# flatironinstitute/bayes-kit

Hardware: AMD Instinct MI355X
Metric: leapfrog steps/sec (whole node), D=1024 × 65 536 chains; ESS/sec (higher is better)
Workload: dtype f64; 1 GPU; BASELINE.json configs[2]: ill-conditioned Gaussian D=1024 (lam=logspace(0,4)), HMC L=64 eps=0.006, diag metric of ones, model-opaque gradient op; chains_per_gpu=65536, dims=1024, leapfrog_steps=64, parallelism=chains sharded x1, chain_tile=8192

## Files before the change

### bayes-kit_amd/bayes_kit_amd/_lib.py

```python
from __future__ import annotations

import ctypes
import os
from ctypes import c_double, c_int, c_int64, c_uint64, c_void_p

import torch

_LIB_PATH = os.path.join(os.path.dirname(os.path.abspath(__file__)), "lib", "libbkhip.so")

RNG_WORDS = 11
RNG_PHILOX = 0
RNG_PCG64 = 1
ACCEPT_HMC = 0
ACCEPT_MALA = 1

P = c_void_p
I = c_int64
F = c_double

SIGNATURES = {
    "bk_version": [],
    "bk_rng_init_philox": [P, I, c_uint64, c_uint64, I, P],
    "bk_refresh_work_elems": [I, I],
    "bk_momentum_refresh": [c_int, P, I, P, F, F, P, I, P, P, P, I, I, P, I, P],
    "bk_momentum_refresh_precond": [c_int, P, I, P, I, P, P, I, I, P, I, P],
    "bk_log_uniform": [c_int, P, I, P, P, I, P],
    "bk_uniform": [c_int, P, I, P, P, I, P],
    "bk_leapfrog_kick_drift": [P, P, P, P, I, P, I, I, P, F, c_int, F, c_int, F, I, I, P],
    "bk_leapfrog_finish": [P, P, I, P, I, I, P, F, c_int, P, I, I, P],
    "bk_precond_pack": [P, P, I, P],
    "bk_leapfrog_finish_precond": [P, P, I, P, I, I, P, F, c_int, P, I, I, P],
    "bk_leapfrog_kick_drift_n": [P, P, P, P, I, P, I, I, P, F, c_int, F, c_int, F, I, I, P, P],
    "bk_leapfrog_first_step_gather": [P, P, P, I, P, P, P, I, P, F, F, I, I, P, P],
    "bk_leapfrog_finish_level": [P, P, I, P, I, I, P, F, c_int, P, I, I, P, P, P, P, P, P, P, P],
    "bk_mh_accept": [c_int, P, P, P, P, P, P, P, P, I, P],
    "bk_select_columns": [P, P, P, P, P, P, I, I, I, P],
    "bk_blend_columns": [P, P, P, P, I, I, I, P],
    "bk_compact_indices": [P, I, P, P, P, P],
    "bk_dr_begin": [P, P, P, P, P, P, I, P],
    "bk_dr_retry_test": [c_int, P, I, P, F, P, I, P],
    "bk_dr_level_begin": [P, P, P, P, P, I, P, P],
    "bk_dr_ghost_update": [P, P, I, P, P, P, P, P],
    "bk_dr_accept_prob": [P, P, P, P, P, F, P, P, I, P, P],
    "bk_dr_accept_test": [c_int, P, I, P, P, P, I, P, P, P, P, P, P, P],
    "bk_dr_accept_prob_test": [c_int, P, I, P, P, P, P, P, F, I, P, P, P, P, P, P, P],
    "bk_dr_accept_prob_ghost": [P, P, P, P, P, F, P, P, I, P, P, P, P],
    "bk_dr_begin_retry": [c_int, P, I, P, P, P, P, P, P, F, P, I, P, I, P],
    "bk_dr_refresh_begin": [c_int, P, I, P, F, F, P, I, P, P, I, I, P, I, P, P, P, P, P, F, P, I, P, P, P],
    "bk_dr_accept_prob_test_next": [c_int, P, I, P, P, P, P, P, F, I, P, P, P, P, P, P, P, P, P],
    "bk_dr_accept_prob_ghost_next": [P, P, P, P, P, F, P, P, I, P, P, P, P, P, P],
    "bk_scatter_columns": [P, P, I, I, P, P, P, P, P, P, I, I, P, P, P, P],
    "bk_mala_propose": [c_int, P, I, P, P, P, I, F, F, I, I, P],
    "bk_mala_propose_from_normals": [P, P, P, I, I, P, I, F, F, I, I, P],
    "bk_mala_propose_from_normals_precond": [P, P, P, I, I, P, P, I, F, F, I, I, P],
    "bk_normals_chain_major": [c_int, P, I, P, I, I, I, P, I, P],
    "bk_mala_logq": [P, P, P, P, I, F, P, P, I, I, P],
    "bk_mala_logq_precond": [P, P, P, P, I, P, F, P, P, I, I, P],
    "bk_mala_single_draw": [c_int, P, I, P, P, P, P, P, P, P, I, P, P, F, F, I, c_int, F, P],
    "bk_mala_step_supported": [I, I, I],
    "bk_mala_step": [P, P, P, P, P, I, P, P, P, P, I, F, F, P, P, P, I, I, P],
    "bk_mala_step_gaussian": [P, P, P, I, P, P, P, P, P, I, F, F, P, P, P, I, I, P],
    "bk_mala_step_precond": [P, P, P, P, P, I, P, P, P, P, P, I, F, F, P, P, P, I, I, P],
    "bk_mala_step_gaussian_precond": [P, P, P, I, P, P, P, P, P, P, I, F, F, P, P, P, I, I, P],
    "bk_target_iso_gaussian_grad": [P, P, P, I, I, I, P],
    "bk_target_diag_gaussian_grad": [P, P, P, I, P, I, I, P],
    "bk_target_funnel_grad": [P, P, P, I, I, I, P],
    "bk_target_iso_gaussian_grad_n": [P, P, P, I, I, I, P, P],
    "bk_target_diag_gaussian_grad_n": [P, P, P, I, P, I, I, P, P],
    "bk_target_funnel_grad_n": [P, P, P, I, I, I, P, P],
    "bk_leapfrog_step_funnel": [P, P, I, P, F, I, I, P, P],
    "bk_leapfrog_step_gaussian": [P, P, I, P, P, F, I, I, P, P],
    "bk_dr_proposal_gaussian": [P, P, P, I, P, P, P, P, P, P, I, P, F, I, I, I, P, P, P, P, P, P, P, P, P, P, P],
    "bk_hmc_trajectory_funnel": [P, P, P, P, P, P, P, I, P, F, I, I, I, P],
    "bk_hmc_trajectory_gaussian": [P, P, P, P, I, P, P, F, I, I, I, P],
    "bk_hmc_draw_gaussian": [P, P, I, P, P, I, P, P, F, I, P, P, P, P, P, P, P, P, P, I, I, P],
    "bk_hmc_draw_gaussian_precond": [P, P, I, P, P, I, P, P, F, I, P, P, P, P, P, P, P, P, P, I, I, P],
    "bk_dr_proposal_funnel": [P, P, P, I, P, P, P, P, P, P, I, P, F, I, I, I, P, P, P, P, P, P, P, P, P, P],
    "bk_dense_metric_apply": [P, I, P, P, I, I, I, P],
    "bk_gemm_chains": [P, I, I, I, P, I, P, I, I, P, I, P],
    "bk_gemm_chains_work_elems": [I, I, I],
    "bk_logistic_residual": [P, I, P, P, I, I, I, P],
    "bk_logistic_finish": [P, P, I, P, I, F, F, P, P, P, I, I, P],
    "bk_dot_columns": [P, P, I, F, P, I, I, P],
    "bk_resample_indices": [P, I, P, I, P, P, P],
    "bk_gather_columns": [P, P, I, P, I, I, I, P],
    "bk_relayout": [P, I, I, P, I, I, I, I, P],
    "bk_welford_update": [P, P, I, P, I, I, I, I, P],
    "bk_record_series": [P, I, P, I, P, P, I, I, I, P],
    "bk_record_series_dev": [P, I, P, I, P, P, I, P, I, I, P],
    "bk_welford_update_dev": [P, P, I, P, I, P, I, I, I, P],
    "bk_rhat_partials": [P, P, I, I, P, P, I, I, P],
    "bk_accept_stat": [P, P, P, P, I, P, P, P],
    "bk_chain_mean_var": [P, I, P, I, P, P, I, P],
    "bk_end_pos_pairs": [P, I, I, P, I, P],
    "bk_ess": [P, I, I, c_int, P, P, I, P],
    "bk_iat_from_acor": [P, I, I, c_int, P, P, I, P],
    "bk_gemm_chains_logistic": [P, I, I, I, P, I, P, I, I, P, P],
    "bk_autocorr": [P, I, I, P, I, I, P],
    "bk_autocorr_fft_work_bytes": [I, I],
    "bk_autocorr_fft": [P, I, I, P, I, I, P, I, P],
    "bk_rank_normalize": [P, F, P, I, P],
    "bk_sort_by_key_work_bytes": [I],
    "bk_sort_by_key": [P, P, P, P, I, P, I, P],
    "bk_count_below": [P, I, P, I, P, P],
    "bk_scatter_ranks": [P, I, F, P, P],
    "bk_ess_multi_work_bytes": [I, I, I],
    "bk_ess_split_moments": [P, I, I, I, c_int, F, P, P, P, P, I, P],
    "bk_ess_between_sq": [P, I, P, P, P, I, P],
    "bk_ess_lag_sums_max_half": [],
    "bk_ess_lag_sums": [P, I, I, I, c_int, F, P, I, I, P, P, I, P],
    "bk_ess_acov_sums": [P, I, I, I, P, I, I, P, P, I, P],
    "bk_ess_indicator": [P, I, I, I, F, P, I, P],
    "bk_select_ranks": [P, P, I, P, I, P, P],
    "bk_host_normals": [c_int, P, P, I],
    "bk_host_uniforms": [c_int, P, P, I],
    "bk_host_log1p": [F],
    "bk_host_exp": [F],
}
_RESTYPE = {"bk_gemm_chains_work_elems": c_int64, "bk_host_log1p": c_double, "bk_host_exp": c_double, "bk_refresh_work_elems": c_int64, "bk_sort_by_key_work_bytes": c_int64,
             "bk_autocorr_fft_work_bytes": c_int64, "bk_ess_multi_work_bytes": c_int64, "bk_ess_lag_sums_max_half": c_int64}


class BkHipError(RuntimeError):
    pass


class GhostLink(ctypes.Structure):
    _fields_ = [("parent_H", P), ("parent_h", P), ("parent_live", P), ("parent_a", P), ("a_out", P),
                ("prob_retry", F), ("next_index", P), ("next_count", P)]


class Ghost0(ctypes.Structure):
    _fields_ = [("h", F), ("steps", I), ("parent_a", P), ("prob_retry", F), ("next_index", P), ("next_count", P),
                ("lanes_out", P), ("lanes_total", P)]


class DiagJob(ctypes.Structure):
    _fields_ = [("theta", P), ("ld_theta", I), ("C", I), ("D", I), ("n_dev", P), ("mean", P), ("m2", P), ("ld", I),
                ("n_offset", I), ("series", P), ("dims", P), ("K", I), ("logp", P), ("capacity", I), ("row_offset", I)]


class ScatterJob(ctypes.Structure):
    _fields_ = [("mask", P), ("index", P), ("n", I), ("D", I), ("dst0", P), ("src0", P), ("dst1", P), ("src1", P),
                ("dst2", P), ("src2", P), ("ld_dst", I), ("ld_src", I), ("sdst", P), ("ssrc", P), ("n_dev", P)]


_lib = None


def lib_path() -> str:
    return _LIB_PATH


def load() -> ctypes.CDLL:
    global _lib
    if _lib is not None:
        return _lib
    if not os.path.exists(_LIB_PATH):
        raise BkHipError(
            f"{_LIB_PATH} is missing: build it with `python bayes-kit_amd/build.py` "
            "(or __graft_entry__.build()).  There is no CPU fallback."
        )
    lib = ctypes.CDLL(_LIB_PATH)
    for name, argtypes in SIGNATURES.items():
        fn = getattr(lib, name)
        fn.argtypes = argtypes
        fn.restype = _RESTYPE.get(name, c_int)
    _lib = lib
    return lib


def require_gpu() -> torch.device:
    load()
    if not torch.cuda.is_available():
        raise BkHipError(
            "bayes_kit_amd needs an AMD Instinct GPU (gfx950) visible to PyTorch-ROCm; "
            "no device found and there is no CPU fallback."
        )
    return torch.device("cuda", torch.cuda.current_device())


class RawDeviceArray:

    _hip = None
    live = 0

    def __init__(self, shape):
        if RawDeviceArray._hip is None:
            RawDeviceArray._hip = ctypes.CDLL("libamdhip64.so")
        self.shape = tuple(int(x) for x in shape)
        n = 8
        for x in self.shape:
            n *= x
        p = c_void_p()
        rc = RawDeviceArray._hip.hipMalloc(ctypes.byref(p), ctypes.c_size_t(max(n, 8)))
        if rc != 0 or not p.value:
            raise BkHipError(f"hipMalloc of {n} bytes failed: hipError_t {rc}")
        self._ptr = p.value
        RawDeviceArray.live += 1
        self.__cuda_array_interface__ = {"shape": self.shape, "typestr": "<f8", "data": (self._ptr, False), "version": 2,
                                         "strides": None}

    def tensor(self):
        t = torch.as_tensor(self, device=torch.device("cuda", torch.cuda.current_device()))
        t._bk_raw = self
        return t

    def __del__(self):
        p, self._ptr = getattr(self, "_ptr", None), None
        cls = type(self)
        hip = getattr(cls, "_hip", None)
        if p and hip is not None:
            cls.live -= 1
            try:
                hip.hipFree(ctypes.c_void_p(p))
            except Exception:
                pass


def check(status: int, what: str) -> None:
    if status != 0:
        kind = "argument/layout error" if status < 0 else "hipError_t"
        raise BkHipError(f"{what} failed: {kind} {status}")


def ptr(t) -> int:
    return 0 if t is None else t.data_ptr()


def stream_handle() -> int:
    return torch.cuda.current_stream().cuda_stream


def _ld(t) -> int:
    if t.dim() != 2 or (t.shape[1] > 1 and t.stride(1) != 1):
        raise BkHipError(f"expected a [D, C] tensor with contiguous chains, got strides {t.stride()}")
    return t.stride(0) if t.shape[0] > 1 else max(t.stride(0), t.shape[1])


class Ops:

    name = "hip"

    def __init__(self):
        self.lib = load()
        self.device = require_gpu()
        self.timed = None
        self.timed_stride = 1
        self._timed_seen = {}

    def _call(self, name, *args):
        rec = self.timed.get(name) if self.timed is not None else None
        if rec is not None and self.timed_stride > 1:
            k = self._timed_seen.get(name, 0)
            self._timed_seen[name] = k + 1
            if k % self.timed_stride:
                rec = None
        if rec is None:
            check(getattr(self.lib, name)(*args), name)
            return
        e0 = torch.cuda.Event(enable_timing=True)
        e1 = torch.cuda.Event(enable_timing=True)
        e0.record()
        check(getattr(self.lib, name)(*args), name)
        e1.record()
        rec.append((e0, e1))

    @staticmethod
    def _s():
        return stream_handle()

    def rng_init_philox(self, state, key0, chain_id0):
        self._call("bk_rng_init_philox", ptr(state), state.stride(0), key0 & (2**64 - 1),
                   chain_id0 & (2**64 - 1), state.shape[1], self._s())

    def refresh_work(self, C, D):
        return torch.empty(self.lib.bk_refresh_work_elems(C, D), dtype=torch.float64, device=self.device)

    def momentum_refresh(self, kind, state, loc_in, loc_mul, scale, out, metric, kin_out, active=None, work=None):
        D, C = out.shape
        self._call("bk_momentum_refresh", kind, ptr(state), state.stride(0), ptr(loc_in), loc_mul, scale,
                   ptr(out), _ld(out), ptr(metric), ptr(kin_out), ptr(active), C, D, ptr(work),
                   0 if work is None else work.numel(), self._s())

    def momentum_refresh_precond(self, kind, state, out, precond, kin_out, work=None):
        D, C = out.shape
        assert precond.is_contiguous() and tuple(precond.shape) == (3, D)
        self._call("bk_momentum_refresh_precond", kind, ptr(state), state.stride(0), ptr(out), _ld(out), ptr(precond),
                   ptr(kin_out), C, D, ptr(work), 0 if work is None else work.numel(), self._s())

    def log_uniform(self, kind, state, out, active=None):
        self._call("bk_log_uniform", kind, ptr(state), state.stride(0), ptr(out), ptr(active),
                   out.shape[0], self._s())

    def uniform(self, kind, state, out, active=None):
        self._call("bk_uniform", kind, ptr(state), state.stride(0), ptr(out), ptr(active), out.shape[0],
                   self._s())

    def kick_drift(self, theta_in, theta_out, rho_in, rho_out, grad, metric, eps,
                   use_pre, pre, use_kick, kick, n_dev=None):
        D, C = theta_out.shape
        ld = _ld(theta_out)
        assert _ld(theta_in) == ld and _ld(rho_in) == ld and _ld(rho_out) == ld
        if n_dev is None:
            self._call("bk_leapfrog_kick_drift", ptr(theta_in), ptr(theta_out), ptr(rho_in), ptr(rho_out), ld,
                       ptr(grad), grad.stride(0), grad.stride(1), ptr(metric), eps, int(use_pre), pre,
                       int(use_kick), kick, C, D, self._s())
        else:
            self._call("bk_leapfrog_kick_drift_n", ptr(theta_in), ptr(theta_out), ptr(rho_in), ptr(rho_out), ld,
                       ptr(grad), grad.stride(0), grad.stride(1), ptr(metric), eps, int(use_pre), pre,
                       int(use_kick), kick, C, D, ptr(n_dev), self._s())

    def first_step_gather(self, theta_in, rho_in, grad_in, src_index, theta_out, rho_out, metric, eps, pre,
                          n_dev=None):
        D, n = theta_out.shape
        ld_in = _ld(theta_in)
        assert _ld(rho_in) == ld_in and _ld(grad_in) == ld_in and _ld(rho_out) == _ld(theta_out)
        self._call("bk_leapfrog_first_step_gather", ptr(theta_in), ptr(rho_in), ptr(grad_in), ld_in,
                   ptr(src_index), ptr(theta_out), ptr(rho_out), _ld(theta_out), ptr(metric), eps, pre,
                   n, D, ptr(n_dev), self._s())

    def leapfrog_finish(self, rho_in, rho_out, grad, metric, half, negate, kin_out, n_dev=None, level=None,
                        lanes_out=None, lanes_total=None):
        D, C = rho_in.shape
        if rho_out is not None:
            assert _ld(rho_out) == _ld(rho_in)
        gs = (0, 0) if grad is None else grad.stride()
        if n_dev is None and level is None and lanes_out is None and lanes_total is None:
            self._call("bk_leapfrog_finish", ptr(rho_in), ptr(rho_out), _ld(rho_in), ptr(grad), gs[0], gs[1],
                       ptr(metric), half, int(negate), ptr(kin_out), C, D, self._s())
            return
        logp, H, h, live = level if level is not None else (None,) * 4
        self._call("bk_leapfrog_finish_level", ptr(rho_in), ptr(rho_out), _ld(rho_in), ptr(grad), gs[0], gs[1],
                   ptr(metric), half, int(negate), ptr(kin_out), C, D, ptr(n_dev), ptr(logp), ptr(H), ptr(h),
                   ptr(live), ptr(lanes_out), ptr(lanes_total), self._s())

    def precond_pack(self, v, precond):
        D = v.shape[0]
        assert v.is_contiguous() and precond.is_contiguous() and tuple(precond.shape) == (3, D)
        self._call("bk_precond_pack", ptr(v), ptr(precond), D, self._s())

    def leapfrog_finish_precond(self, rho_in, rho_out, grad, precond, half, negate, kin_out):
        D, C = rho_in.shape
        if rho_out is not None:
            assert _ld(rho_out) == _ld(rho_in)
        assert precond.is_contiguous() and tuple(precond.shape) == (3, D)
        gs = (0, 0) if grad is None else grad.stride()
        self._call("bk_leapfrog_finish_precond", ptr(rho_in), ptr(rho_out), _ld(rho_in), ptr(grad), gs[0], gs[1],
                   ptr(precond), half, int(negate), ptr(kin_out), C, D, self._s())

    def accept_stat(self, lp_cur, a_cur, lp_prop, a_prop, out, work=None):
        C = lp_cur.shape[0]
        if work is None:
            work = torch.empty(max(2, 2 * ((C + 255) // 256)), dtype=torch.float64, device=lp_cur.device)
        assert work.numel() >= 2 * ((C + 255) // 256)
        self._call("bk_accept_stat", ptr(lp_cur), ptr(a_cur), ptr(lp_prop), ptr(a_prop), C, ptr(out), ptr(work), self._s())

    def mh_accept(self, mode, lp_cur, a_cur, lp_prop, a_prop, log_u, mask, ret, count):
        self._call("bk_mh_accept", mode, ptr(lp_cur), ptr(a_cur), ptr(lp_prop), ptr(a_prop), ptr(log_u),
                   ptr(mask), ptr(ret), ptr(count), lp_cur.shape[0], self._s())

    def select_columns(self, mask, dst0, src0, dst1=None, src1=None, copy0=None):
        D, C = dst0.shape
        ld = _ld(dst0)
        assert _ld(src0) == ld and (dst1 is None or (_ld(dst1) == ld and _ld(src1) == ld))
        assert copy0 is None or _ld(copy0) == ld
        self._call("bk_select_columns", ptr(mask), ptr(dst0), ptr(src0), ptr(dst1), ptr(src1), ptr(copy0), ld,
                   C, D, self._s())


    def blend_columns(self, mask, a, b, out):
        D, C = a.shape
        ld = _ld(a)
        assert _ld(b) == ld and _ld(out) == ld
        self._call("bk_blend_columns", ptr(mask), ptr(a), ptr(b), ptr(out), ld, C, D, self._s())

    def compact_indices(self, mask, n, idx_out, count_out, n_dev=None):
        self._call("bk_compact_indices", ptr(mask), n, ptr(idx_out), ptr(count_out), ptr(n_dev), self._s())

    def dr_begin(self, logp, kin, cur_H, cur_h, rej, alive):
        self._call("bk_dr_begin", ptr(logp), ptr(kin), ptr(cur_H), ptr(cur_h), ptr(rej), ptr(alive),
                   logp.shape[0], self._s())

    def dr_retry_test(self, kind, state, rej, prob_retry, alive):
        self._call("bk_dr_retry_test", kind, ptr(state), state.stride(0), ptr(rej), float(prob_retry),
                   ptr(alive), alive.shape[0], self._s())

    def dr_level_begin(self, logp, kin, H, h, live, n, n_dev=None):
        self._call("bk_dr_level_begin", ptr(logp), ptr(kin), ptr(H), ptr(h), ptr(live), n, ptr(n_dev), self._s())

    def dr_ghost_update(self, ga, sub_index, m, h, live, a, n_dev=None):
        self._call("bk_dr_ghost_update", ptr(ga), ptr(sub_index), m, ptr(h), ptr(live), ptr(a), ptr(n_dev),
                   self._s())

    def dr_accept_prob(self, H, cur_H, h, cur_h, cur_index, prob_retry, live, a, n, n_dev=None):
        self._call("bk_dr_accept_prob", ptr(H), ptr(cur_H), ptr(h), ptr(cur_h), ptr(cur_index),
                   float(prob_retry), ptr(live), ptr(a), n, ptr(n_dev), self._s())

    def dr_accept_test(self, kind, state, chain_index, a, H, n, cur_H, cur_h, rej, alive, accepted, n_dev=None):
        self._call("bk_dr_accept_test", kind, ptr(state), state.stride(0), ptr(chain_index), ptr(a), ptr(H),
                   n, ptr(cur_H), ptr(cur_h), ptr(rej), ptr(alive), ptr(accepted), ptr(n_dev), self._s())

    def dr_accept_prob_test(self, kind, state, chain_index, H, h, live, a, prob_retry, n, cur_H, cur_h, rej, alive,
                            accepted, n_dev=None):
        self._call("bk_dr_accept_prob_test", kind, ptr(state), state.stride(0), ptr(chain_index), ptr(H), ptr(h),
                   ptr(live), ptr(a), float(prob_retry), n, ptr(cur_H), ptr(cur_h), ptr(rej), ptr(alive),
                   ptr(accepted), ptr(n_dev), self._s())

    def dr_accept_prob_ghost(self, H, parent_H, h, parent_h, sub_index, prob_retry, live, a, n, parent_live, parent_a,
                             n_dev=None):
        self._call("bk_dr_accept_prob_ghost", ptr(H), ptr(parent_H), ptr(h), ptr(parent_h), ptr(sub_index),
                   float(prob_retry), ptr(live), ptr(a), n, ptr(n_dev), ptr(parent_live), ptr(parent_a), self._s())

    def dr_begin_retry(self, kind, state, logp, kin, cur_H, cur_h, rej, alive, prob_retry, counters, draw_counter=None):
        self._call("bk_dr_begin_retry", kind, ptr(state), state.stride(0), ptr(logp), ptr(kin), ptr(cur_H), ptr(cur_h),
                   ptr(rej), ptr(alive), float(prob_retry), ptr(counters), 0 if counters is None else counters.numel(),
                   ptr(draw_counter), logp.shape[0], self._s())

    def dr_refresh_begin(self, kind, state, loc_in, loc_mul, scale, out, metric, kin_out, work, logp, cur_H, cur_h, rej,
                         alive, prob_retry, counters, draw_counter=None, side=None):
        D, C = out.shape
        self._call("bk_dr_refresh_begin", kind, ptr(state), state.stride(0), ptr(loc_in), loc_mul, scale, ptr(out),
                   _ld(out), ptr(metric), ptr(kin_out), C, D, ptr(work), 0 if work is None else work.numel(), ptr(logp),
                   ptr(cur_H), ptr(cur_h), ptr(rej), ptr(alive), float(prob_retry), ptr(counters),
                   0 if counters is None else counters.numel(), ptr(draw_counter),
                   None if side is None else ctypes.cast(ctypes.pointer(side), P), self._s())

    def diag_job(self, theta, n_dev, welford=None, record=None):
        D, C = theta.shape
        assert n_dev.dtype == torch.int64 and (welford is not None or record is not None)
        j = DiagJob(ptr(theta), _ld(theta), C, D, ptr(n_dev), None, None, 0, 0, None, None, 0, None, 0, 0)
        if welford is not None:
            mean, m2, n_offset = welford
            assert _ld(m2) == _ld(mean)
            j.mean, j.m2, j.ld, j.n_offset = ptr(mean), ptr(m2), _ld(mean), int(n_offset)
        if record is not None:
            dims, logp, series, row_offset = record
            j.series, j.dims, j.K, j.logp = ptr(series), ptr(dims), (0 if dims is None else dims.numel()), ptr(logp) or None
            j.capacity, j.row_offset = series.shape[1], int(row_offset)
        return j

    def dr_accept_prob_test_next(self, kind, state, chain_index, H, h, live, a, prob_retry, n, cur_H, cur_h, rej, alive,
                                 accepted, next_index, next_count, n_dev=None):
        self._call("bk_dr_accept_prob_test_next", kind, ptr(state), state.stride(0), ptr(chain_index), ptr(H), ptr(h),
                   ptr(live), ptr(a), float(prob_retry), n, ptr(cur_H), ptr(cur_h), ptr(rej), ptr(alive),
                   ptr(accepted), ptr(n_dev), ptr(next_index), ptr(next_count), self._s())

    def dr_accept_prob_ghost_next(self, H, parent_H, h, parent_h, sub_index, prob_retry, live, a, n, parent_live,
                                  parent_a, next_index, next_count, n_dev=None):
        self._call("bk_dr_accept_prob_ghost_next", ptr(H), ptr(parent_H), ptr(h), ptr(parent_h), ptr(sub_index),
                   float(prob_retry), ptr(live), ptr(a), n, ptr(n_dev), ptr(parent_live), ptr(parent_a),
                   ptr(next_index), ptr(next_count), self._s())

    def scatter_columns(self, mask, index, n, dsts, srcs, sdst=None, ssrc=None, n_dev=None):
        d = list(dsts) + [None] * (3 - len(dsts))
        s_ = list(srcs) + [None] * (3 - len(srcs))
        D = dsts[0].shape[0]
        self._call("bk_scatter_columns", ptr(mask), ptr(index), n, D, ptr(d[0]), ptr(s_[0]), ptr(d[1]),
                   ptr(s_[1]), ptr(d[2]), ptr(s_[2]), _ld(dsts[0]), _ld(srcs[0]), ptr(sdst), ptr(ssrc),
                   ptr(n_dev), self._s())

    def mala_propose(self, kind, state, theta, grad, theta_prop, eps, sqrt2eps):
        D, C = theta.shape
        ld = _ld(theta)
        assert _ld(grad) == ld and _ld(theta_prop) == ld
        self._call("bk_mala_propose", kind, ptr(state), state.stride(0), ptr(theta), ptr(grad),
                   ptr(theta_prop), ld, eps, sqrt2eps, C, D, self._s())

    def mala_propose_from_normals(self, theta, grad, z, theta_prop, eps, sqrt2eps):
        D, C = theta.shape
        ld = _ld(theta)
        assert _ld(grad) == ld and _ld(theta_prop) == ld and tuple(z.shape) == (D, C)
        self._call("bk_mala_propose_from_normals", ptr(theta), ptr(grad), ptr(z), z.stride(0), z.stride(1),
                   ptr(theta_prop), ld, eps, sqrt2eps, C, D, self._s())

    def mala_propose_from_normals_precond(self, theta, grad, z, precond, theta_prop, eps, sqrt2eps):
        D, C = theta.shape
        ld = _ld(theta)
        assert _ld(grad) == ld and _ld(theta_prop) == ld and tuple(z.shape) == (D, C)
        assert precond.is_contiguous() and tuple(precond.shape) == (3, D)
        self._call("bk_mala_propose_from_normals_precond", ptr(theta), ptr(grad), ptr(z), z.stride(0), z.stride(1),
                   ptr(precond), ptr(theta_prop), ld, eps, sqrt2eps, C, D, self._s())

    def normals_chain_major(self, kind, state, zt, D, snapshot=None, max_workgroups=0):
        C = zt.shape[0]
        assert zt.stride(1) == 1 and zt.shape[1] >= D
        assert snapshot is None or (snapshot.shape == state.shape and snapshot.stride(0) == state.stride(0))
        self._call("bk_normals_chain_major", kind, ptr(state), state.stride(0), ptr(zt), zt.stride(0), C, D,
                   ptr(snapshot), int(max_workgroups or 0), self._s())

    def mala_logq(self, theta, grad, theta_prop, grad_prop, eps, lp_forward, lp_reverse):
        D, C = theta.shape
        ld = _ld(theta)
        assert _ld(grad) == ld and _ld(theta_prop) == ld and _ld(grad_prop) == ld
        self._call("bk_mala_logq", ptr(theta), ptr(grad), ptr(theta_prop), ptr(grad_prop), ld, eps,
                   ptr(lp_forward), ptr(lp_reverse), C, D, self._s())

    def mala_logq_precond(self, theta, grad, theta_prop, grad_prop, precond, eps, lp_forward, lp_reverse):
        D, C = theta.shape
        ld = _ld(theta)
        assert _ld(grad) == ld and _ld(theta_prop) == ld and _ld(grad_prop) == ld
        assert precond.is_contiguous() and tuple(precond.shape) == (3, D)
        self._call("bk_mala_logq_precond", ptr(theta), ptr(grad), ptr(theta_prop), ptr(grad_prop), ld, ptr(precond), eps,
                   ptr(lp_forward), ptr(lp_reverse), C, D, self._s())

    def mala_step_supported(self, C, D, ld):
        return bool(self.lib.bk_mala_step_supported(C, D, ld))

    def mala_step(self, theta, theta_out, grad, theta_prop, grad_prop, lp, lp_prop, log_u, zt_next, eps, sqrt2eps,
                  mask, ret, count):
        D, C = theta.shape
        ld = _ld(theta)
        assert _ld(theta_out) == ld and _ld(grad) == ld and _ld(theta_prop) == ld and _ld(grad_prop) == ld
        ldz = 0
        if zt_next is not None:
            assert zt_next.shape[0] == C and zt_next.stride(1) == 1 and zt_next.shape[1] >= D
            ldz = zt_next.stride(0)
        self._call("bk_mala_step", ptr(theta), ptr(theta_out), ptr(grad), ptr(theta_prop), ptr(grad_prop), ld,
                   ptr(lp), ptr(lp_prop), ptr(log_u), ptr(zt_next), ldz, eps, sqrt2eps, ptr(mask), ptr(ret),
                   ptr(count), C, D, self._s())

    def mala_step_precond(self, theta, theta_out, grad, theta_prop, grad_prop, precond, lp, lp_prop, log_u, zt_next, eps,
                          sqrt2eps, mask, ret, count):
        D, C = theta.shape
        ld = _ld(theta)
        assert _ld(theta_out) == ld and _ld(grad) == ld and _ld(theta_prop) == ld and _ld(grad_prop) == ld
        assert precond.is_contiguous() and tuple(precond.shape) == (3, D)
        ldz = 0
        if zt_next is not None:
            assert zt_next.shape[0] == C and zt_next.stride(1) == 1 and zt_next.shape[1] >= D
            ldz = zt_next.stride(0)
        self._call("bk_mala_step_precond", ptr(theta), ptr(theta_out), ptr(grad), ptr(theta_prop), ptr(grad_prop), ld,
                   ptr(precond), ptr(lp), ptr(lp_prop), ptr(log_u), ptr(zt_next), ldz, eps, sqrt2eps, ptr(mask), ptr(ret),
                   ptr(count), C, D, self._s())

    def mala_step_gaussian(self, lam, theta, theta_out, theta_prop, lp, lp_prop, log_u, zt_next, eps, sqrt2eps, mask, ret,
                           count, precond=None):
        D, C = theta.shape
        ld = _ld(theta)
        assert _ld(theta_out) == ld and _ld(theta_prop) == ld
        ldz = 0
        if zt_next is not None:
            assert zt_next.shape[0] == C and zt_next.stride(1) == 1 and zt_next.shape[1] >= D
            ldz = zt_next.stride(0)
        if precond is not None:
            assert precond.is_contiguous() and tuple(precond.shape) == (3, D)
            self._call("bk_mala_step_gaussian_precond", ptr(theta), ptr(theta_out), ptr(theta_prop), ld, ptr(lam),
                       ptr(precond), ptr(lp), ptr(lp_prop), ptr(log_u), ptr(zt_next), ldz, eps, sqrt2eps, ptr(mask),
                       ptr(ret), ptr(count), C, D, self._s())
            return
        self._call("bk_mala_step_gaussian", ptr(theta), ptr(theta_out), ptr(theta_prop), ld, ptr(lam), ptr(lp), ptr(lp_prop),
                   ptr(log_u), ptr(zt_next), ldz, eps, sqrt2eps, ptr(mask), ptr(ret), ptr(count), C, D, self._s())

    def target_grad(self, kind, params, theta, grad, logp, n_dev=None):
        D, C = theta.shape
        ld = _ld(theta)
        if grad is not None:
            assert _ld(grad) == ld
        if n_dev is not None:
            if kind == "iso_gaussian":
                self._call("bk_target_iso_gaussian_grad_n", ptr(theta), ptr(grad), ptr(logp), ld, C, D, ptr(n_dev),
                           self._s())
            elif kind == "diag_gaussian":
                self._call("bk_target_diag_gaussian_grad_n", ptr(theta), ptr(grad), ptr(logp), ld, ptr(params),
                           C, D, ptr(n_dev), self._s())
            elif kind == "funnel":
                self._call("bk_target_funnel_grad_n", ptr(theta), ptr(grad), ptr(logp), ld, C, D, ptr(n_dev),
                           self._s())
            else:
                raise BkHipError(f"built-in target {kind!r} has no counted gradient")
        elif kind == "iso_gaussian":
            self._call("bk_target_iso_gaussian_grad", ptr(theta), ptr(grad), ptr(logp), ld, C, D, self._s())
        elif kind == "diag_gaussian":
            self._call("bk_target_diag_gaussian_grad", ptr(theta), ptr(grad), ptr(logp), ld, ptr(params),
                       C, D, self._s())
        elif kind == "funnel":
            self._call("bk_target_funnel_grad", ptr(theta), ptr(grad), ptr(logp), ld, C, D, self._s())
        else:
            raise BkHipError(f"unknown built-in target {kind!r}")

    def hmc_trajectory_funnel(self, theta_in, rho, grad_in, theta_out, grad_out, logp_out, kin_out, metric, eps, steps):
        D, C = theta_in.shape
        ld = _ld(theta_in)
        assert all(_ld(t) == ld for t in (rho, grad_in, theta_out, grad_out))
        self._call("bk_hmc_trajectory_funnel", ptr(theta_in), ptr(rho), ptr(grad_in), ptr(theta_out), ptr(grad_out),
                   ptr(logp_out), ptr(kin_out), ld, ptr(metric), eps, steps, C, D, self._s())

    def leapfrog_step_funnel(self, theta, rho, metric, h, n_dev=None):
        D, n = theta.shape
        ld = _ld(theta)
        assert _ld(rho) == ld
        self._call("bk_leapfrog_step_funnel", ptr(theta), ptr(rho), ld, ptr(metric), h, n, D, ptr(n_dev), self._s())

    def hmc_trajectory_gaussian(self, theta_in, theta_out, rho_in, rho_out, lam, metric, eps, steps):
        D, C = theta_in.shape
        ld = _ld(theta_in)
        assert _ld(theta_out) == ld and _ld(rho_in) == ld and _ld(rho_out) == ld
        self._call("bk_hmc_trajectory_gaussian", ptr(theta_in), ptr(theta_out), ptr(rho_in), ptr(rho_out), ld,
                   ptr(lam), ptr(metric), eps, steps, C, D, self._s())

    def hmc_draw_gaussian(self, theta_in, theta_out, rho_in, zt, lam, metric, eps, steps, part, kin0, kin1, lp_out,
                          accept=None, precond=None):
        D, C = theta_in.shape
        ld = _ld(theta_in)
        assert _ld(theta_out) == ld and (rho_in is None or _ld(rho_in) == ld) and part.numel() >= 12 * C
        ldz = 0
        if zt is not None:
            assert zt.shape[0] == C and zt.stride(1) == 1 and zt.shape[1] >= D
            ldz = zt.stride(0)
        lp_cur, log_u, mask, ret, count = accept if accept is not None else (None,) * 5
        name = "bk_hmc_draw_gaussian"
        if precond is not None:
            assert metric is None and precond.is_contiguous() and tuple(precond.shape) == (3, D)
            name, metric = "bk_hmc_draw_gaussian_precond", precond
        self._call(name, ptr(theta_in), ptr(theta_out), ld, ptr(rho_in), ptr(zt), ldz, ptr(lam),
                   ptr(metric), eps, steps, ptr(part), ptr(kin0), ptr(kin1), ptr(lp_out), ptr(lp_cur), ptr(log_u),
                   ptr(mask), ptr(ret), ptr(count), C, D, self._s())

    def scatter_job(self, mask, index, n, dsts, srcs, sdst=None, ssrc=None, n_dev=None):
        d = list(dsts) + [None] * (3 - len(dsts))
        s_ = list(srcs) + [None] * (3 - len(srcs))
        return ScatterJob(ptr(mask) or None, ptr(index) or None, n, dsts[0].shape[0], ptr(d[0]) or None, ptr(s_[0]) or None,
                          ptr(d[1]) or None, ptr(s_[1]) or None, ptr(d[2]) or None, ptr(s_[2]) or None, _ld(dsts[0]),
                          _ld(srcs[0]), ptr(sdst) or None, ptr(ssrc) or None, ptr(n_dev) or None)

    def ghost_link(self, parent_H, parent_h, parent_live, parent_a, a_out, prob_retry, next_index=None, next_count=None):
        return GhostLink(ptr(parent_H), ptr(parent_h), ptr(parent_live), ptr(parent_a), ptr(a_out), float(prob_retry),
                         ptr(next_index) or None, ptr(next_count) or None)

    def ghost0(self, h, steps, parent_a, prob_retry, next_index=None, next_count=None, lanes_out=None, lanes_total=None):
        return Ghost0(float(h), int(steps), ptr(parent_a), float(prob_retry), ptr(next_index) or None,
                      ptr(next_count) or None, ptr(lanes_out) or None, ptr(lanes_total) or None)

    def dr_proposal_gaussian(self, lam, theta_in, rho_in, grad_in, src_index, theta_out, rho_out, grad_out, logp_out,
                             kin_out, metric, h, steps, n_dev=None, lanes_out=None, lanes_total=None, level=None, job=None,
                             ghost=None, ghost0=None):
        D, n = theta_out.shape
        H, hh, live = level if level is not None else (None, None, None)
        ld_in = _ld(theta_in)
        assert _ld(rho_in) == ld_in and (grad_in is None or _ld(grad_in) == ld_in)
        ld_out = _ld(theta_out)
        assert _ld(rho_out) == ld_out and (grad_out is None or _ld(grad_out) == ld_out)
        self._call("bk_dr_proposal_gaussian", ptr(theta_in), ptr(rho_in), ptr(grad_in), ld_in, ptr(src_index),
                   ptr(theta_out), ptr(rho_out), ptr(grad_out), ptr(logp_out), ptr(kin_out), ld_out, ptr(metric),
                   h, steps, n, D, ptr(n_dev), ptr(lanes_out), ptr(lanes_total), ptr(H), ptr(hh), ptr(live),
                   None if job is None else ctypes.byref(job), None if ghost is None else ctypes.byref(ghost),
                   None if ghost0 is None else ctypes.byref(ghost0), ptr(lam), self._s())

    def leapfrog_step_gaussian(self, lam, theta, rho, metric, h, n_dev=None):
        D, n = theta.shape
        ld = _ld(theta)
        assert _ld(rho) == ld
        self._call("bk_leapfrog_step_gaussian", ptr(theta), ptr(rho), ld, ptr(lam), ptr(metric), h, n, D, ptr(n_dev), self._s())

    def dr_proposal_funnel(self, theta_in, rho_in, grad_in, src_index, theta_out, rho_out, grad_out, logp_out,
                           kin_out, metric, h, steps, n_dev=None, lanes_out=None, lanes_total=None, level=None, job=None,
                           ghost=None, ghost0=None):
        D, n = theta_out.shape
        H, hh, live = level if level is not None else (None, None, None)
        ld_in = _ld(theta_in)
        assert _ld(rho_in) == ld_in and (grad_in is None or _ld(grad_in) == ld_in)
        ld_out = _ld(theta_out)
        assert _ld(rho_out) == ld_out and (grad_out is None or _ld(grad_out) == ld_out)
        args = (ptr(theta_in), ptr(rho_in), ptr(grad_in), ld_in, ptr(src_index),
                ptr(theta_out), ptr(rho_out), ptr(grad_out), ptr(logp_out), ptr(kin_out), ld_out, ptr(metric),
                h, steps, n, D, ptr(n_dev), ptr(lanes_out), ptr(lanes_total), ptr(H), ptr(hh), ptr(live))
        self._call("bk_dr_proposal_funnel", *args, None if job is None else ctypes.byref(job),
                   None if ghost is None else ctypes.byref(ghost),
                   None if ghost0 is None else ctypes.byref(ghost0), self._s())

    def dense_metric_apply(self, M, X, Y):
        D, C = X.shape
        assert _ld(Y) == _ld(X)
        self._call("bk_dense_metric_apply", ptr(M), _ld(M), ptr(X), ptr(Y), _ld(X), C, D, self._s())

    def gemm_chains_work(self, R, K, C):
        n = int(self.lib.bk_gemm_chains_work_elems(R, K, C))
        return torch.empty(n, dtype=torch.float64, device=self.device) if n > 0 else None

    def gemm_chains(self, A, X, Y, work=None):
        R, K = A.shape
        assert X.shape[0] == K and Y.shape[0] == R
        self._call("bk_gemm_chains", ptr(A), _ld(A), R, K, ptr(X), _ld(X), ptr(Y), _ld(Y), X.shape[1],
                   ptr(work), 0 if work is None else work.numel(), self._s())

    def gemm_chains_logistic(self, A, X, Y, y_rows):
        R, K = A.shape
        assert X.shape[0] == K and Y.shape[0] == R and y_rows.numel() == R
        self._call("bk_gemm_chains_logistic", ptr(A), _ld(A), R, K, ptr(X), _ld(X), ptr(Y), _ld(Y), X.shape[1],
                   ptr(y_rows), self._s())

    def logistic_residual(self, Z, y, part, segments=None):
        N, C = Z.shape
        self._call("bk_logistic_residual", ptr(Z), _ld(Z), ptr(y), ptr(part), N, C,
                   part.shape[0] if part is not None else int(segments or 256), self._s())

    def logistic_finish(self, G, theta, part, inv_prior_var, t, grad, logp, loglik):
        D, C = theta.shape
        ld = _ld(theta)
        assert (G is None or _ld(G) == ld) and (grad is None or _ld(grad) == ld)
        self._call("bk_logistic_finish", ptr(G), ptr(theta), ld, ptr(part), 1 if part is None else part.shape[0], inv_prior_var, t,
                   ptr(grad), ptr(logp), ptr(loglik), C, D, self._s())

    def dot_columns(self, x, y, scale, out):
        D, C = x.shape
        assert _ld(y) == _ld(x)
        self._call("bk_dot_columns", ptr(x), ptr(y), _ld(x), scale, ptr(out), C, D, self._s())

    def resample_indices(self, weights, u, cdf_work, idx_out):
        self._call("bk_resample_indices", ptr(weights), weights.shape[0], ptr(u), u.shape[0], ptr(cdf_work),
                   ptr(idx_out), self._s())

    def gather_columns(self, index, src, dst):
        D, m = dst.shape
        self._call("bk_gather_columns", ptr(index), ptr(src), _ld(src), ptr(dst), _ld(dst), m, D, self._s())

    def relayout(self, src, dst):
        D, C = dst.shape
        self._call("bk_relayout", ptr(src), src.stride(0), src.stride(1), ptr(dst), dst.stride(0),
                   dst.stride(1), C, D, self._s())

    def welford_update(self, mean, m2, theta, n):
        D, C = theta.shape
        assert _ld(m2) == _ld(mean)
        self._call("bk_welford_update", ptr(mean), ptr(m2), _ld(mean), ptr(theta), _ld(theta), n, C, D, self._s())

    def record_series(self, theta, dims, logp, series, row):
        D, C = theta.shape
        assert series.is_contiguous() and series.shape[2] == C
        self._call("bk_record_series", ptr(theta), _ld(theta), ptr(dims), 0 if dims is None else dims.numel(), ptr(logp),
                   ptr(series), series.shape[1], row, C, self._s())

    def record_series_dev(self, theta, dims, logp, series, row_dev, row_offset):
        D, C = theta.shape
        assert series.is_contiguous() and series.shape[2] == C and row_dev.dtype == torch.int64
        self._call("bk_record_series_dev", ptr(theta), _ld(theta), ptr(dims), 0 if dims is None else dims.numel(),
                   ptr(logp), ptr(series), series.shape[1], ptr(row_dev), int(row_offset), C, self._s())

    def welford_update_dev(self, mean, m2, theta, n_dev, n_offset):
        D, C = theta.shape
        assert _ld(m2) == _ld(mean) and n_dev.dtype == torch.int64
        self._call("bk_welford_update_dev", ptr(mean), ptr(m2), _ld(mean), ptr(theta), _ld(theta), ptr(n_dev),
                   int(n_offset), C, D, self._s())

    def rhat_partials(self, mean, m2, n, center, out):
        D, C = mean.shape
        assert _ld(m2) == _ld(mean)
        self._call("bk_rhat_partials", ptr(mean), ptr(m2), _ld(mean), n, ptr(center), ptr(out), C, D,
                   self._s())

    def chain_mean_var(self, x, lengths, mean, var):
        N, C = x.shape
        self._call("bk_chain_mean_var", ptr(x), _ld(x), ptr(lengths), N, ptr(mean), ptr(var), C, self._s())

    def rank_normalize(self, rank, S, out):
        self._call("bk_rank_normalize", ptr(rank), float(S), ptr(out), rank.numel(), self._s())

    def sort_by_key(self, keys, vals):
        n = keys.numel()
        ko, vo = torch.empty_like(keys), torch.empty_like(vals)
        if n == 0:
            return ko, vo
        nb = self.lib.bk_sort_by_key_work_bytes(n)
        if nb < 0:
            raise BkHipError("bk_sort_by_key_work_bytes failed")
        work = torch.empty(max(1, nb), dtype=torch.uint8, device=keys.device)
        self._call("bk_sort_by_key", ptr(keys), ptr(ko), ptr(vals), ptr(vo), n, ptr(work), work.numel(), self._s())
        return ko, vo

    def count_below(self, sorted_keys, queries):
        out = torch.empty(queries.numel(), dtype=torch.int64, device=queries.device)
        self._call("bk_count_below", ptr(sorted_keys), sorted_keys.numel(), ptr(queries), queries.numel(), ptr(out),
                   self._s())
        return out

    def scatter_ranks(self, payload, base, out):
        self._call("bk_scatter_ranks", ptr(payload), payload.numel(), float(base), ptr(out), self._s())

    def autocorr(self, x, out):
        N, C = x.shape
        self._call("bk_autocorr", ptr(x), _ld(x), N, ptr(out), _ld(out), C, self._s())

    def autocorr_fft_work_bytes(self, N, C):
        return int(self.lib.bk_autocorr_fft_work_bytes(N, C))

    def autocorr_fft(self, x, out):
        N, C = x.shape
        work = torch.empty(max(16, self.lib.bk_autocorr_fft_work_bytes(N, C)), dtype=torch.uint8, device=x.device)
        self._call("bk_autocorr_fft", ptr(x), _ld(x), N, ptr(out), _ld(out), C, ptr(work), work.numel(), self._s())

    def end_pos_pairs(self, acor, out):
        N, C = acor.shape
        self._call("bk_end_pos_pairs", ptr(acor), max(C, acor.stride(0)) if N else C, N, ptr(out), C, self._s())

    def iat_from_acor(self, acor, estimator, ess_out, iat_out=None):
        N, C = acor.shape
        self._call("bk_iat_from_acor", ptr(acor), _ld(acor), N, estimator, ptr(ess_out), ptr(iat_out), C, self._s())

    def ess(self, x, estimator, ess_out, iat_out=None):
        N, C = x.shape
        self._call("bk_ess", ptr(x), _ld(x), N, estimator, ptr(ess_out), ptr(iat_out), C, self._s())

    def _ess_work(self, n, C, nlags, device):
        nb = int(self.lib.bk_ess_multi_work_bytes(n, C, nlags))
        if nb < 0:
            raise BkHipError("bk_ess_multi_work_bytes failed")
        return torch.empty(nb // 8, dtype=torch.float64, device=device)

    def ess_lag_sums_max_half(self):
        return int(self.lib.bk_ess_lag_sums_max_half())

    def ess_split_moments(self, x, q, chain_mean, chain_g0):
        N, C = x.shape
        out = torch.empty(3, dtype=torch.float64, device=x.device)
        work = self._ess_work(N // 2, C, 1, x.device)
        self._call("bk_ess_split_moments", ptr(x), _ld(x), N, C, 0 if q is None else 1, 0.0 if q is None else float(q),
                   ptr(chain_mean), ptr(chain_g0), ptr(out), ptr(work), work.numel() * 8, self._s())
        return out

    def ess_between_sq(self, chain_mean, centre):
        out = torch.empty(1, dtype=torch.float64, device=chain_mean.device)
        work = self._ess_work(1, chain_mean.numel(), 1, chain_mean.device)
        self._call("bk_ess_between_sq", ptr(chain_mean), chain_mean.numel(), ptr(centre), ptr(out), ptr(work),
                   work.numel() * 8, self._s())
        return out

    def ess_lag_sums(self, x, q, chain_mean, lag0, nlags):
        N, C = x.shape
        out = torch.empty(nlags, dtype=torch.float64, device=x.device)
        work = self._ess_work(N // 2, C, nlags, x.device)
        self._call("bk_ess_lag_sums", ptr(x), _ld(x), N, C, 0 if q is None else 1, 0.0 if q is None else float(q),
                   ptr(chain_mean), lag0, nlags, ptr(out), ptr(work), work.numel() * 8, self._s())
        return out

    def ess_acov_sums(self, acor, chain_g0, lag0, nlags):
        n, C = acor.shape
        out = torch.empty(nlags, dtype=torch.float64, device=acor.device)
        work = self._ess_work(n, C, nlags, acor.device)
        self._call("bk_ess_acov_sums", ptr(acor), _ld(acor), n, C, ptr(chain_g0), lag0, nlags, ptr(out), ptr(work),
                   work.numel() * 8, self._s())
        return out

    def ess_indicator(self, x, q, out):
        n, C = x.shape
        self._call("bk_ess_indicator", ptr(x), _ld(x), n, C, float(q), ptr(out), _ld(out), self._s())

    def select_ranks(self, rank, values, targets, out):
        self._call("bk_select_ranks", ptr(rank), ptr(values), rank.numel(), ptr(targets), targets.numel(), ptr(out),
                   self._s())


_default_ops = None


def default_ops() -> Ops:
    global _default_ops
    if _default_ops is None:
        _default_ops = Ops()
    return _default_ops
```

### bayes-kit_amd/bayes_kit_amd/hmc.py

```python
from __future__ import annotations

from typing import Optional

import numpy as np
import torch

from . import _lib
from ._engine import ManyChainSampler


class HMCDiag(ManyChainSampler):
    TUNING = ("graph", "prefetch_rng", "tune_placement", "chain_tile")

    def __init__(
        self,
        model,
        stepsize: float,
        steps: int,
        metric_diag=None,
        init=None,
        seed=None,
        *,
        chains: Optional[int] = None,
        chain_id0: int = 0,
        path: str = "auto",
        metric_dense=None,
        precond_diag=None,
        tuning: Optional[dict] = None,
        ops=None,
        **knobs,
    ):
        fuse_builtin, fuse_steps = self._resolve_path(path)
        tn = self._resolve_tuning(tuning, knobs)
        chain_tile, graph = tn.get("chain_tile"), tn.get("graph")
        prefetch_rng, tune_placement = tn.get("prefetch_rng"), tn.get("tune_placement")
        self._stepsize = stepsize
        self._steps = steps
        self._pd = None
        self._stat = None
        if precond_diag is not None and (metric_diag is not None or metric_dense is not None):
            raise ValueError("give precond_diag or metric_diag / metric_dense, not both")
        self._setup(model, metric_diag, init, seed, chains, chain_id0, ops)
        self._M = None
        if metric_dense is not None:
            if metric_diag is not None:
                raise ValueError("give metric_diag or metric_dense, not both")
            if not self._batched:
                raise ValueError("metric_dense needs a batched device model")
            self._install_metric_dense(metric_dense)
            fuse_builtin = False
        if precond_diag is not None:
            self._install_precond(precond_diag)
        self._init_graph(graph, prefetch_rng)
        self._fused_draw = (bool(fuse_builtin) and self._batched and self._M is None and hasattr(model, "bk_hmc_draw"))
        if self._pd is not None and not hasattr(model, "bk_hmc_draw_precond"):
            self._fused_draw = False
        self._fused = self._fused_draw
        self._lanes_traj = (bool(fuse_builtin) and self._batched and self._M is None and hasattr(model, "bk_hmc_proposal"))
        self._step_hook = (bool(fuse_steps) and self._batched and self._M is None and hasattr(model, "bk_leapfrog_step"))
        self._traj_hook = (bool(fuse_builtin) and self._step_hook and hasattr(model, "bk_leapfrog_trajectory"))
        self._chain_tile = self._pick_tile(chain_tile)
        self._fused_zt = self._fused_draw and self._rng_kind == _lib.RNG_PHILOX and self._dim >= 32
        D, C, dev = self._dim, self._C, self._ops.device
        f64 = dict(dtype=torch.float64, device=dev)
        self._rho_bufs = [None if self._fused_zt else torch.empty((D, C), **f64)]
        self._theta_p = torch.empty((D, C), **f64)
        self._grad = torch.empty((D, C), **f64)
        self._grad_p = torch.empty((D, C), **f64)
        self._lp = torch.empty(C, **f64)
        self._lp_p = torch.empty(C, **f64)
        self._kin0_bufs = [torch.empty(C, **f64)]
        self._kin1 = torch.empty(C, **f64)
        self._logu_bufs = [torch.empty(C, **f64)]
        self._ret = torch.empty(C, **f64)
        self._mask = torch.empty(C, dtype=torch.uint8, device=dev)
        self._accepted = torch.zeros(1, dtype=torch.int32, device=dev)
        if self._fused_draw:
            self._part = torch.empty(12 * C, **f64)
        if self._fused_zt:
            dp = (D + 7) // 8 * 8
            self._zt_bufs = [torch.empty((C, dp), **f64)]
        if self._M is not None:
            self._mv = torch.empty((D, C), **f64)
            self._mv_rng = torch.empty((D, C), **f64)
        self._have_cache = False
        self._draws = 0
        self._rebind = self._batched and not self._use_graph
        if prefetch_rng is None:
            prefetch_rng = self._batched and self._ops.device.type == "cuda"
        self._prefetch = bool(prefetch_rng) and self._batched and not self._use_graph
        self._pf_slot = 0
        self._pf_ready = False
        self._pf_event = None
        self._pf_kin_stale = False
        self._snap = None
        if self._prefetch:
            if self._fused_zt:
                self._zt_bufs.append(torch.empty_like(self._zt_bufs[0]))
                self._rho_bufs.append(None)
            else:
                self._rho_bufs.append(torch.empty((D, C), **f64))
            self._kin0_bufs.append(torch.empty(C, **f64))
            self._logu_bufs.append(torch.empty(C, **f64))
            self._init_side_stream()
            if self._fused_zt:
                self._snap = [torch.empty_like(self._rng_state) for _ in range(2)]
            else:
                self._rng_logical = self._rng_state.clone()
        self.placement = None
        if self._wants_placement_tuning(tune_placement) and not self._fused and self._M is None:
            self._tune_placement()

    def _install_metric_dense(self, metric_dense):
        if isinstance(metric_dense, torch.Tensor) and metric_dense.dim() == 1 and self._M is not None:
            v = metric_dense.to(device=self._ops.device, dtype=torch.float64)
            if v.shape[0] != self._dim:
                raise ValueError(f"a diagonal metric needs {self._dim} entries")
            self._M.copy_(torch.diag(v))
            self._M_chol.copy_(torch.diag(torch.sqrt(v)))
            self._M_inv.copy_(torch.diag(1.0 / v))
            return
        Mt = torch.as_tensor(metric_dense, dtype=torch.float64).cpu()
        if tuple(Mt.shape) != (self._dim, self._dim):
            raise ValueError(f"metric_dense must be ({self._dim}, {self._dim})")
        Mt = 0.5 * (Mt + Mt.t())
        dev_ = self._ops.device
        chol = torch.linalg.cholesky(Mt)
        inv = torch.linalg.inv(Mt)
        inv = 0.5 * (inv + inv.t())
        if self._M is None:
            self._M, self._M_chol, self._M_inv = (x.to(dev_).contiguous() for x in (Mt, chol, inv))
        else:
            self._M.copy_(Mt)
            self._M_chol.copy_(chol)
            self._M_inv.copy_(inv)

    def set_metric_dense(self, metric_dense):
        if self._M is None:
            raise ValueError("this sampler was built without metric_dense")
        self._install_metric_dense(metric_dense)
        if self._prefetch and self._pf_ready:
            if self._pf_event is not None:
                torch.cuda.current_stream().wait_event(self._pf_event)
            self._pf_ready, self._pf_event = False, None

    def _install_precond(self, v):
        if self._M is not None or (self._pd is None and self._metric_dev is not None):
            raise ValueError("precond_diag cannot be combined with metric_diag / metric_dense")
        vt = torch.as_tensor(v, dtype=torch.float64).reshape(-1)
        if vt.shape[0] != self._dim:
            raise ValueError(f"precond_diag has {vt.shape[0]} entries, model has {self._dim} dims")
        vt = vt.to(self._ops.device).contiguous()
        if not bool((torch.isfinite(vt) & (vt > 0.0)).all()):
            raise ValueError("precond_diag must hold finite, positive variances")
        if self._pd is None:
            self._pd = torch.empty((3, self._dim), dtype=torch.float64, device=self._ops.device)
            self._metric_dev, self._metric_identity = self._pd[0], False
            self._drop_graphs()
        self._ops.precond_pack(vt, self._pd)

    def set_precond_diag(self, v):
        self._install_precond(v)
        if self._fused_draw and not hasattr(self._model, "bk_hmc_draw_precond"):
            self._leave_whole_draw()
        if getattr(self, "_prefetch", False) and self._pf_ready and not self._fused_zt:
            if self._pf_event is not None:
                torch.cuda.current_stream().wait_event(self._pf_event)
            self._rng_state.copy_(self._rng_logical)
            self._pf_ready, self._pf_event = False, None

    def _leave_whole_draw(self):
        if self._prefetch and self._pf_ready:
            if self._pf_event is not None:
                torch.cuda.current_stream().wait_event(self._pf_event)
            self._rng_state.copy_(self._snap[self._pf_slot] if self._snap is not None else self._rng_logical)
            self._pf_ready, self._pf_event = False, None
        self._fused_draw = self._fused = self._fused_zt = False
        self._rho_bufs = [r if r is not None else torch.empty_like(self._theta_p) for r in self._rho_bufs]
        if self._prefetch and self._snap is not None:
            self._snap, self._rng_logical = None, self._rng_state.clone()
        self._have_cache = False
        self._drop_graphs()

    @property
    def precond_diag(self):
        return None if self._pd is None else self._pd[0].cpu().numpy().copy()

    def _tune_placement(self):
        ops, m, eps = self._ops, self._metric_dev, float(self._stepsize)
        n_rho = len(self._rho_bufs)

        builtin = hasattr(self._model, "bk_eval")

        def cost(a):
            tp, gp, rhos = a[0], a[1], a[2:2 + n_rho]
            ms = sum(self._time_ms(lambda r=r: ops.kick_drift(tp, tp, r, r, gp, m, eps, False, 0.0, True, eps))
                     for r in rhos) / n_rho
            if builtin:
                ms += self._time_ms(lambda: self._model.bk_eval(tp, gp, None))
            return ms

        chosen, rep = self._tune_roles([self._theta_p, self._grad_p] + list(self._rho_bufs) + [self._grad], cost)
        self._theta_p, self._grad_p = chosen[0], chosen[1]
        self._rho_bufs = chosen[2:2 + n_rho]
        self._grad = chosen[2 + n_rho]
        key = "step_ms" if builtin else "kick_drift_ms"
        self.placement = {key + "_as_allocated": rep["ms_as_allocated"], key + "_chosen": rep["ms_chosen"],
                          "assignments_tried": rep["assignments_tried"]}

    LLC_BYTES = 192 << 20
    MIN_TILE = 8192

    @classmethod
    def default_chain_tile(cls, C, D):
        t = cls.LLC_BYTES // (3 * 8 * D)
        t -= t % 2
        return t if t >= cls.MIN_TILE and C >= 2 * t else C

    def _pick_tile(self, chain_tile):
        C = self._C
        if chain_tile is None:
            opaque_loop = (self._batched and self._M is None and hasattr(self._model, "bk_eval")
                           and not self._fused_draw and not self._lanes_traj and not self._step_hook)
            return self.default_chain_tile(C, self._dim) if opaque_loop else C
        t = int(chain_tile)
        return C if t <= 0 or t >= C else max(2, t - t % 2)

    def accept_rate(self) -> float:
        n = self._draws * self._C
        return float(self._accepted.item()) / n if n else float("nan")

    @property
    def last_accept(self):
        return self._mask.bool() if self._batched else bool(self._mask[0].item())

    def _set_metric(self, m):
        if self._pd is not None:
            raise ValueError("metric_diag cannot be combined with precond_diag")
        super()._set_metric(m)
        self._pf_kin_stale = True


    def rng_state(self):
        return self._logical_rng().cpu().numpy().view(np.uint64)

    def _state_tensors(self):
        return {"theta": self._theta_dc, "grad": self._grad, "lp": self._lp, "accepted": self._accepted}

    def _logical_rng(self):
        if getattr(self, "_prefetch", False) and self._pf_ready:
            if self._pf_event is not None:
                self._pf_event.synchronize()
            return self._rng_logical if self._snap is None else self._snap[self._pf_slot]
        return self._rng_state

    def load_state_dict(self, sd):
        if getattr(self, "_prefetch", False) and self._pf_ready:
            torch.cuda.synchronize()
            self._pf_ready, self._pf_event = False, None
        if self._rebind:
            self._theta_dc = torch.empty_like(self._theta_dc)
        super().load_state_dict(sd)

    def _state_extra(self):
        return {"stepsize": float(self._stepsize), "precond_diag": None if self._pd is None else self._pd[0].cpu().clone()}

    def _load_extra(self, extra):
        if "stepsize" in extra:
            self._stepsize = extra["stepsize"]
        pv = extra.get("precond_diag")
        if pv is not None:
            self._install_precond(pv)
            if self._fused_draw and not hasattr(self._model, "bk_hmc_draw_precond"):
                self._leave_whole_draw()
        elif self._pd is not None and "precond_diag" in extra:
            raise ValueError("checkpoint was written without precond_diag, this sampler has one")

    def _after_load(self):
        self._pf_event, self._pf_slot, self._pf_ready, self._pf_kin_stale = None, 0, False, False

    def _refresh_stale_kinetic(self):
        if self._pf_kin_stale and self._pf_ready and not self._fused_draw:
            self._ops.leapfrog_finish(self._rho_bufs[self._pf_slot], None, None, self._metric_dev, 0.0, False,
                                      self._kin0_bufs[self._pf_slot])
        self._pf_kin_stale = False

    def _randomness(self, slot):
        ops = self._ops
        if self._fused_zt:
            ops.normals_chain_major(self._rng_kind, self._rng_state, self._zt_bufs[slot], self._dim,
                                    None if self._snap is None else self._snap[slot])
        elif self._pd is not None:
            ops.momentum_refresh_precond(self._rng_kind, self._rng_state, self._rho_bufs[slot], self._pd,
                                         self._kin0_bufs[slot], self._rng_work)
        elif self._M is None:
            ops.momentum_refresh(self._rng_kind, self._rng_state, None, 0.0, 1.0, self._rho_bufs[slot],
                                 self._metric_dev, None if self._fused_draw else self._kin0_bufs[slot], None,
                                 self._rng_work)
        else:
            ops.momentum_refresh(self._rng_kind, self._rng_state, None, 0.0, 1.0, self._mv_rng, None, None,
                                 None, self._rng_work)
            ops.dense_metric_apply(self._M_chol, self._mv_rng, self._rho_bufs[slot])
            self._dense_kinetic(self._rho_bufs[slot], self._kin0_bufs[slot], self._mv_rng)
        ops.log_uniform(self._rng_kind, self._rng_state, self._logu_bufs[slot])

    def _dense_kinetic(self, rho, kin_out, scratch):
        self._ops.dense_metric_apply(self._M_inv, rho, scratch)
        self._ops.dot_columns(rho, scratch, 0.5, kin_out)

    def _mg(self, g):
        if self._M is None:
            return g
        self._ops.dense_metric_apply(self._M, self._materialize_dense(g), self._mv)
        return self._mv

    def _materialize_dense(self, g):
        if g.dim() == 2 and g.stride(1) == 1:
            return g
        self._ops.relayout(g, self._grad_p)
        return self._grad_p

    def _current_randomness(self):
        self._zt_slot = 0 if not self._prefetch else self._pf_slot
        if not self._prefetch:
            self._randomness(0)
            return self._rho_bufs[0], self._kin0_bufs[0], self._logu_bufs[0]
        cur = self._pf_slot
        if not self._pf_ready:
            self._randomness(cur)
            self._pf_kin_stale = False
        else:
            if self._pf_event is not None:
                torch.cuda.current_stream().wait_event(self._pf_event)
            self._refresh_stale_kinetic()
        return self._rho_bufs[cur], self._kin0_bufs[cur], self._logu_bufs[cur]

    def _start_next_randomness(self):
        if not self._prefetch:
            return
        main = torch.cuda.current_stream()
        nxt = 1 - self._pf_slot
        ready, ev = self._ev_ready[nxt], self._ev_done[nxt]
        ready.record(main)
        self._side.wait_event(ready)
        with torch.cuda.stream(self._side):
            if self._snap is None:
                self._rng_logical.copy_(self._rng_state)
            self._randomness(nxt)
            ev.record(self._side)
        self._pf_event, self._pf_slot, self._pf_ready = ev, nxt, True

    def _graph_key(self):
        return (float(self._stepsize), int(self._steps))

    def warmup(self, draws, target_accept=0.8, adapt_metric=True, group=None):
        from .adapt import DualAveraging, warmup_windows
        from .diagnostics import RunningMoments, _gather_sum, pooled_variance_from_moments

        draws = int(draws)
        if draws < 1:
            raise ValueError(f"warmup: draws must be >= 1, got {draws}")
        if not 0.0 < float(target_accept) < 1.0:
            raise ValueError(f"warmup: target_accept must be inside (0, 1), got {target_accept}")
        if adapt_metric and (self._M is not None or (self._pd is None and self._metric_dev is not None)):
            raise ValueError("warmup: adapt_metric=True estimates precond_diag, which cannot be combined with "
                             "metric_diag / metric_dense (pass adapt_metric=False to tune the step size alone)")
        if not self._batched:
            raise ValueError("warmup needs a batched device model (the statistics are taken across chains)")
        ops, dev, C, D = self._ops, self._ops.device, self._C, self._dim
        init, term, ends = warmup_windows(draws)
        if not adapt_metric:
            ends = []
        da = DualAveraging(float(self._stepsize), float(target_accept))
        mom = RunningMoments(D, C, ops) if ends else None
        self._stat = torch.zeros(3, dtype=torch.float64, device=dev)
        self._stat[2] = float(C)
        self._stat_work = torch.empty(max(2, 2 * ((C + 255) // 256)), dtype=torch.float64, device=dev)
        eps_hist, alpha_hist, nan_chains = [], [], 0
        try:
            for it in range(draws):
                eps_hist.append(float(self._stepsize))
                self._draw()
                self._join_side_stream()
                self._draws += 1
                tot = _gather_sum(self._stat, group).cpu()
                chains_total = float(tot[2])
                alpha = float(tot[0]) / chains_total
                alpha_hist.append(alpha)
                nan_chains += int(tot[1])
                if mom is not None and init <= it < draws - term:
                    mom.update(self._theta_dc, layout="dc")
                eps = da.step(alpha)
                if it + 1 in ends:
                    n_eff = float(mom.n) * chains_total
                    var = pooled_variance_from_moments(mom.mean, mom.m2, mom.n, ops, group)
                    self.set_precond_diag(n_eff / (n_eff + 5.0) * var + 1e-3 * 5.0 / (n_eff + 5.0))
                    mom.reset()
                    eps = da.final()
                    da.restart(eps)
                if it + 1 == draws:
                    eps = da.final()
                self._stepsize = eps
        finally:
            self._stat, self._stat_work = None, None
            del mom
            self._drop_graphs()
        return {"stepsize": float(self._stepsize), "precond_diag": self.precond_diag, "eps": eps_hist, "alpha": alpha_hist,
                "window_ends": list(ends), "nan_chains": nan_chains}

    def sample(self):
        self._run_draw(self._draw)
        self._join_side_stream()
        self._draws += 1
        return self._draw_out(self._theta_dc, self._ret)

    def _draw(self):
        ops = self._ops
        eps, L, m = float(self._stepsize), int(self._steps), self._metric_dev
        half = 0.5 * eps
        th, thp = self._theta_dc, self._theta_p
        mirror = not self._batched

        rho, kin0, logu = self._current_randomness()
        self._start_next_randomness()

        if self._fused_draw:
            if not self._have_cache:
                self._eval_logp(th, self._lp)
                self._have_cache = True
            zt = self._zt_bufs[self._zt_slot] if self._fused_zt else None
            m_draw = None if (m is None or self._metric_identity) else m
            accept = (self._lp, logu, self._mask, self._ret, self._accepted)
            in_launch = accept if self._stat is None else None
            if self._pd is not None:
                self._model.bk_hmc_draw_precond(th, thp, rho, zt, self._pd, eps, L, self._part, kin0, self._kin1, self._lp_p,
                                                accept=in_launch)
            else:
                self._model.bk_hmc_draw(th, thp, rho, zt, m_draw, eps, L, self._part, kin0, self._kin1, self._lp_p,
                                        accept=in_launch)
            if in_launch is None:
                self._accept(kin0, logu)
            self._take(th, thp)
            return

        if self._lanes_traj and L >= 1 and self._pd is None:
            if not self._have_cache:
                self._materialize(self._eval_grad(th, self._grad, self._lp), self._grad)
                self._have_cache = True
            if self._model.bk_hmc_proposal(th, rho, self._grad, thp, self._grad_p, self._lp_p, self._kin1, m, eps, L):
                self._accept(kin0, logu)
                self._take(th, thp, self._grad, self._grad_p)
                return

        if mirror:
            self._eval_logp(th, self._lp)
            g = self._eval_grad(th, self._grad, None)
        else:
            if not self._have_cache:
                self._materialize(self._eval_grad(th, self._grad, self._lp), self._grad)
                self._have_cache = True
            g = self._grad

        if self._M is not None:
            m = None
        if L == 0:
            ops.kick_drift(th, thp, rho, rho, self._mg(g), m, 0.0, True, -half, False, 0.0)
            g_last = g
            if not mirror:
                self._lp_p.copy_(self._lp)
        elif (self._traj_hook and not mirror and self._chain_tile >= self._C
              and self._model.bk_leapfrog_trajectory(th, rho, g, None, thp, rho, self._grad_p, self._lp_p, m, eps, L,
                                                     hmc_first=True)):
            self._grad_calls += L
            g_last = self._grad_p
        else:
            g_last = None
            T = self._chain_tile
            for c0 in range(0, self._C, T):
                c1 = min(self._C, c0 + T)
                tile = (c0, c1) != (0, self._C)
                v = (lambda a: a[:, c0:c1]) if tile else (lambda a: a)
                th_t, thp_t, rho_t, gp_t, g_t = v(th), v(thp), v(rho), v(self._grad_p), v(g)
                lp_t = self._lp_p[c0:c1] if tile else self._lp_p
                gl = None
                for n in range(L):
                    last = n == L - 1
                    if n == 0:
                        ops.kick_drift(th_t, thp_t, rho_t, rho_t, self._mg(g_t), m, eps, True, -half, True, eps)
                    elif self._step_hook and not mirror:
                        self._grad_calls += 1
                        self._model.bk_leapfrog_step(thp_t, rho_t, m, eps)
                    else:
                        ops.kick_drift(thp_t, thp_t, rho_t, rho_t, self._mg(gl), m, eps, False, 0.0, True, eps)
                    if self._step_hook and not mirror and not last:
                        continue
                    want_lp = lp_t if (last and not mirror) else None
                    gl = self._eval_grad(thp_t, gp_t, want_lp)
                if tile:
                    self._materialize(gl, gp_t)
                    g_last = self._grad_p
                else:
                    g_last = gl
        if self._pd is not None:
            ops.leapfrog_finish_precond(rho, None, g_last, self._pd, half, False, self._kin1)
        elif self._M is None:
            ops.leapfrog_finish(rho, None, g_last, m, half, False, self._kin1)
        else:
            ops.leapfrog_finish(rho, rho, self._mg(g_last), None, half, False, None)
            self._dense_kinetic(rho, self._kin1, self._mv)
        if mirror:
            self._eval_logp(thp, self._lp_p)
        self._accept(kin0, logu)
        if mirror:
            self._select(self._mask, th, thp)
        else:
            gp = self._materialize(g_last, self._grad_p) if L > 0 else None
            self._take(th, thp, self._grad if gp is not None else None, gp)

    def _accept(self, kin0, logu):
        if self._stat is not None:
            self._ops.accept_stat(self._lp, kin0, self._lp_p, self._kin1, self._stat, self._stat_work)
        self._ops.mh_accept(_lib.ACCEPT_HMC, self._lp, kin0, self._lp_p, self._kin1, logu,
                            self._mask, self._ret, self._accepted)

    def _take(self, th, thp, g=None, gp=None):
        if not self._rebind:
            self._select(self._mask, th, thp, g, gp)
            return
        self._out = torch.empty_like(th)
        self._ops.blend_columns(self._mask, th, thp, self._out)
        self._theta_dc = self._out
        if gp is not None:
            self._ops.select_columns(self._mask, g, gp)
```

### bayes-kit_amd/build.py

```python
#!/usr/bin/env python3
import os
import subprocess
import sys
from concurrent.futures import ThreadPoolExecutor

HERE = os.path.dirname(os.path.abspath(__file__))
CSRC = os.path.join(HERE, "csrc")
OUT_DIR = os.path.join(HERE, "bayes_kit_amd", "lib")
OBJ_DIR = os.path.join(HERE, "build")
LIB = os.path.join(OUT_DIR, "libbkhip.so")
SOURCES = ["bk_rng.hip", "bk_integrator.hip", "bk_targets.hip", "bk_targets_gauss_lanes.hip", "bk_diag.hip", "bk_dr.hip", "bk_dense.hip", "bk_smc.hip", "bk_mala.hip", "bk_sort.hip", "bk_fft.hip", "bk_ess_multi.hip"]
HEADERS = ["bk_common.hpp", "bk_ess_tile.hpp", "bk_rng.hpp", "bk_lanes.hpp", "bk_elementwise.hpp", "bk_mala_step.hpp", "ziggurat_tables.inc", os.path.join("..", "..", "include", "bkhip.h"),
           os.path.join("..", "..", "include", "bkhip_math.h")]
FLAGS = ["--offload-arch=gfx950", "-O3", "-std=c++17", "-fPIC", "-ffp-contract=off", "-fno-fast-math",
         "-Wall", "-Wno-unused-function"]
FILE_FLAGS = {"bk_rng.hip": ["-mllvm", "-disable-machine-licm"]}


def _hipcc():
    for c in (os.environ.get("HIPCC"), "/opt/rocm/bin/hipcc", "hipcc"):
        if c and (os.path.isabs(c) and os.path.exists(c) or not os.path.isabs(c)):
            return c
    return "hipcc"


def _stale(target, deps):
    if not os.path.exists(target):
        return True
    t = os.path.getmtime(target)
    return any(os.path.getmtime(d) > t for d in deps)


def build(force=False, verbose=True):
    os.makedirs(OUT_DIR, exist_ok=True)
    os.makedirs(OBJ_DIR, exist_ok=True)
    hdrs = [os.path.join(CSRC, h) for h in HEADERS] + [os.path.abspath(__file__)]
    hipcc = _hipcc()
    jobs = []
    objs = []
    for s in SOURCES:
        src = os.path.join(CSRC, s)
        obj = os.path.join(OBJ_DIR, s.replace(".hip", ".o"))
        objs.append(obj)
        if force or _stale(obj, [src] + hdrs):
            jobs.append([hipcc] + FLAGS + FILE_FLAGS.get(s, []) + ["-c", src, "-o", obj])

    def run(cmd):
        if verbose:
            print(" ".join(cmd), flush=True)
        subprocess.check_call(cmd)

    with ThreadPoolExecutor(max_workers=4) as ex:
        list(ex.map(run, jobs))
    if force or jobs or _stale(LIB, objs):
        run([hipcc, "--offload-arch=gfx950", "-shared", "-fPIC", "-o", LIB] + objs)
    return LIB


PLUGIN_DIR = os.path.join(HERE, "..", "examples", "plugin_target")
PLUGINS = ["ar1_target", "funnel_target"]
PLUGIN_LIB = os.path.join(PLUGIN_DIR, "libar1_target.so")


def build_example_plugin(force=False, verbose=True):
    libs = []
    for name in PLUGINS:
        src = os.path.abspath(os.path.join(PLUGIN_DIR, name + ".hip"))
        lib = os.path.abspath(os.path.join(PLUGIN_DIR, "lib" + name + ".so"))
        public = [os.path.abspath(os.path.join(HERE, "..", "include", h)) for h in ("bkhip.h", "bkhip_math.h")]
        if force or _stale(lib, [src] + public):
            cmd = [_hipcc(), "--offload-arch=gfx950", "-O3", "-std=c++17", "-fPIC", "-shared", "-ffp-contract=off",
                   src, "-o", lib]
            if verbose:
                print(" ".join(cmd), flush=True)
            subprocess.check_call(cmd)
        libs.append(lib)
    return libs[0]


C_HOST_SRC = os.path.join(HERE, "..", "examples", "c_host", "hmc_main.c")
C_HOST_BIN = os.path.join(HERE, "..", "examples", "c_host", "hmc_main")


def build_c_host_example(force=False, verbose=True):
    src, exe = os.path.abspath(C_HOST_SRC), os.path.abspath(C_HOST_BIN)
    if force or _stale(exe, [src, LIB, os.path.join(HERE, "..", "include", "bkhip.h")]):
        rocm = os.environ.get("ROCM_PATH", "/opt/rocm")
        cmd = ["gcc", "-std=gnu11", "-O2", "-D__HIP_PLATFORM_AMD__", src, "-I" + os.path.join(rocm, "include"),
               "-I" + os.path.abspath(os.path.join(HERE, "..", "include")), "-L" + OUT_DIR, "-lbkhip",
               "-L" + os.path.join(rocm, "lib"), "-lamdhip64",
               "-Wl,-rpath,$ORIGIN/../../bayes-kit_amd/bayes_kit_amd/lib", "-Wl,-rpath," + os.path.join(rocm, "lib"),
               "-o", exe]
        if verbose:
            print(" ".join(cmd), flush=True)
        subprocess.check_call(cmd)
    return exe


if __name__ == "__main__":
    print(build(force="--force" in sys.argv))
    print(build_example_plugin(force="--force" in sys.argv))
    print(build_c_host_example(force="--force" in sys.argv))
```

### bayes-kit_amd/csrc/bk_integrator.hip

```cpp
#include "bk_common.hpp"

namespace {

constexpr int KD_ROWS = 4;
constexpr int KD_BLOCK = 256;

__device__ __forceinline__ double kd_elem(double th, double rho, double g, double m, bool has_m,
                                          double eps, int use_pre, double pre, int use_kick,
                                          double kick, double& rho_new) {
  double t = has_m ? m * g : g;
  double r = rho;
  if (use_pre) r = r + pre * t;
  if (use_kick) r = r + kick * t;
  rho_new = r;
  return th + eps * r;
}

typedef double dvec2 __attribute__((ext_vector_type(2)));

template <int ROWS, bool NT>
__global__ __launch_bounds__(KD_BLOCK) void k_kick_drift_v2(
    const double* th_in, double* th_out, const double* rho_in, double* rho_out, i64 ld,
    const double* grad, i64 ldg, const double* metric, double eps, int use_pre, double pre,
    int use_kick, double kick, i64 C2, i64 D) {
  i64 c2 = (i64)blockIdx.x * KD_BLOCK + threadIdx.x;
  i64 d0 = (i64)blockIdx.y * ROWS;
  if (c2 >= C2) return;
  dvec2 t[ROWS], r[ROWS], g[ROWS];
  double m[ROWS];
#pragma unroll
  for (int i = 0; i < ROWS; ++i) {
    i64 d = d0 + i;
    if (d < D) {
      const dvec2* pt = reinterpret_cast<const dvec2*>(th_in + d * ld + 2 * c2);
      const dvec2* pr = reinterpret_cast<const dvec2*>(rho_in + d * ld + 2 * c2);
      const dvec2* pg = reinterpret_cast<const dvec2*>(grad + d * ldg + 2 * c2);
      if (NT) {
        t[i] = __builtin_nontemporal_load(pt);
        r[i] = __builtin_nontemporal_load(pr);
        g[i] = __builtin_nontemporal_load(pg);
      } else {
        t[i] = *pt;
        r[i] = *pr;
        g[i] = *pg;
      }
      m[i] = metric ? metric[d] : 1.0;
    }
  }
#pragma unroll
  for (int i = 0; i < ROWS; ++i) {
    i64 d = d0 + i;
    if (d < D) {
      dvec2 rn, tn;
      double rx, ry;
      tn.x = kd_elem(t[i].x, r[i].x, g[i].x, m[i], metric != nullptr, eps, use_pre, pre, use_kick, kick, rx);
      tn.y = kd_elem(t[i].y, r[i].y, g[i].y, m[i], metric != nullptr, eps, use_pre, pre, use_kick, kick, ry);
      rn.x = rx;
      rn.y = ry;
      dvec2* qr = reinterpret_cast<dvec2*>(rho_out + d * ld + 2 * c2);
      dvec2* qt = reinterpret_cast<dvec2*>(th_out + d * ld + 2 * c2);
      if (NT) {
        __builtin_nontemporal_store(rn, qr);
        __builtin_nontemporal_store(tn, qt);
      } else {
        *qr = rn;
        *qt = tn;
      }
    }
  }
}

__global__ __launch_bounds__(KD_BLOCK) void k_kick_drift_s(
    const double* th_in, double* th_out, const double* rho_in, double* rho_out, i64 ld,
    const double* grad, i64 ldg_d, i64 ldg_c, const double* metric, double eps, int use_pre,
    double pre, int use_kick, double kick, i64 C, i64 D) {
  i64 c = (i64)blockIdx.x * KD_BLOCK + threadIdx.x;
  i64 d0 = (i64)blockIdx.y * KD_ROWS;
  if (c >= C) return;
  double t[KD_ROWS], r[KD_ROWS], g[KD_ROWS], m[KD_ROWS];
#pragma unroll
  for (int i = 0; i < KD_ROWS; ++i) {
    i64 d = d0 + i;
    if (d < D) {
      t[i] = th_in[d * ld + c];
      r[i] = rho_in[d * ld + c];
      g[i] = grad[d * ldg_d + c * ldg_c];
      m[i] = metric ? metric[d] : 1.0;
    }
  }
#pragma unroll
  for (int i = 0; i < KD_ROWS; ++i) {
    i64 d = d0 + i;
    if (d < D) {
      double rn;
      double tn = kd_elem(t[i], r[i], g[i], m[i], metric != nullptr, eps, use_pre, pre, use_kick, kick, rn);
      rho_out[d * ld + c] = rn;
      th_out[d * ld + c] = tn;
    }
  }
}

constexpr int TR_TILE = 64;
__global__ __launch_bounds__(256) void k_kick_drift_tr(
    const double* th_in, double* th_out, const double* rho_in, double* rho_out, i64 ld,
    const double* grad, i64 ldg_c, const double* metric, double eps, int use_pre, double pre,
    int use_kick, double kick, i64 C, i64 D) {
  __shared__ double tile[TR_TILE][TR_TILE + 1];
  i64 c0 = (i64)blockIdx.x * TR_TILE, d0 = (i64)blockIdx.y * TR_TILE;
  int tx = threadIdx.x & 63, ty = bk_wave_id();
#pragma unroll 4
  for (int i = 0; i < TR_TILE / 4; ++i) {
    int cl = ty + 4 * i;
    i64 c = c0 + cl, d = d0 + tx;
    tile[cl][tx] = (c < C && d < D) ? grad[c * ldg_c + d] : 0.0;
  }
  __syncthreads();
  i64 c = c0 + tx;
  if (c >= C) return;
#pragma unroll 4
  for (int i = 0; i < TR_TILE / 4; ++i) {
    int dl = ty + 4 * i;
    i64 d = d0 + dl;
    if (d < D) {
      double rn;
      double m = metric ? metric[d] : 1.0;
      double tn = kd_elem(th_in[d * ld + c], rho_in[d * ld + c], tile[tx][dl], m, metric != nullptr, eps,
                          use_pre, pre, use_kick, kick, rn);
      rho_out[d * ld + c] = rn;
      th_out[d * ld + c] = tn;
    }
  }
}

constexpr int PC_BLOCK = 64;
constexpr int RED_BLOCK_N = 4 * BK_WAVE;
constexpr int PC_UNROLL = 8;

__global__ __launch_bounds__(PC_BLOCK) void k_first_step_gather(
    const double* th_in, const double* rho_in, const double* g_in, i64 ld_in, const int32_t* idx,
    double* th_out, double* rho_out, i64 ld_out, const double* metric, double eps, double pre, i64 n,
    i64 D) {
  i64 j = (i64)blockIdx.x * PC_BLOCK + threadIdx.x;
  if (j >= n) return;
  i64 src = idx ? (i64)idx[j] : j;
  for (i64 d0 = 0; d0 < D; d0 += PC_UNROLL) {
    double t[PC_UNROLL], r[PC_UNROLL], g[PC_UNROLL];
#pragma unroll
    for (int u = 0; u < PC_UNROLL; ++u)
      if (d0 + u < D) {
        i64 o = (d0 + u) * ld_in + src;
        t[u] = th_in[o];
        r[u] = rho_in[o];
        g[u] = g_in[o];
      }
#pragma unroll
    for (int u = 0; u < PC_UNROLL; ++u)
      if (d0 + u < D) {
        double rn;
        double m = metric ? metric[d0 + u] : 1.0;
        double tn = kd_elem(t[u], r[u], g[u], m, metric != nullptr, eps, 1, pre, 0, 0.0, rn);
        i64 o = (d0 + u) * ld_out + j;
        rho_out[o] = rn;
        th_out[o] = tn;
      }
  }
}

constexpr int KN_U = 8;
__global__ __launch_bounds__(RED_BLOCK_N) void k_kick_drift_n(
    const double* th_in, const double* rho_in, const double* g_in, i64 ld_in, i64 ldg, const int32_t* idx,
    double* th_out, double* rho_out, i64 ld_out, const double* metric, double eps, int use_pre, double pre,
    int use_kick, double kick, i64 n_host, i64 D, const uint32_t* n_dev) {
  const i64 n = bk_lanes(n_host, n_dev);
  const i64 j0 = (i64)blockIdx.x * BK_WAVE;
  if (j0 >= n) return;
  const int lane = threadIdx.x & (BK_WAVE - 1), w = bk_wave_id();
  const i64 j = j0 + lane;
  if (j >= n) return;
  const i64 src = idx ? (i64)idx[j] : j;
  const i64 stride = (i64)4 * gridDim.y;
  for (i64 d0 = (i64)blockIdx.y * 4 + w; d0 < D; d0 += stride * KN_U) {
    double t[KN_U], r[KN_U], g[KN_U], m[KN_U];
#pragma unroll
    for (int u = 0; u < KN_U; ++u) {
      const i64 d = d0 + u * stride;
      if (d < D) {
        t[u] = th_in[d * ld_in + src];
        r[u] = rho_in[d * ld_in + src];
        g[u] = g_in[d * ldg + src];
        m[u] = metric ? metric[d] : 1.0;
      }
    }
#pragma unroll
    for (int u = 0; u < KN_U; ++u) {
      const i64 d = d0 + u * stride;
      if (d < D) {
        double rn;
        double tn = kd_elem(t[u], r[u], g[u], m[u], metric != nullptr, eps, use_pre, pre, use_kick, kick, rn);
        rho_out[d * ld_out + j] = rn;
        th_out[d * ld_out + j] = tn;
      }
    }
  }
}

constexpr int RED_WAVES = 4;
constexpr int RED_BLOCK = RED_WAVES * BK_WAVE;
constexpr int FIN_UNROLL = 8;

__device__ __forceinline__ double red_combine(double (&part)[RED_WAVES][BK_WAVE], int w, int lane, double p) {
  part[w][lane] = p;
  __syncthreads();
  double s = part[0][lane];
#pragma unroll
  for (int k = 1; k < RED_WAVES; ++k) s = s + part[k][lane];
  return s;
}

struct FinishLevel {
  const double* logp;
  double* H;
  double* h;
  uint8_t* live;
  uint32_t* lanes_out;
  unsigned long long* lanes_total;
};

template <bool KV>
__global__ __launch_bounds__(RED_BLOCK) void k_finish(const double* rho_in, double* rho_out, i64 ld,
                                                      const double* grad, i64 ldg_d, i64 ldg_c,
                                                      const double* metric, double half, int negate,
                                                      double* kin_out, i64 C_host, i64 D, const uint32_t* n_dev,
                                                      FinishLevel lv) {
  __shared__ double part[RED_WAVES][BK_WAVE];
  constexpr int PC_UNROLL = FIN_UNROLL;
  const int lane = threadIdx.x & (BK_WAVE - 1), w = bk_wave_id();
  const i64 C = bk_lanes(C_host, n_dev);
  if (blockIdx.x == 0 && threadIdx.x == 0) {
    if (lv.lanes_out) *lv.lanes_out = (uint32_t)C;
    if (lv.lanes_total) *lv.lanes_total += (unsigned long long)C;
  }
  if ((i64)blockIdx.x * BK_WAVE >= C) return;
  const i64 c = (i64)blockIdx.x * BK_WAVE + lane;
  const i64 Dq = (D + RED_WAVES - 1) / RED_WAVES;
  const i64 dlo = w * Dq, dhi = (dlo + Dq < D) ? dlo + Dq : D;
  double kin = 0.0;
  if (c < C) {
    for (i64 d0 = dlo; d0 < dhi; d0 += PC_UNROLL) {
      double r[PC_UNROLL], g[PC_UNROLL];
#pragma unroll
      for (int u = 0; u < PC_UNROLL; ++u)
        if (d0 + u < dhi) {
          r[u] = rho_in[(d0 + u) * ld + c];
          g[u] = grad ? grad[(d0 + u) * ldg_d + c * ldg_c] : 0.0;
        }
#pragma unroll
      for (int u = 0; u < PC_UNROLL; ++u)
        if (d0 + u < dhi) {
          double m = metric ? metric[d0 + u] : 1.0;
          double t = metric ? m * g[u] : g[u];
          double v = grad ? r[u] + half * t : r[u];
          if (negate) v = -v;
          if (rho_out) rho_out[(d0 + u) * ld + c] = v;
          double mv = KV ? metric[2 * D + d0 + u] * v : (metric ? m * v : v);
          kin = kin + v * mv;
        }
    }
  }
  if (!kin_out) return;
  double s = red_combine(part, w, lane, kin);
  if (w == 0 && c < C) {
    const double k = 0.5 * s;
    kin_out[c] = k;
    if (lv.H) {
      lv.H[c] = dr_joint(lv.logp[c], k);
      lv.h[c] = 0.0;
      lv.live[c] = 1;
    }
  }
}

template <bool KV>
__global__ __launch_bounds__(RED_BLOCK) void k_finish_v2(const double* rho_in, double* rho_out, i64 ld,
                                                         const double* grad, i64 ldg, const double* metric,
                                                         double half, int negate, double* kin_out, i64 C2, i64 D) {
  __shared__ dvec2 part[RED_WAVES][BK_WAVE];
  constexpr int U = FIN_UNROLL;
  const int lane = threadIdx.x & (BK_WAVE - 1), w = bk_wave_id();
  const i64 c2 = (i64)blockIdx.x * BK_WAVE + lane;
  const i64 Dq = (D + RED_WAVES - 1) / RED_WAVES;
  const i64 dlo = w * Dq, dhi = (dlo + Dq < D) ? dlo + Dq : D;
  dvec2 kin = {0.0, 0.0};
  if (c2 < C2) {
    for (i64 d0 = dlo; d0 < dhi; d0 += U) {
      dvec2 r[U], g[U];
#pragma unroll
      for (int u = 0; u < U; ++u)
        if (d0 + u < dhi) {
          r[u] = __builtin_nontemporal_load(reinterpret_cast<const dvec2*>(rho_in + (d0 + u) * ld + 2 * c2));
          if (grad) g[u] = __builtin_nontemporal_load(reinterpret_cast<const dvec2*>(grad + (d0 + u) * ldg + 2 * c2));
        }
#pragma unroll
      for (int u = 0; u < U; ++u)
        if (d0 + u < dhi) {
          const double m = metric ? metric[d0 + u] : 1.0;
          dvec2 v;
          {
            double t = metric ? m * g[u].x : g[u].x;
            v.x = grad ? r[u].x + half * t : r[u].x;
            t = metric ? m * g[u].y : g[u].y;
            v.y = grad ? r[u].y + half * t : r[u].y;
          }
          if (negate) {
            v.x = -v.x;
            v.y = -v.y;
          }
          if (rho_out) *reinterpret_cast<dvec2*>(rho_out + (d0 + u) * ld + 2 * c2) = v;
          const double km = KV ? metric[2 * D + d0 + u] : m;
          const double mx = metric ? km * v.x : v.x, my = metric ? km * v.y : v.y;
          kin.x = kin.x + v.x * mx;
          kin.y = kin.y + v.y * my;
        }
    }
  }
  if (!kin_out) return;
  part[w][lane] = kin;
  __syncthreads();
  if (w == 0 && c2 < C2) {
    dvec2 s = part[0][lane];
#pragma unroll
    for (int k = 1; k < RED_WAVES; ++k) {
      s.x = s.x + part[k][lane].x;
      s.y = s.y + part[k][lane].y;
    }
    s.x = 0.5 * s.x;
    s.y = 0.5 * s.y;
    *reinterpret_cast<dvec2*>(kin_out + 2 * c2) = s;
  }
}

__global__ __launch_bounds__(256) void k_mh_accept(int mode, double* lp_cur, const double* a_cur,
                                                   const double* lp_prop, const double* a_prop,
                                                   const double* log_u, uint8_t* mask, double* ret,
                                                   uint32_t* count, i64 C) {
  i64 c = (i64)blockIdx.x * 256 + threadIdx.x;
  bool acc = false;
  if (c < C) {
    double l0 = lp_cur[c], l1 = lp_prop[c];
    double a0 = a_cur ? a_cur[c] : 0.0, a1 = a_prop ? a_prop[c] : 0.0;
    double r0, r1;
    if (mode == BK_ACCEPT_HMC) {
      double h0 = l0 - a0, h1 = l1 - a1;
      acc = log_u[c] < h1 - h0;
      r0 = h0;
      r1 = h1;
    } else {
      acc = log_u[c] < (l1 - l0) + (a1 - a0);
      r0 = l0;
      r1 = l1;
    }
    if (mask) mask[c] = acc ? 1 : 0;
    if (ret) ret[c] = acc ? r1 : r0;
    if (acc) lp_cur[c] = l1;
  }
  if (count) {
    unsigned long long b = __ballot(acc);
    if ((threadIdx.x & (BK_WAVE - 1)) == 0 && b) atomicAdd(count, (uint32_t)__popcll(b));
  }
}

constexpr int SEL_ROWS = 2;
__global__ __launch_bounds__(256) void k_select(const uint8_t* mask, double* dst0, const double* src0,
                                                double* dst1, const double* src1, double* copy0, i64 ld,
                                                i64 C, i64 D) {
  i64 c = (i64)blockIdx.x * 256 + threadIdx.x;
  i64 d0 = (i64)blockIdx.y * SEL_ROWS;
  if (c >= C) return;
  const bool m = mask[c] != 0;
  if (!m && !copy0) return;
  double a[SEL_ROWS], b[SEL_ROWS];
#pragma unroll
  for (int i = 0; i < SEL_ROWS; ++i)
    if (d0 + i < D) {
      a[i] = m ? src0[(d0 + i) * ld + c] : dst0[(d0 + i) * ld + c];
      if (dst1 && m) b[i] = src1[(d0 + i) * ld + c];
    }
#pragma unroll
  for (int i = 0; i < SEL_ROWS; ++i)
    if (d0 + i < D) {
      if (m) dst0[(d0 + i) * ld + c] = a[i];
      if (dst1 && m) dst1[(d0 + i) * ld + c] = b[i];
      if (copy0) copy0[(d0 + i) * ld + c] = a[i];
    }
}

template <bool COPY>
__global__ __launch_bounds__(256) void k_select_v2(const uint8_t* mask, double* dst0, const double* src0,
                                                   double* dst1, const double* src1, double* copy0, i64 ld,
                                                   i64 C2, i64 D) {
  i64 c2 = (i64)blockIdx.x * 256 + threadIdx.x;
  i64 d0 = (i64)blockIdx.y * SEL_ROWS;
  if (c2 >= C2) return;
  const bool m0 = mask[2 * c2] != 0, m1 = mask[2 * c2 + 1] != 0;
  const bool any = m0 || m1, both = m0 && m1;
  dvec2 a[SEL_ROWS], b[SEL_ROWS];
#pragma unroll
  for (int i = 0; i < SEL_ROWS; ++i)
    if (d0 + i < D) {
      const i64 o = (d0 + i) * ld + 2 * c2;
      if (any) {
        a[i] = __builtin_nontemporal_load(reinterpret_cast<const dvec2*>(src0 + o));
        if (dst1) b[i] = __builtin_nontemporal_load(reinterpret_cast<const dvec2*>(src1 + o));
      }
      if (!both) {
        dvec2 old = __builtin_nontemporal_load(reinterpret_cast<const dvec2*>(dst0 + o));
        if (!m0) a[i].x = old.x;
        if (!m1) a[i].y = old.y;
        if (dst1) {
          old = __builtin_nontemporal_load(reinterpret_cast<const dvec2*>(dst1 + o));
          if (!m0) b[i].x = old.x;
          if (!m1) b[i].y = old.y;
        }
      }
    }
#pragma unroll
  for (int i = 0; i < SEL_ROWS; ++i)
    if (d0 + i < D) {
      const i64 o = (d0 + i) * ld + 2 * c2;
      __builtin_nontemporal_store(a[i], reinterpret_cast<dvec2*>(dst0 + o));
      if (dst1) __builtin_nontemporal_store(b[i], reinterpret_cast<dvec2*>(dst1 + o));
      if (COPY) __builtin_nontemporal_store(a[i], reinterpret_cast<dvec2*>(copy0 + o));
    }
}

__global__ __launch_bounds__(256) void k_blend(const uint8_t* mask, const double* a, const double* b, double* out,
                                               i64 ld, i64 C, i64 D) {
  i64 c = (i64)blockIdx.x * 256 + threadIdx.x;
  i64 d0 = (i64)blockIdx.y * SEL_ROWS;
  if (c >= C) return;
  const double* src = mask[c] ? b : a;
#pragma unroll
  for (int i = 0; i < SEL_ROWS; ++i)
    if (d0 + i < D) out[(d0 + i) * ld + c] = src[(d0 + i) * ld + c];
}

__global__ __launch_bounds__(256) void k_blend_v2(const uint8_t* mask, const double* a, const double* b,
                                                  double* out, i64 ld, i64 C2, i64 D) {
  i64 c2 = (i64)blockIdx.x * 256 + threadIdx.x;
  i64 d0 = (i64)blockIdx.y * SEL_ROWS;
  if (c2 >= C2) return;
  const bool m0 = mask[2 * c2] != 0, m1 = mask[2 * c2 + 1] != 0;
  dvec2 v[SEL_ROWS];
#pragma unroll
  for (int i = 0; i < SEL_ROWS; ++i)
    if (d0 + i < D) {
      const i64 o = (d0 + i) * ld + 2 * c2;
      if (m0 || m1) v[i] = __builtin_nontemporal_load(reinterpret_cast<const dvec2*>(b + o));
      if (!(m0 && m1)) {
        dvec2 old = __builtin_nontemporal_load(reinterpret_cast<const dvec2*>(a + o));
        if (!m0) v[i].x = old.x;
        if (!m1) v[i].y = old.y;
      }
    }
#pragma unroll
  for (int i = 0; i < SEL_ROWS; ++i)
    if (d0 + i < D)
      __builtin_nontemporal_store(v[i], reinterpret_cast<dvec2*>(out + (d0 + i) * ld + 2 * c2));
}

template <bool PC>
__global__ __launch_bounds__(RED_BLOCK) void k_mala_logq(const double* th, const double* g,
                                                         const double* thp, const double* gp, i64 ld,
                                                         double eps, double* fwd, double* rev, i64 C,
                                                         i64 D, const double* __restrict__ pc) {
  __shared__ double part_f[RED_WAVES][BK_WAVE];
  __shared__ double part_r[RED_WAVES][BK_WAVE];
  const int lane = threadIdx.x & (BK_WAVE - 1), w = bk_wave_id();
  const i64 c = (i64)blockIdx.x * BK_WAVE + lane;
  const i64 Dq = (D + RED_WAVES - 1) / RED_WAVES;
  const i64 dlo = w * Dq, dhi = (dlo + Dq < D) ? dlo + Dq : D;
  double sf = 0.0, sr = 0.0;
  constexpr int U = 4;
  if (c < C) {
    for (i64 d0 = dlo; d0 < dhi; d0 += U) {
      double a[U], b[U], p[U], q[U];
#pragma unroll
      for (int u = 0; u < U; ++u)
        if (d0 + u < dhi) {
          i64 o = (d0 + u) * ld + c;
          a[u] = th[o];
          b[u] = g[o];
          p[u] = thp[o];
          q[u] = gp[o];
        }
#pragma unroll
      for (int u = 0; u < U; ++u)
        if (d0 + u < dhi) {
          if (PC) {
            const double v = pc[d0 + u], iv = pc[2 * D + d0 + u];
            double xf = (p[u] - a[u]) - eps * (v * b[u]);
            double xr = (a[u] - p[u]) - eps * (v * q[u]);
            sf = sf + (xf * xf) * iv;
            sr = sr + (xr * xr) * iv;
          } else {
            double xf = (p[u] - a[u]) - eps * b[u];
            double xr = (a[u] - p[u]) - eps * q[u];
            sf = sf + xf * xf;
            sr = sr + xr * xr;
          }
        }
    }
  }
  double tf = red_combine(part_f, w, lane, sf);
  double tr = red_combine(part_r, w, lane, sr);
  if (w == 0 && c < C) {
    double k = -0.25 / eps;
    fwd[c] = k * tf;
    rev[c] = k * tr;
  }
}

__global__ __launch_bounds__(256) void k_relayout(const double* src, i64 s_d, i64 s_c, double* dst,
                                                  i64 t_d, i64 t_c, i64 C, i64 D) {
  __shared__ double tile[TR_TILE][TR_TILE + 1];
  i64 c0 = (i64)blockIdx.x * TR_TILE, d0 = (i64)blockIdx.y * TR_TILE;
  int tx = threadIdx.x & 63, ty = bk_wave_id();
  bool src_d_fast = (s_d == 1);
#pragma unroll 4
  for (int i = 0; i < TR_TILE / 4; ++i) {
    int slow = ty + 4 * i;
    int cl = src_d_fast ? slow : tx, dl = src_d_fast ? tx : slow;
    i64 c = c0 + cl, d = d0 + dl;
    if (c < C && d < D) tile[cl][dl] = src[d * s_d + c * s_c];
  }
  __syncthreads();
  bool dst_d_fast = (t_d == 1);
#pragma unroll 4
  for (int i = 0; i < TR_TILE / 4; ++i) {
    int slow = ty + 4 * i;
    int cl = dst_d_fast ? slow : tx, dl = dst_d_fast ? tx : slow;
    i64 c = c0 + cl, d = d0 + dl;
    if (c < C && d < D) dst[d * t_d + c * t_c] = tile[cl][dl];
  }
}

}

extern "C" {

int bk_leapfrog_kick_drift(const double* theta_in, double* theta_out, const double* rho_in,
                           double* rho_out, int64_t ld, const double* grad, int64_t ldg_d,
                           int64_t ldg_c, const double* metric, double eps, int use_pre, double pre,
                           int use_kick, double kick, int64_t C, int64_t D, void* stream) {
  if (!theta_in || !theta_out || !rho_in || !rho_out || !grad || C < 0 || D < 0) return BK_E_ARG;
  if (ld < C) return BK_E_ALIGN;
  if (C == 0 || D == 0) return BK_OK;
  hipStream_t s = bk_stream(stream);
  if (ldg_c == 1) {
    bool vec = (C % 2 == 0) && (ld % 2 == 0) && (ldg_d % 2 == 0) && bk_aligned16(theta_in) &&
               bk_aligned16(theta_out) && bk_aligned16(rho_in) && bk_aligned16(rho_out) &&
               bk_aligned16(grad);
    if (vec) {
      const i64 arrays = bk_distinct_arrays({theta_in, theta_out, rho_in, rho_out, grad});
#define BK_KD_LAUNCH(ROWS, NT)                                                                          \
  do {                                                                                                  \
    dim3 grid((unsigned)bk_cdiv(C / 2, KD_BLOCK), (unsigned)bk_cdiv(D, ROWS));                          \
    k_kick_drift_v2<ROWS, NT><<<grid, dim3(KD_BLOCK), 0, s>>>(theta_in, theta_out, rho_in, rho_out, ld, \
                                                              grad, ldg_d, metric, eps, use_pre, pre,   \
                                                              use_kick, kick, C / 2, D);                \
  } while (0)
      if (bk_streams_past_llc(arrays * C * D))
        BK_KD_LAUNCH(2, true);
      else if (D <= 65535)
        BK_KD_LAUNCH(1, false);
      else
        BK_KD_LAUNCH(2, false);
#undef BK_KD_LAUNCH
      BK_RETURN_LAUNCH_STATUS();
    }
  } else if (ldg_d == 1 && C >= TR_TILE / 2 && D >= TR_TILE / 2) {
    dim3 grid((unsigned)bk_cdiv(C, TR_TILE), (unsigned)bk_cdiv(D, TR_TILE));
    k_kick_drift_tr<<<grid, dim3(256), 0, s>>>(theta_in, theta_out, rho_in, rho_out, ld, grad, ldg_c, metric,
                                               eps, use_pre, pre, use_kick, kick, C, D);
    BK_RETURN_LAUNCH_STATUS();
  }
  dim3 grid((unsigned)bk_cdiv(C, KD_BLOCK), (unsigned)bk_cdiv(D, KD_ROWS));
  k_kick_drift_s<<<grid, dim3(KD_BLOCK), 0, s>>>(theta_in, theta_out, rho_in, rho_out, ld, grad, ldg_d, ldg_c,
                                                 metric, eps, use_pre, pre, use_kick, kick, C, D);
  BK_RETURN_LAUNCH_STATUS();
}

static unsigned kn_row_groups(i64 D) {
  i64 g = bk_cdiv(D, 4 * KN_U);
  return (unsigned)(g < 1 ? 1 : (g > 65535 ? 65535 : g));
}

int bk_leapfrog_kick_drift_n(const double* theta_in, double* theta_out, const double* rho_in, double* rho_out,
                             int64_t ld, const double* grad, int64_t ldg_d, int64_t ldg_c, const double* metric,
                             double eps, int use_pre, double pre, int use_kick, double kick, int64_t C, int64_t D,
                             const uint32_t* n_dev, void* stream) {
  if (!n_dev)
    return bk_leapfrog_kick_drift(theta_in, theta_out, rho_in, rho_out, ld, grad, ldg_d, ldg_c, metric, eps, use_pre,
                                  pre, use_kick, kick, C, D, stream);
  if (!theta_in || !theta_out || !rho_in || !rho_out || !grad || C < 0 || D < 0) return BK_E_ARG;
  if (ldg_c != 1 && C > 1) return BK_E_ARG;
  if (ld < C) return BK_E_ALIGN;
  if (C == 0 || D == 0) return BK_OK;
  dim3 grid((unsigned)bk_cdiv(C, BK_WAVE), kn_row_groups(D));
  k_kick_drift_n<<<grid, dim3(RED_BLOCK_N), 0, bk_stream(stream)>>>(theta_in, rho_in, grad, ld, ldg_d, nullptr, theta_out,
                                                                    rho_out, ld, metric, eps, use_pre, pre, use_kick,
                                                                    kick, C, D, n_dev);
  BK_RETURN_LAUNCH_STATUS();
}

int bk_leapfrog_first_step_gather(const double* theta_in, const double* rho_in, const double* grad_in,
                                    int64_t ld_in, const int32_t* src_index, double* theta_out, double* rho_out,
                                    int64_t ld_out, const double* metric, double eps, double pre, int64_t n,
                                    int64_t D, const uint32_t* n_dev, void* stream) {
  if (!theta_in || !rho_in || !grad_in || !theta_out || !rho_out || n < 0 || D < 0) return BK_E_ARG;
  if (ld_out < n) return BK_E_ALIGN;
  if (n == 0 || D == 0) return BK_OK;
  dim3 grid((unsigned)bk_cdiv(n, BK_WAVE), kn_row_groups(D));
  k_kick_drift_n<<<grid, dim3(RED_BLOCK_N), 0, bk_stream(stream)>>>(theta_in, rho_in, grad_in, ld_in, ld_in, src_index,
                                                                    theta_out, rho_out, ld_out, metric, eps, 1, pre, 0,
                                                                    0.0, n, D, n_dev);
  BK_RETURN_LAUNCH_STATUS();
}

}

__global__ __launch_bounds__(256) void k_precond_pack(const double* v, double* precond, i64 D) {
  const i64 d = (i64)blockIdx.x * 256 + threadIdx.x;
  if (d >= D) return;
  const double x = v[d];
  precond[d] = x;
  precond[D + d] = sqrt(x);
  precond[2 * D + d] = 1.0 / x;
}

template <bool KV>
static int finish_level(const double* rho_in, double* rho_out, int64_t ld, const double* grad, int64_t ldg_d,
                        int64_t ldg_c, const double* metric, double half, int negate, double* kin_out,
                        int64_t C, int64_t D, const uint32_t* n_dev, const double* logp, double* H_out,
                        double* h_out, uint8_t* live_out, uint32_t* lanes_out, uint64_t* lanes_total,
                        void* stream) {
  if (!rho_in || C < 0 || D < 0 || (KV && !metric)) return BK_E_ARG;
  if (H_out && (!logp || !h_out || !live_out || !kin_out)) return BK_E_ARG;
  if (ld < C) return BK_E_ALIGN;
  hipStream_t s = bk_stream(stream);
  if (C == 0) {
    if (lanes_out) return (int)hipMemsetAsync(lanes_out, 0, sizeof(uint32_t), s);
    return BK_OK;
  }
  FinishLevel lv = {logp, H_out, h_out, live_out, lanes_out, reinterpret_cast<unsigned long long*>(lanes_total)};
  const bool plain = !n_dev && !H_out && !lanes_out && !lanes_total;
  const bool vec = plain && C % 2 == 0 && ld % 2 == 0 && C * D >= ((i64)1 << 22) && bk_aligned16(rho_in) &&
                   (!rho_out || bk_aligned16(rho_out)) && (!kin_out || bk_aligned16(kin_out)) &&
                   (!grad || (ldg_c == 1 && ldg_d % 2 == 0 && bk_aligned16(grad)));
  if (vec)
    k_finish_v2<KV><<<dim3((unsigned)bk_cdiv(C / 2, BK_WAVE)), dim3(RED_BLOCK), 0, s>>>(
        rho_in, rho_out, ld, grad, ldg_d, metric, half, negate, kin_out, C / 2, D);
  else
    k_finish<KV><<<dim3((unsigned)bk_cdiv(C, BK_WAVE)), dim3(RED_BLOCK), 0, s>>>(
        rho_in, rho_out, ld, grad, ldg_d, ldg_c, metric, half, negate, kin_out, C, D, n_dev, lv);
  BK_RETURN_LAUNCH_STATUS();
}

extern "C" {

int bk_leapfrog_finish_level(const double* rho_in, double* rho_out, int64_t ld, const double* grad, int64_t ldg_d,
                             int64_t ldg_c, const double* metric, double half, int negate, double* kin_out,
                             int64_t C, int64_t D, const uint32_t* n_dev, const double* logp, double* H_out,
                             double* h_out, uint8_t* live_out, uint32_t* lanes_out, uint64_t* lanes_total,
                             void* stream) {
  return finish_level<false>(rho_in, rho_out, ld, grad, ldg_d, ldg_c, metric, half, negate, kin_out, C, D, n_dev, logp, H_out,
                             h_out, live_out, lanes_out, lanes_total, stream);
}

int bk_precond_pack(const double* v, double* precond, int64_t D, void* stream) {
  if (!v || !precond || D < 0) return BK_E_ARG;
  if (D == 0) return BK_OK;
  k_precond_pack<<<dim3((unsigned)bk_cdiv(D, 256)), dim3(256), 0, bk_stream(stream)>>>(v, precond, D);
  BK_RETURN_LAUNCH_STATUS();
}

int bk_leapfrog_finish_precond(const double* rho_in, double* rho_out, int64_t ld, const double* grad, int64_t ldg_d,
                               int64_t ldg_c, const double* precond, double half, int negate, double* kin_out, int64_t C,
                               int64_t D, void* stream) {
  return finish_level<true>(rho_in, rho_out, ld, grad, ldg_d, ldg_c, precond, half, negate, kin_out, C, D, nullptr, nullptr,
                            nullptr, nullptr, nullptr, nullptr, nullptr, stream);
}

int bk_leapfrog_finish(const double* rho_in, double* rho_out, int64_t ld, const double* grad,
                       int64_t ldg_d, int64_t ldg_c, const double* metric, double half, int negate,
                       double* kin_out, int64_t C, int64_t D, void* stream) {
  return bk_leapfrog_finish_level(rho_in, rho_out, ld, grad, ldg_d, ldg_c, metric, half, negate, kin_out, C, D,
                                  nullptr, nullptr, nullptr, nullptr, nullptr, nullptr, nullptr, stream);
}

int bk_mh_accept(int mode, double* lp_cur, const double* a_cur, const double* lp_prop,
                 const double* a_prop, const double* log_u, uint8_t* accept_mask, double* ret,
                 uint32_t* accept_count, int64_t C, void* stream) {
  if (!lp_cur || !lp_prop || !log_u || C < 0) return BK_E_ARG;
  if (mode != BK_ACCEPT_HMC && mode != BK_ACCEPT_MALA) return BK_E_ARG;
  if (C == 0) return BK_OK;
  k_mh_accept<<<dim3((unsigned)bk_cdiv(C, 256)), dim3(256), 0, bk_stream(stream)>>>(
      mode, lp_cur, a_cur, lp_prop, a_prop, log_u, accept_mask, ret, accept_count, C);
  BK_RETURN_LAUNCH_STATUS();
}

int bk_select_columns(const uint8_t* mask, double* dst0, const double* src0, double* dst1,
                      const double* src1, double* copy0, int64_t ld, int64_t C, int64_t D, void* stream) {
  if (!mask || !dst0 || !src0 || (dst1 && !src1) || C < 0 || D < 0) return BK_E_ARG;
  if (ld < C) return BK_E_ALIGN;
  if (C == 0 || D == 0) return BK_OK;
  hipStream_t s = bk_stream(stream);
  if (C % 2 == 0 && ld % 2 == 0 && bk_aligned16(dst0) && bk_aligned16(src0) &&
      (!dst1 || (bk_aligned16(dst1) && bk_aligned16(src1))) && (!copy0 || bk_aligned16(copy0))) {
    dim3 grid((unsigned)bk_cdiv(C / 2, 256), (unsigned)bk_cdiv(D, SEL_ROWS));
    if (copy0)
      k_select_v2<true><<<grid, dim3(256), 0, s>>>(mask, dst0, src0, dst1, src1, copy0, ld, C / 2, D);
    else
      k_select_v2<false><<<grid, dim3(256), 0, s>>>(mask, dst0, src0, dst1, src1, nullptr, ld, C / 2, D);
  } else {
    dim3 grid((unsigned)bk_cdiv(C, 256), (unsigned)bk_cdiv(D, SEL_ROWS));
    k_select<<<grid, dim3(256), 0, s>>>(mask, dst0, src0, dst1, src1, copy0, ld, C, D);
  }
  BK_RETURN_LAUNCH_STATUS();
}

int bk_blend_columns(const uint8_t* mask, const double* a, const double* b, double* out, int64_t ld, int64_t C,
                     int64_t D, void* stream) {
  if (!mask || !a || !b || !out || C < 0 || D < 0) return BK_E_ARG;
  if (ld < C) return BK_E_ALIGN;
  if (C == 0 || D == 0) return BK_OK;
  hipStream_t s = bk_stream(stream);
  if (C % 2 == 0 && ld % 2 == 0 && bk_aligned16(a) && bk_aligned16(b) && bk_aligned16(out)) {
    dim3 grid((unsigned)bk_cdiv(C / 2, 256), (unsigned)bk_cdiv(D, SEL_ROWS));
    k_blend_v2<<<grid, dim3(256), 0, s>>>(mask, a, b, out, ld, C / 2, D);
  } else {
    dim3 grid((unsigned)bk_cdiv(C, 256), (unsigned)bk_cdiv(D, SEL_ROWS));
    k_blend<<<grid, dim3(256), 0, s>>>(mask, a, b, out, ld, C, D);
  }
  BK_RETURN_LAUNCH_STATUS();
}

int bk_mala_logq(const double* theta, const double* grad, const double* theta_prop,
                 const double* grad_prop, int64_t ld, double eps, double* lp_forward,
                 double* lp_reverse, int64_t C, int64_t D, void* stream) {
  if (!theta || !grad || !theta_prop || !grad_prop || !lp_forward || !lp_reverse || C < 0 || D < 0)
    return BK_E_ARG;
  if (ld < C) return BK_E_ALIGN;
  if (C == 0) return BK_OK;
  k_mala_logq<false><<<dim3((unsigned)bk_cdiv(C, BK_WAVE)), dim3(RED_BLOCK), 0, bk_stream(stream)>>>(
      theta, grad, theta_prop, grad_prop, ld, eps, lp_forward, lp_reverse, C, D, nullptr);
  BK_RETURN_LAUNCH_STATUS();
}

int bk_mala_logq_precond(const double* theta, const double* grad, const double* theta_prop,
                         const double* grad_prop, int64_t ld, const double* precond, double eps,
                         double* lp_forward, double* lp_reverse, int64_t C, int64_t D, void* stream) {
  if (!theta || !grad || !theta_prop || !grad_prop || !precond || !lp_forward || !lp_reverse || C < 0 || D < 0)
    return BK_E_ARG;
  if (ld < C) return BK_E_ALIGN;
  if (C == 0 || D == 0) return BK_OK;
  k_mala_logq<true><<<dim3((unsigned)bk_cdiv(C, BK_WAVE)), dim3(RED_BLOCK), 0, bk_stream(stream)>>>(
      theta, grad, theta_prop, grad_prop, ld, eps, lp_forward, lp_reverse, C, D, precond);
  BK_RETURN_LAUNCH_STATUS();
}

int bk_relayout(const double* src, int64_t lds_d, int64_t lds_c, double* dst, int64_t ldd_d,
                int64_t ldd_c, int64_t C, int64_t D, void* stream) {
  if (!src || !dst || C < 0 || D < 0) return BK_E_ARG;
  if (C == 0 || D == 0) return BK_OK;
  dim3 grid((unsigned)bk_cdiv(C, TR_TILE), (unsigned)bk_cdiv(D, TR_TILE));
  k_relayout<<<grid, dim3(256), 0, bk_stream(stream)>>>(src, lds_d, lds_c, dst, ldd_d, ldd_c, C, D);
  BK_RETURN_LAUNCH_STATUS();
}

}
```

### bayes-kit_amd/csrc/bk_targets.hip

```cpp
#include "bk_common.hpp"
#include "bk_elementwise.hpp"
#include "bk_mala_step.hpp"
#include "bk_lanes.hpp"

namespace {

constexpr int TG_ROWS = 4;
constexpr int TG_BLOCK = 256;

typedef double dvec2 __attribute__((ext_vector_type(2)));

template <int ROWS, bool NT>
__global__ __launch_bounds__(TG_BLOCK) void k_gauss_grad_v2(const double* th, double* g, i64 ld,
                                                            const double* lam, i64 C2, i64 D) {
  i64 c2 = (i64)blockIdx.x * TG_BLOCK + threadIdx.x;
  i64 d0 = (i64)blockIdx.y * ROWS;
  if (c2 >= C2) return;
  dvec2 t[ROWS];
  double l[ROWS];
#pragma unroll
  for (int i = 0; i < ROWS; ++i)
    if (d0 + i < D) {
      const dvec2* p = reinterpret_cast<const dvec2*>(th + (d0 + i) * ld + 2 * c2);
      t[i] = NT ? __builtin_nontemporal_load(p) : *p;
      l[i] = lam ? lam[d0 + i] : 1.0;
    }
#pragma unroll
  for (int i = 0; i < ROWS; ++i)
    if (d0 + i < D) {
      dvec2 o;
      o.x = lam ? -(l[i] * t[i].x) : -t[i].x;
      o.y = lam ? -(l[i] * t[i].y) : -t[i].y;
      dvec2* q = reinterpret_cast<dvec2*>(g + (d0 + i) * ld + 2 * c2);
      if (NT) __builtin_nontemporal_store(o, q);
      else *q = o;
    }
}

__global__ __launch_bounds__(TG_BLOCK) void k_gauss_grad_s(const double* th, double* g, i64 ld,
                                                           const double* lam, i64 C_host, i64 D,
                                                           const uint32_t* n_dev) {
  const i64 C = bk_lanes(C_host, n_dev);
  i64 c = (i64)blockIdx.x * TG_BLOCK + threadIdx.x;
  i64 d0 = (i64)blockIdx.y * TG_ROWS;
  if (c >= C) return;
#pragma unroll
  for (int i = 0; i < TG_ROWS; ++i)
    if (d0 + i < D) {
      double t = th[(d0 + i) * ld + c];
      g[(d0 + i) * ld + c] = lam ? -(lam[d0 + i] * t) : -t;
    }
}

constexpr int RED_WAVES = 4;
constexpr int RED_BLOCK = RED_WAVES * BK_WAVE;
__global__ __launch_bounds__(RED_BLOCK) void k_gauss_logp(const double* th, double* g, double* logp, i64 ld,
                                                          const double* lam, i64 C_host, i64 D,
                                                          const uint32_t* n_dev) {
  __shared__ double part[RED_WAVES][BK_WAVE];
  constexpr int PC_UNROLL = 8;
  const int lane = threadIdx.x & (BK_WAVE - 1), w = bk_wave_id();
  const i64 C = bk_lanes(C_host, n_dev);
  if ((i64)blockIdx.x * BK_WAVE >= C) return;
  const i64 c = (i64)blockIdx.x * BK_WAVE + lane;
  const i64 Dq = (D + RED_WAVES - 1) / RED_WAVES;
  const i64 dlo = w * Dq, dhi = (dlo + Dq < D) ? dlo + Dq : D;
  double s = 0.0;
  if (c < C) {
    for (i64 d0 = dlo; d0 < dhi; d0 += PC_UNROLL) {
      double t[PC_UNROLL];
#pragma unroll
      for (int u = 0; u < PC_UNROLL; ++u)
        if (d0 + u < dhi) t[u] = th[(d0 + u) * ld + c];
#pragma unroll
      for (int u = 0; u < PC_UNROLL; ++u)
        if (d0 + u < dhi) {
          double lt = lam ? lam[d0 + u] * t[u] : t[u];
          s = s + t[u] * lt;
          if (g) g[(d0 + u) * ld + c] = -lt;
        }
    }
  }
  part[w][lane] = s;
  __syncthreads();
  if (w == 0 && c < C) {
    double tot = part[0][lane];
#pragma unroll
    for (int k = 1; k < RED_WAVES; ++k) tot = tot + part[k][lane];
    logp[c] = -0.5 * tot;
  }
}

__global__ __launch_bounds__(RED_BLOCK) void k_gauss_logp_v2(const double* th, double* g, double* logp, i64 ld,
                                                             const double* lam, i64 C2, i64 D) {
  __shared__ dvec2 part[RED_WAVES][BK_WAVE];
  constexpr int U = 8;
  const int lane = threadIdx.x & (BK_WAVE - 1), w = bk_wave_id();
  const i64 c2 = (i64)blockIdx.x * BK_WAVE + lane;
  const i64 Dq = (D + RED_WAVES - 1) / RED_WAVES;
  const i64 dlo = w * Dq, dhi = (dlo + Dq < D) ? dlo + Dq : D;
  dvec2 s = {0.0, 0.0};
  if (c2 < C2) {
    for (i64 d0 = dlo; d0 < dhi; d0 += U) {
      dvec2 t[U];
#pragma unroll
      for (int u = 0; u < U; ++u)
        if (d0 + u < dhi) t[u] = __builtin_nontemporal_load(reinterpret_cast<const dvec2*>(th + (d0 + u) * ld + 2 * c2));
#pragma unroll
      for (int u = 0; u < U; ++u)
        if (d0 + u < dhi) {
          const double l = lam ? lam[d0 + u] : 1.0;
          const double lx = lam ? l * t[u].x : t[u].x, ly = lam ? l * t[u].y : t[u].y;
          s.x = s.x + t[u].x * lx;
          s.y = s.y + t[u].y * ly;
          if (g) {
            dvec2 o = {-lx, -ly};
            __builtin_nontemporal_store(o, reinterpret_cast<dvec2*>(g + (d0 + u) * ld + 2 * c2));
          }
        }
    }
  }
  part[w][lane] = s;
  __syncthreads();
  if (w == 0 && c2 < C2) {
    dvec2 tot = part[0][lane];
#pragma unroll
    for (int k = 1; k < RED_WAVES; ++k) {
      tot.x = tot.x + part[k][lane].x;
      tot.y = tot.y + part[k][lane].y;
    }
    tot.x = -0.5 * tot.x;
    tot.y = -0.5 * tot.y;
    *reinterpret_cast<dvec2*>(logp + 2 * c2) = tot;
  }
}

template <bool HL>
struct GaussTerm {
  __device__ __forceinline__ static void eval(double th, i64 d, const double* lam, double& term, double& grad) {
    const double lt = HL ? lam[d] * th : th;
    term = th * lt;
    grad = -lt;
  }
  __device__ __forceinline__ static double finish(double s) { return -0.5 * s; }
};

struct FunnelDensity {
  static constexpr int HEAD = 1;
  template <class L>
  __device__ __forceinline__ static double eval(L& c, const double*) {
    const double v = c.head(0);
    const double s = c.sum([](double x, i64) { return x * x; });
    const double ev = bk_exp(-v);
    const double hn = 0.5 * (double)(c.dims() - 1);
    const double he = 0.5 * ev;
    c.grad_head(0, ((-v / 9.0) - hn) + he * s);
    c.grad([ev](double x, i64) { return -(ev * x); });
    return ((-(v * v) / 18.0) - hn * v) - he * s;
  }
};

int gauss(const double* theta, double* grad, double* logp, i64 ld, const double* lam, i64 C, i64 D,
          const uint32_t* n_dev, void* stream) {
  if (!theta || (!grad && !logp) || C < 0 || D < 0) return BK_E_ARG;
  if (ld < C) return BK_E_ALIGN;
  if (C == 0) return BK_OK;
  hipStream_t s = bk_stream(stream);
  if (n_dev) {
    if (logp)
      k_gauss_logp<<<dim3((unsigned)bk_cdiv(C, BK_WAVE)), dim3(RED_BLOCK), 0, s>>>(theta, grad, logp, ld, lam, C, D, n_dev);
    else if (D > 0)
      k_gauss_grad_s<<<dim3((unsigned)bk_cdiv(C, TG_BLOCK), (unsigned)bk_cdiv(D, TG_ROWS)), dim3(TG_BLOCK), 0, s>>>(
          theta, grad, ld, lam, C, D, n_dev);
    BK_RETURN_LAUNCH_STATUS();
  }
  if (logp) {
    if (C % 2 == 0 && ld % 2 == 0 && C * D >= ((i64)1 << 22) && bk_aligned16(theta) && bk_aligned16(logp) &&
        (!grad || bk_aligned16(grad)))
      k_gauss_logp_v2<<<dim3((unsigned)bk_cdiv(C / 2, BK_WAVE)), dim3(RED_BLOCK), 0, s>>>(theta, grad, logp, ld, lam,
                                                                                          C / 2, D);
    else
      k_gauss_logp<<<dim3((unsigned)bk_cdiv(C, BK_WAVE)), dim3(RED_BLOCK), 0, s>>>(theta, grad, logp, ld, lam, C, D,
                                                                                   nullptr);
    BK_RETURN_LAUNCH_STATUS();
  }
  if (D == 0) return BK_OK;
  if (C % 2 == 0 && ld % 2 == 0 && bk_aligned16(theta) && bk_aligned16(grad)) {
    const bool streams = bk_streams_past_llc(bk_distinct_arrays({theta, grad}) * C * D);
    if (D <= 65535) {
      dim3 grid((unsigned)bk_cdiv(C / 2, TG_BLOCK), (unsigned)D);
      if (streams) k_gauss_grad_v2<1, true><<<grid, dim3(TG_BLOCK), 0, s>>>(theta, grad, ld, lam, C / 2, D);
      else k_gauss_grad_v2<1, false><<<grid, dim3(TG_BLOCK), 0, s>>>(theta, grad, ld, lam, C / 2, D);
    } else {
      dim3 grid((unsigned)bk_cdiv(C / 2, TG_BLOCK), (unsigned)bk_cdiv(D, 2));
      k_gauss_grad_v2<2, false><<<grid, dim3(TG_BLOCK), 0, s>>>(theta, grad, ld, lam, C / 2, D);
    }
  } else {
    dim3 grid((unsigned)bk_cdiv(C, TG_BLOCK), (unsigned)bk_cdiv(D, TG_ROWS));
    k_gauss_grad_s<<<grid, dim3(TG_BLOCK), 0, s>>>(theta, grad, ld, lam, C, D, nullptr);
  }
  BK_RETURN_LAUNCH_STATUS();
}

}

extern "C" {

int bk_target_iso_gaussian_grad(const double* theta, double* grad, double* logp, int64_t ld, int64_t C,
                                int64_t D, void* stream) {
  return gauss(theta, grad, logp, ld, nullptr, C, D, nullptr, stream);
}

int bk_target_diag_gaussian_grad(const double* theta, double* grad, double* logp, int64_t ld,
                                 const double* lam, int64_t C, int64_t D, void* stream) {
  if (!lam) return BK_E_ARG;
  return gauss(theta, grad, logp, ld, lam, C, D, nullptr, stream);
}

int bk_target_iso_gaussian_grad_n(const double* theta, double* grad, double* logp, int64_t ld, int64_t C,
                                  int64_t D, const uint32_t* n_dev, void* stream) {
  return gauss(theta, grad, logp, ld, nullptr, C, D, n_dev, stream);
}

int bk_target_diag_gaussian_grad_n(const double* theta, double* grad, double* logp, int64_t ld,
                                   const double* lam, int64_t C, int64_t D, const uint32_t* n_dev, void* stream) {
  if (!lam) return BK_E_ARG;
  return gauss(theta, grad, logp, ld, lam, C, D, n_dev, stream);
}

int bk_hmc_trajectory_gaussian(const double* theta_in, double* theta_out, const double* rho_in,
                               double* rho_out, int64_t ld, const double* lam, const double* metric,
                               double eps, int64_t steps, int64_t C, int64_t D, void* stream) {
  if (lam)
    return bke::hmc_trajectory_launch<GaussTerm<true>>(theta_in, theta_out, rho_in, rho_out, ld, lam, metric, eps, steps, C, D,
                                                       stream);
  return bke::hmc_trajectory_launch<GaussTerm<false>>(theta_in, theta_out, rho_in, rho_out, ld, lam, metric, eps, steps, C, D,
                                                      stream);
}

int bk_hmc_draw_gaussian(const double* theta_in, double* theta_out, int64_t ld, const double* rho_in,
                         const double* zt, int64_t ldz, const double* lam, const double* metric, double eps,
                         int64_t steps, double* part, double* kin0, double* kin1, double* lp_out, double* lp_cur,
                         const double* log_u, uint8_t* accept_mask, double* ret, uint32_t* accept_count, int64_t C,
                         int64_t D, void* stream) {
  if (lam)
    return bke::hmc_draw_launch<GaussTerm<true>>(theta_in, theta_out, ld, rho_in, zt, ldz, lam, metric, eps, steps, part, kin0,
                                                 kin1, lp_out, lp_cur, log_u, accept_mask, ret, accept_count, C, D, stream);
  return bke::hmc_draw_launch<GaussTerm<false>>(theta_in, theta_out, ld, rho_in, zt, ldz, lam, metric, eps, steps, part, kin0,
                                                kin1, lp_out, lp_cur, log_u, accept_mask, ret, accept_count, C, D, stream);
}

int bk_hmc_draw_gaussian_precond(const double* theta_in, double* theta_out, int64_t ld, const double* rho_in,
                                 const double* zt, int64_t ldz, const double* lam, const double* precond, double eps,
                                 int64_t steps, double* part, double* kin0, double* kin1, double* lp_out, double* lp_cur,
                                 const double* log_u, uint8_t* accept_mask, double* ret, uint32_t* accept_count, int64_t C,
                                 int64_t D, void* stream) {
  if (lam)
    return bke::hmc_draw_launch<GaussTerm<true>, true>(theta_in, theta_out, ld, rho_in, zt, ldz, lam, precond, eps, steps, part,
                                                       kin0, kin1, lp_out, lp_cur, log_u, accept_mask, ret, accept_count, C, D,
                                                       stream);
  return bke::hmc_draw_launch<GaussTerm<false>, true>(theta_in, theta_out, ld, rho_in, zt, ldz, lam, precond, eps, steps, part,
                                                      kin0, kin1, lp_out, lp_cur, log_u, accept_mask, ret, accept_count, C, D,
                                                      stream);
}

int bk_mala_step_gaussian(const double* theta, double* theta_out, double* theta_prop, int64_t ld, const double* lam,
                          double* lp, const double* lp_prop, const double* log_u, const double* zt_next, int64_t ldz,
                          double eps, double sqrt2eps, uint8_t* accept_mask, double* ret, uint32_t* accept_count, int64_t C,
                          int64_t D, void* stream) {
  if (lam)
    return bkm::mala_step_sep_launch<GaussTerm<true>>(theta, theta_out, theta_prop, ld, lam, lp, lp_prop, log_u, zt_next, ldz, eps,
                                                      sqrt2eps, accept_mask, ret, accept_count, C, D, stream);
  return bkm::mala_step_sep_launch<GaussTerm<false>>(theta, theta_out, theta_prop, ld, lam, lp, lp_prop, log_u, zt_next, ldz, eps,
                                                     sqrt2eps, accept_mask, ret, accept_count, C, D, stream);
}

int bk_mala_step_gaussian_precond(const double* theta, double* theta_out, double* theta_prop, int64_t ld, const double* lam,
                                  const double* precond, double* lp, const double* lp_prop, const double* log_u,
                                  const double* zt_next, int64_t ldz, double eps, double sqrt2eps, uint8_t* accept_mask,
                                  double* ret, uint32_t* accept_count, int64_t C, int64_t D, void* stream) {
  if (lam)
    return bkm::mala_step_sep_launch<GaussTerm<true>, true>(theta, theta_out, theta_prop, ld, lam, lp, lp_prop, log_u, zt_next,
                                                            ldz, eps, sqrt2eps, accept_mask, ret, accept_count, C, D, stream,
                                                            precond);
  return bkm::mala_step_sep_launch<GaussTerm<false>, true>(theta, theta_out, theta_prop, ld, lam, lp, lp_prop, log_u, zt_next,
                                                           ldz, eps, sqrt2eps, accept_mask, ret, accept_count, C, D, stream,
                                                           precond);
}

int bk_target_funnel_grad_n(const double* theta, double* grad, double* logp, int64_t ld, int64_t C,
                            int64_t D, const uint32_t* n_dev, void* stream) {
  return bkl::target_launch<FunnelDensity>(theta, grad, logp, ld, nullptr, C, D, n_dev, stream);
}

int bk_target_funnel_grad(const double* theta, double* grad, double* logp, int64_t ld, int64_t C,
                          int64_t D, void* stream) {
  return bkl::target_launch<FunnelDensity>(theta, grad, logp, ld, nullptr, C, D, nullptr, stream);
}

int bk_leapfrog_step_funnel(double* theta, double* rho, int64_t ld, const double* metric, double h, int64_t n, int64_t D,
                            const uint32_t* n_dev, void* stream) {
  return bkl::step_launch<FunnelDensity>(theta, rho, ld, metric, h, nullptr, n, D, n_dev, stream);
}

int bk_hmc_trajectory_funnel(const double* theta_in, double* rho, const double* grad_in, double* theta_out, double* grad_out,
                             double* logp_out, double* kin_out, int64_t ld, const double* metric, double eps, int64_t steps,
                             int64_t C, int64_t D, void* stream) {
  return bkl::hmc_trajectory_launch<FunnelDensity>(theta_in, rho, grad_in, ld, theta_out, grad_out, logp_out, kin_out, ld, metric,
                                                   eps, steps, C, D, nullptr, stream);
}

int bk_dr_proposal_funnel(const double* theta_in, const double* rho_in, const double* grad_in, int64_t ld_in,
                              const int32_t* src_index, double* theta_out, double* rho_out, double* grad_out,
                              double* logp_out, double* kin_out, int64_t ld_out, const double* metric, double h,
                              int64_t steps, int64_t n, int64_t D, const uint32_t* n_dev, uint32_t* lanes_out,
                              uint64_t* lanes_total, double* H_out, double* h_out, uint8_t* live_out,
                              const bk_scatter_job* job_in, const bk_ghost_link* ghost_in, const bk_ghost0* g0_in,
                              void* stream) {
  return bkl::dr_proposal_launch<FunnelDensity>(theta_in, rho_in, grad_in, ld_in, src_index, theta_out, rho_out, grad_out,
                                                logp_out, kin_out, ld_out, metric, h, steps, n, D, n_dev, lanes_out,
                                                lanes_total, H_out, h_out, live_out, job_in, ghost_in, g0_in, nullptr, stream);
}

}
```

### include/bkhip.h

```cpp
#ifndef BKHIP_H
#define BKHIP_H

#include <stdint.h>

#ifdef __cplusplus
extern "C" {
#endif

#define BK_OK 0
#define BK_E_ARG (-1)
#define BK_E_ALIGN (-2)

#define BK_RNG_WORDS 11
#define BK_RNG_PHILOX 0
#define BK_RNG_PCG64 1

int bk_version(void);

int bk_rng_init_philox(uint64_t* state, int64_t ldr, uint64_t key0, uint64_t chain_id0,
                       int64_t C, void* stream);

int64_t bk_refresh_work_elems(int64_t C, int64_t D);
int bk_momentum_refresh(int rng_kind, uint64_t* state, int64_t ldr,
                        const double* loc_in, double loc_mul, double scale,
                        double* out, int64_t ld, const double* metric, double* kin_out,
                        const uint8_t* active, int64_t C, int64_t D, double* work,
                        int64_t work_elems, void* stream);

int bk_momentum_refresh_precond(int rng_kind, uint64_t* state, int64_t ldr, double* out, int64_t ld,
                                const double* precond, double* kin_out, int64_t C, int64_t D, double* work,
                                int64_t work_elems, void* stream);

typedef struct bk_diag_job {
  const double* theta;
  int64_t ld_theta;
  int64_t C, D;
  const int64_t* n_dev;
  double* mean;
  double* m2;
  int64_t ld;
  int64_t n_offset;
  double* series;
  const int32_t* dims;
  int64_t K;
  const double* logp;
  int64_t capacity;
  int64_t row_offset;
} bk_diag_job;
int bk_dr_refresh_begin(int rng_kind, uint64_t* state, int64_t ldr, const double* loc_in, double loc_mul,
                        double scale, double* out, int64_t ld, const double* metric, double* kin_out, int64_t C,
                        int64_t D, double* work, int64_t work_elems, const double* logp, double* cur_H,
                        double* cur_h, double* rej, uint8_t* alive, double prob_retry, uint32_t* counters,
                        int64_t n_counters, int64_t* draw_counter, const bk_diag_job* side, void* stream);

int bk_log_uniform(int rng_kind, uint64_t* state, int64_t ldr, double* out,
                   const uint8_t* active, int64_t C, void* stream);

int bk_uniform(int rng_kind, uint64_t* state, int64_t ldr, double* out, const uint8_t* active,
               int64_t C, void* stream);

int bk_leapfrog_kick_drift(const double* theta_in, double* theta_out,
                           const double* rho_in, double* rho_out, int64_t ld,
                           const double* grad, int64_t ldg_d, int64_t ldg_c,
                           const double* metric, double eps,
                           int use_pre, double pre, int use_kick, double kick,
                           int64_t C, int64_t D, void* stream);

int bk_leapfrog_first_step_gather(const double* theta_in, const double* rho_in, const double* grad_in,
                                  int64_t ld_in, const int32_t* src_index, double* theta_out,
                                  double* rho_out, int64_t ld_out, const double* metric, double eps,
                                  double pre, int64_t n, int64_t D, const uint32_t* n_dev, void* stream);

int bk_leapfrog_finish(const double* rho_in, double* rho_out, int64_t ld,
                       const double* grad, int64_t ldg_d, int64_t ldg_c,
                       const double* metric, double half, int negate,
                       double* kin_out, int64_t C, int64_t D, void* stream);

int bk_precond_pack(const double* v, double* precond, int64_t D, void* stream);

int bk_leapfrog_finish_precond(const double* rho_in, double* rho_out, int64_t ld, const double* grad, int64_t ldg_d,
                               int64_t ldg_c, const double* precond, double half, int negate, double* kin_out,
                               int64_t C, int64_t D, void* stream);

int bk_leapfrog_kick_drift_n(const double* theta_in, double* theta_out, const double* rho_in, double* rho_out,
                             int64_t ld, const double* grad, int64_t ldg_d, int64_t ldg_c,
                             const double* metric, double eps, int use_pre, double pre, int use_kick,
                             double kick, int64_t C, int64_t D, const uint32_t* n_dev, void* stream);
int bk_leapfrog_finish_level(const double* rho_in, double* rho_out, int64_t ld, const double* grad,
                             int64_t ldg_d, int64_t ldg_c, const double* metric, double half, int negate,
                             double* kin_out, int64_t C, int64_t D, const uint32_t* n_dev,
                             const double* logp, double* H_out, double* h_out, uint8_t* live_out,
                             uint32_t* lanes_out, uint64_t* lanes_total, void* stream);

#define BK_ACCEPT_HMC 0
#define BK_ACCEPT_MALA 1
int bk_mh_accept(int mode, double* lp_cur, const double* a_cur, const double* lp_prop,
                 const double* a_prop, const double* log_u, uint8_t* accept_mask,
                 double* ret, uint32_t* accept_count, int64_t C, void* stream);

int bk_select_columns(const uint8_t* mask, double* dst0, const double* src0,
                      double* dst1, const double* src1, double* copy0, int64_t ld,
                      int64_t C, int64_t D, void* stream);

int bk_blend_columns(const uint8_t* mask, const double* a, const double* b, double* out,
                     int64_t ld, int64_t C, int64_t D, void* stream);


int bk_compact_indices(const uint8_t* mask, int64_t n, int32_t* idx_out, uint32_t* count_out,
                       const uint32_t* n_dev, void* stream);

int bk_dr_begin(const double* logp, const double* kin, double* cur_H, double* cur_h, double* rej,
                uint8_t* alive, int64_t C, void* stream);

int bk_dr_retry_test(int rng_kind, uint64_t* state, int64_t ldr, const double* rej,
                     double prob_retry, uint8_t* alive, int64_t C, void* stream);

int bk_dr_level_begin(const double* logp, const double* kin, double* H, double* h, uint8_t* live,
                      int64_t n, const uint32_t* n_dev, void* stream);

int bk_dr_ghost_update(const double* ga, const int32_t* sub_index, int64_t m, double* h,
                       uint8_t* live, double* a, const uint32_t* n_dev, void* stream);

int bk_dr_accept_prob(const double* H, const double* cur_H, const double* h, const double* cur_h,
                      const int32_t* cur_index, double prob_retry, const uint8_t* live, double* a,
                      int64_t n, const uint32_t* n_dev, void* stream);

int bk_dr_accept_test(int rng_kind, uint64_t* state, int64_t ldr, const int32_t* chain_index,
                      const double* a, const double* H, int64_t n, double* cur_H, double* cur_h,
                      double* rej, uint8_t* alive, uint8_t* accepted, const uint32_t* n_dev,
                      void* stream);

int bk_dr_accept_prob_test(int rng_kind, uint64_t* state, int64_t ldr, const int32_t* chain_index,
                           const double* H, const double* h, const uint8_t* live, double* a,
                           double prob_retry, int64_t n, double* cur_H, double* cur_h, double* rej,
                           uint8_t* alive, uint8_t* accepted, const uint32_t* n_dev, void* stream);

int bk_dr_begin_retry(int rng_kind, uint64_t* state, int64_t ldr, const double* logp, const double* kin,
                      double* cur_H, double* cur_h, double* rej, uint8_t* alive, double prob_retry,
                      uint32_t* counters, int64_t n_counters, int64_t* draw_counter, int64_t C, void* stream);

int bk_dr_accept_prob_test_next(int rng_kind, uint64_t* state, int64_t ldr, const int32_t* chain_index,
                                const double* H, const double* h, const uint8_t* live, double* a,
                                double prob_retry, int64_t n, double* cur_H, double* cur_h, double* rej,
                                uint8_t* alive, uint8_t* accepted, const uint32_t* n_dev, int32_t* next_index,
                                uint32_t* next_count, void* stream);

int bk_dr_accept_prob_ghost_next(const double* H, const double* parent_H, const double* h, double* parent_h,
                                 const int32_t* sub_index, double prob_retry, const uint8_t* live, double* a,
                                 int64_t n, const uint32_t* n_dev, uint8_t* parent_live, double* parent_a,
                                 int32_t* next_index, uint32_t* next_count, void* stream);

int bk_dr_accept_prob_ghost(const double* H, const double* parent_H, const double* h, double* parent_h,
                            const int32_t* sub_index, double prob_retry, const uint8_t* live, double* a,
                            int64_t n, const uint32_t* n_dev, uint8_t* parent_live, double* parent_a,
                            void* stream);

int bk_scatter_columns(const uint8_t* mask, const int32_t* index, int64_t n, int64_t D,
                       double* dst0, const double* src0, double* dst1, const double* src1,
                       double* dst2, const double* src2, int64_t ld_dst, int64_t ld_src,
                       double* sdst, const double* ssrc, const uint32_t* n_dev, void* stream);

int bk_mala_propose(int rng_kind, uint64_t* state, int64_t ldr, const double* theta,
                    const double* grad, double* theta_prop, int64_t ld, double eps,
                    double sqrt2eps, int64_t C, int64_t D, void* stream);

int bk_mala_propose_from_normals(const double* theta, const double* grad, const double* z,
                                 int64_t z_stride_d, int64_t z_stride_c, double* theta_prop,
                                 int64_t ld, double eps, double sqrt2eps, int64_t C, int64_t D,
                                 void* stream);

int bk_mala_propose_from_normals_precond(const double* theta, const double* grad, const double* z,
                                         int64_t z_stride_d, int64_t z_stride_c, const double* precond,
                                         double* theta_prop, int64_t ld, double eps, double sqrt2eps,
                                         int64_t C, int64_t D, void* stream);

int bk_normals_chain_major(int rng_kind, uint64_t* state, int64_t ldr, double* zt, int64_t ldz, int64_t C,
                           int64_t D, uint64_t* snapshot, int64_t max_workgroups, void* stream);

int bk_mala_single_draw(int rng_kind, uint64_t* state, int64_t ldr, double* theta, double* grad, double* lp,
                        double* theta_prop, const double* host_in, double* host_out, uint64_t* snapshot,
                        int64_t lds, uint8_t* accept_mask, uint32_t* accept_count, double eps, double sqrt2eps,
                        int64_t D, int have_prop, double seq, void* stream);

int bk_mala_logq(const double* theta, const double* grad, const double* theta_prop,
                 const double* grad_prop, int64_t ld, double eps, double* lp_forward,
                 double* lp_reverse, int64_t C, int64_t D, void* stream);

int bk_mala_logq_precond(const double* theta, const double* grad, const double* theta_prop,
                         const double* grad_prop, int64_t ld, const double* precond, double eps,
                         double* lp_forward, double* lp_reverse, int64_t C, int64_t D, void* stream);

int bk_mala_step_supported(int64_t C, int64_t D, int64_t ld);
int bk_mala_step(const double* theta, double* theta_out, double* grad, double* theta_prop,
                 const double* grad_prop, int64_t ld, double* lp, const double* lp_prop,
                 const double* log_u, const double* zt_next, int64_t ldz, double eps,
                 double sqrt2eps, uint8_t* accept_mask, double* ret, uint32_t* accept_count,
                 int64_t C, int64_t D, void* stream);

int bk_mala_step_precond(const double* theta, double* theta_out, double* grad, double* theta_prop,
                         const double* grad_prop, int64_t ld, const double* precond, double* lp,
                         const double* lp_prop, const double* log_u, const double* zt_next, int64_t ldz,
                         double eps, double sqrt2eps, uint8_t* accept_mask, double* ret,
                         uint32_t* accept_count, int64_t C, int64_t D, void* stream);

int bk_target_iso_gaussian_grad(const double* theta, double* grad, double* logp, int64_t ld,
                                int64_t C, int64_t D, void* stream);
int bk_target_diag_gaussian_grad(const double* theta, double* grad, double* logp, int64_t ld,
                                 const double* lam, int64_t C, int64_t D, void* stream);
int bk_target_funnel_grad(const double* theta, double* grad, double* logp, int64_t ld,
                          int64_t C, int64_t D, void* stream);

int bk_target_iso_gaussian_grad_n(const double* theta, double* grad, double* logp, int64_t ld,
                                  int64_t C, int64_t D, const uint32_t* n_dev, void* stream);
int bk_target_diag_gaussian_grad_n(const double* theta, double* grad, double* logp, int64_t ld,
                                   const double* lam, int64_t C, int64_t D, const uint32_t* n_dev,
                                   void* stream);
int bk_target_funnel_grad_n(const double* theta, double* grad, double* logp, int64_t ld,
                            int64_t C, int64_t D, const uint32_t* n_dev, void* stream);

int bk_leapfrog_step_funnel(double* theta, double* rho, int64_t ld, const double* metric, double h, int64_t n,
                            int64_t D, const uint32_t* n_dev, void* stream);

int bk_hmc_trajectory_funnel(const double* theta_in, double* rho, const double* grad_in, double* theta_out,
                             double* grad_out, double* logp_out, double* kin_out, int64_t ld,
                             const double* metric, double eps, int64_t steps, int64_t C, int64_t D, void* stream);

typedef int (*bk_target_fn)(const double* theta, double* grad, double* logp, int64_t ld,
                            const void* params, int64_t C, int64_t D, void* stream);

typedef int (*bk_target_fn_n)(const double* theta, double* grad, double* logp, int64_t ld,
                              const void* params, int64_t C, int64_t D, const uint32_t* n_dev,
                              void* stream);

int bk_hmc_trajectory_gaussian(const double* theta_in, double* theta_out, const double* rho_in,
                               double* rho_out, int64_t ld, const double* lam, const double* metric,
                               double eps, int64_t steps, int64_t C, int64_t D, void* stream);

int bk_hmc_draw_gaussian(const double* theta_in, double* theta_out, int64_t ld, const double* rho_in,
                         const double* zt, int64_t ldz, const double* lam, const double* metric,
                         double eps, int64_t steps, double* part, double* kin0, double* kin1,
                         double* lp_out, double* lp_cur, const double* log_u, uint8_t* accept_mask,
                         double* ret, uint32_t* accept_count, int64_t C, int64_t D, void* stream);

int bk_hmc_draw_gaussian_precond(const double* theta_in, double* theta_out, int64_t ld, const double* rho_in,
                                 const double* zt, int64_t ldz, const double* lam, const double* precond, double eps,
                                 int64_t steps, double* part, double* kin0, double* kin1, double* lp_out,
                                 double* lp_cur, const double* log_u, uint8_t* accept_mask, double* ret,
                                 uint32_t* accept_count, int64_t C, int64_t D, void* stream);

int bk_mala_step_gaussian(const double* theta, double* theta_out, double* theta_prop, int64_t ld, const double* lam,
                          double* lp, const double* lp_prop, const double* log_u, const double* zt_next, int64_t ldz,
                          double eps, double sqrt2eps, uint8_t* accept_mask, double* ret, uint32_t* accept_count, int64_t C,
                          int64_t D, void* stream);

int bk_mala_step_gaussian_precond(const double* theta, double* theta_out, double* theta_prop, int64_t ld, const double* lam,
                                  const double* precond, double* lp, const double* lp_prop, const double* log_u,
                                  const double* zt_next, int64_t ldz, double eps, double sqrt2eps, uint8_t* accept_mask,
                                  double* ret, uint32_t* accept_count, int64_t C, int64_t D, void* stream);


typedef struct bk_scatter_job {
  const uint8_t* mask;
  const int32_t* index;
  int64_t n, D;
  double* dst0; const double* src0;
  double* dst1; const double* src1;
  double* dst2; const double* src2;
  int64_t ld_dst, ld_src;
  double* sdst; const double* ssrc;
  const uint32_t* n_dev;
} bk_scatter_job;

typedef struct bk_ghost_link {
  const double* parent_H;
  double* parent_h;
  uint8_t* parent_live;
  double* parent_a;
  double* a_out;
  double prob_retry;
  int32_t* next_index;
  uint32_t* next_count;
} bk_ghost_link;

typedef struct bk_ghost0 {
  double h;
  int64_t steps;
  double* parent_a;
  double prob_retry;
  int32_t* next_index;
  uint32_t* next_count;
  uint32_t* lanes_out;
  uint64_t* lanes_total;
} bk_ghost0;

int bk_dr_proposal_funnel(const double* theta_in, const double* rho_in, const double* grad_in,
                          int64_t ld_in, const int32_t* src_index, double* theta_out,
                          double* rho_out, double* grad_out, double* logp_out, double* kin_out,
                          int64_t ld_out, const double* metric, double h, int64_t steps, int64_t n,
                          int64_t D, const uint32_t* n_dev, uint32_t* lanes_out, uint64_t* lanes_total,
                          double* H_out, double* h_out, uint8_t* live_out, const bk_scatter_job* job,
                              const bk_ghost_link* ghost, const bk_ghost0* ghost0, void* stream);

int bk_dr_proposal_gaussian(const double* theta_in, const double* rho_in, const double* grad_in,
                                int64_t ld_in, const int32_t* src_index, double* theta_out,
                                double* rho_out, double* grad_out, double* logp_out, double* kin_out,
                                int64_t ld_out, const double* metric, double h, int64_t steps, int64_t n,
                                int64_t D, const uint32_t* n_dev, uint32_t* lanes_out, uint64_t* lanes_total,
                                double* H_out, double* h_out, uint8_t* live_out, const bk_scatter_job* job,
                                const bk_ghost_link* ghost, const bk_ghost0* ghost0, const double* lam,
                                void* stream);
int bk_leapfrog_step_gaussian(double* theta, double* rho, int64_t ld, const double* lam, const double* metric,
                              double h, int64_t n, int64_t D, const uint32_t* n_dev, void* stream);

int bk_dense_metric_apply(const double* M, int64_t ldm, const double* X, double* Y, int64_t ld,
                          int64_t C, int64_t D, void* stream);

int64_t bk_gemm_chains_work_elems(int64_t R, int64_t K, int64_t C);
int bk_gemm_chains(const double* A, int64_t lda, int64_t R, int64_t K, const double* X, int64_t ldx,
                   double* Y, int64_t ldy, int64_t C, double* work, int64_t work_elems, void* stream);

int bk_gemm_chains_logistic(const double* A, int64_t lda, int64_t R, int64_t K, const double* X, int64_t ldx,
                            double* Y, int64_t ldy, int64_t C, const double* y_rows, void* stream);

int bk_logistic_residual(double* Z, int64_t ldz, const double* y, double* part, int64_t N, int64_t C,
                         int64_t segments, void* stream);
int bk_logistic_finish(const double* G, const double* theta, int64_t ld, const double* part,
                       int64_t segments, double inv_prior_var, double t, double* grad, double* logp,
                       double* loglik, int64_t C, int64_t D, void* stream);

int bk_dot_columns(const double* x, const double* y, int64_t ld, double scale, double* out,
                   int64_t C, int64_t D, void* stream);

int bk_resample_indices(const double* weights, int64_t n, const double* u, int64_t m,
                        double* cdf_work, int32_t* idx_out, void* stream);

int bk_gather_columns(const int32_t* index, const double* src, int64_t ld_src, double* dst,
                      int64_t ld_dst, int64_t m, int64_t D, void* stream);

int bk_relayout(const double* src, int64_t lds_d, int64_t lds_c, double* dst, int64_t ldd_d,
                int64_t ldd_c, int64_t C, int64_t D, void* stream);

int bk_welford_update(double* mean, double* m2, int64_t ld, const double* theta, int64_t ld_theta,
                      int64_t n, int64_t C, int64_t D, void* stream);
int bk_welford_update_dev(double* mean, double* m2, int64_t ld, const double* theta, int64_t ld_theta,
                          const int64_t* n_dev, int64_t n_offset, int64_t C, int64_t D, void* stream);

int bk_record_series(const double* theta, int64_t ld, const int32_t* dims, int64_t K, const double* logp,
                     double* series, int64_t capacity, int64_t row, int64_t C, void* stream);

int bk_record_series_dev(const double* theta, int64_t ld, const int32_t* dims, int64_t K, const double* logp,
                         double* series, int64_t capacity, const int64_t* row_dev, int64_t row_offset, int64_t C,
                         void* stream);

int bk_rhat_partials(const double* mean, const double* m2, int64_t ld, int64_t n,
                     const double* center, double* out, int64_t C, int64_t D, void* stream);

int bk_accept_stat(const double* lp_cur, const double* a_cur, const double* lp_prop, const double* a_prop, int64_t C,
                   double* out, double* work, void* stream);

int bk_chain_mean_var(const double* x, int64_t ld, const int32_t* len, int64_t N,
                      double* mean, double* var, int64_t C, void* stream);

int bk_rank_normalize(const double* rank, double S, double* out, int64_t n, void* stream);

int64_t bk_sort_by_key_work_bytes(int64_t n);
int bk_sort_by_key(const double* keys_in, double* keys_out, const int64_t* vals_in, int64_t* vals_out,
                   int64_t n, void* work, int64_t work_bytes, void* stream);
int bk_count_below(const double* sorted_keys, int64_t n, const double* queries, int64_t m, int64_t* out,
                   void* stream);
int bk_scatter_ranks(const int64_t* payload, int64_t n, double base, double* out, void* stream);

int bk_autocorr(const double* x, int64_t ld, int64_t N, double* out, int64_t ldo, int64_t C,
                void* stream);

int64_t bk_autocorr_fft_work_bytes(int64_t N, int64_t C);
int bk_autocorr_fft(const double* x, int64_t ld, int64_t N, double* out, int64_t ldo, int64_t C, void* work,
                    int64_t work_bytes, void* stream);

int bk_iat_from_acor(const double* acor, int64_t ld, int64_t N, int estimator, double* ess_out,
                     double* iat_out, int64_t C, void* stream);

int bk_end_pos_pairs(const double* acor, int64_t ld, int64_t N, int64_t* out, int64_t C,
                     void* stream);

int bk_ess(const double* x, int64_t ld, int64_t N, int estimator, double* ess_out,
           double* iat_out, int64_t C, void* stream);

int64_t bk_ess_multi_work_bytes(int64_t n, int64_t C, int64_t nlags);
int bk_ess_split_moments(const double* x, int64_t ld, int64_t N, int64_t C, int indicator, double q, double* chain_mean,
                         double* chain_g0, double* out, void* work, int64_t work_bytes, void* stream);
int bk_ess_between_sq(const double* chain_mean, int64_t M, const double* centre, double* out, void* work,
                      int64_t work_bytes, void* stream);
int64_t bk_ess_lag_sums_max_half(void);
int bk_ess_lag_sums(const double* x, int64_t ld, int64_t N, int64_t C, int indicator, double q, const double* chain_mean,
                    int64_t lag0, int64_t nlags, double* out, void* work, int64_t work_bytes, void* stream);
int bk_ess_acov_sums(const double* acor, int64_t ldo, int64_t n, int64_t C, const double* chain_g0, int64_t lag0,
                     int64_t nlags, double* out, void* work, int64_t work_bytes, void* stream);
int bk_ess_indicator(const double* x, int64_t ld, int64_t n, int64_t C, double q, double* out, int64_t ldo, void* stream);
int bk_select_ranks(const double* rank, const double* values, int64_t n, const double* targets, int64_t k, double* out,
                    void* stream);

int bk_host_normals(int rng_kind, uint64_t* state_words , double* out,
                    int64_t n);
int bk_host_uniforms(int rng_kind, uint64_t* state_words, double* out, int64_t n);
double bk_host_log1p(double x);
double bk_host_exp(double x);

#ifdef __cplusplus
}
#endif
#endif
```

Measured before the change: 111.8 million leapfrog steps/sec.

## Store proposal theta/grad tile-major and run whole trajectory per chain tile

When chains are tiled, the proposal position and gradient buffers are laid out tile-major, so each 8192-chain tile is a contiguous dense block with its own leading dimension. The full L-step trajectory, finish, MH accept and column select then run per tile, using new leading-dimension-aware kick-drift/select/blend kernels with non-temporal hints. A tiled reduction kernel is added for the finish step when the data fits in the LLC. The intent is to keep each tile's working set cache-resident and contiguous instead of touching strided slices of full-width arrays. In exchange it adds layout-conversion logic through property accessors, which assemble a copy on read and can cost extra when used.

```diff
diff --git a/bayes-kit_amd/bayes_kit_amd/_lib.py b/bayes-kit_amd/bayes_kit_amd/_lib.py
--- a/bayes-kit_amd/bayes_kit_amd/_lib.py
+++ b/bayes-kit_amd/bayes_kit_amd/_lib.py
@@ -36,6 +36,9 @@
     "bk_mh_accept": [c_int, P, P, P, P, P, P, P, P, I, P],
     "bk_select_columns": [P, P, P, P, P, P, I, I, I, P],
     "bk_blend_columns": [P, P, P, P, I, I, I, P],
+    "bk_leapfrog_kick_drift_ld": [P, I, P, I, P, I, P, I, P, I, I, P, F, c_int, F, c_int, F, I, I, P],
+    "bk_blend_columns_ld": [P, P, I, P, I, P, I, I, I, P],
+    "bk_select_columns_ld": [P, P, I, P, I, I, I, P],
     "bk_compact_indices": [P, I, P, P, P, P],
     "bk_dr_begin": [P, P, P, P, P, P, I, P],
     "bk_dr_retry_test": [c_int, P, I, P, F, P, I, P],
@@ -311,6 +314,13 @@
                        ptr(grad), grad.stride(0), grad.stride(1), ptr(metric), eps, int(use_pre), pre,
                        int(use_kick), kick, C, D, ptr(n_dev), self._s())
 
+    def kick_drift_ld(self, theta_in, theta_out, rho_in, rho_out, grad, metric, eps, use_pre, pre, use_kick, kick):
+        D, C = theta_out.shape
+        assert theta_in.shape == (D, C) and rho_in.shape == (D, C) and rho_out.shape == (D, C) and grad.shape == (D, C)
+        self._call("bk_leapfrog_kick_drift_ld", ptr(theta_in), _ld(theta_in), ptr(theta_out), _ld(theta_out), ptr(rho_in),
+                   _ld(rho_in), ptr(rho_out), _ld(rho_out), ptr(grad), grad.stride(0), grad.stride(1), ptr(metric), eps,
+                   int(use_pre), pre, int(use_kick), kick, C, D, self._s())
+
     def first_step_gather(self, theta_in, rho_in, grad_in, src_index, theta_out, rho_out, metric, eps, pre,
                           n_dev=None):
         D, n = theta_out.shape
@@ -374,6 +384,16 @@
         ld = _ld(a)
         assert _ld(b) == ld and _ld(out) == ld
         self._call("bk_blend_columns", ptr(mask), ptr(a), ptr(b), ptr(out), ld, C, D, self._s())
+
+    def blend_columns_ld(self, mask, a, b, out):
+        D, C = out.shape
+        assert a.shape == (D, C) and b.shape == (D, C) and mask.shape[0] == C
+        self._call("bk_blend_columns_ld", ptr(mask), ptr(a), _ld(a), ptr(b), _ld(b), ptr(out), _ld(out), C, D, self._s())
+
+    def select_columns_ld(self, mask, dst, src):
+        D, C = dst.shape
+        assert src.shape == (D, C) and mask.shape[0] == C
+        self._call("bk_select_columns_ld", ptr(mask), ptr(dst), _ld(dst), ptr(src), _ld(src), C, D, self._s())
 
     def compact_indices(self, mask, n, idx_out, count_out, n_dev=None):
         self._call("bk_compact_indices", ptr(mask), n, ptr(idx_out), ptr(count_out), ptr(n_dev), self._s())
diff --git a/bayes-kit_amd/bayes_kit_amd/hmc.py b/bayes-kit_amd/bayes_kit_amd/hmc.py
--- a/bayes-kit_amd/bayes_kit_amd/hmc.py
+++ b/bayes-kit_amd/bayes_kit_amd/hmc.py
@@ -74,6 +74,7 @@
         self._logu_bufs = [torch.empty(C, **f64)]
         self._ret = torch.empty(C, **f64)
         self._mask = torch.empty(C, dtype=torch.uint8, device=dev)
+        self._rho_tile = torch.empty(D * self._chain_tile, **f64) if self._chain_tile < C else None
         self._accepted = torch.zeros(1, dtype=torch.int32, device=dev)
         if self._fused_draw:
             self._part = torch.empty(12 * C, **f64)
@@ -176,7 +177,7 @@
             self._rng_state.copy_(self._snap[self._pf_slot] if self._snap is not None else self._rng_logical)
             self._pf_ready, self._pf_event = False, None
         self._fused_draw = self._fused = self._fused_zt = False
-        self._rho_bufs = [r if r is not None else torch.empty_like(self._theta_p) for r in self._rho_bufs]
+        self._rho_bufs = [r if r is not None else torch.empty_like(self._thp_raw) for r in self._rho_bufs]
         if self._prefetch and self._snap is not None:
             self._snap, self._rng_logical = None, self._rng_state.clone()
         self._have_cache = False
@@ -207,6 +208,78 @@
         key = "step_ms" if builtin else "kick_drift_ms"
         self.placement = {key + "_as_allocated": rep["ms_as_allocated"], key + "_chosen": rep["ms_chosen"],
                           "assignments_tried": rep["assignments_tried"]}
+
+    _tm_last = False
+
+    @staticmethod
+    def tile_major_blocks(C, D, T):
+        return [(c0, min(C, c0 + T), D * c0) for c0 in range(0, C, T)]
+
+    def _tm_assemble(self, raw):
+        D, C = self._dim, self._C
+        flat, out = raw.view(-1), torch.empty((D, C), dtype=raw.dtype, device=raw.device)
+        for c0, c1, off in self.tile_major_blocks(C, D, self._chain_tile):
+            out[:, c0:c1].copy_(flat[off:off + D * (c1 - c0)].view(D, c1 - c0))
+        return out
+
+    @property
+    def _theta_p(self):
+        return self._tm_assemble(self._thp_raw) if self._tm_last else self._thp_raw
+
+    @_theta_p.setter
+    def _theta_p(self, a):
+        self._thp_raw = a
+
+    @property
+    def _grad_p(self):
+        return self._tm_assemble(self._gp_raw) if self._tm_last else self._gp_raw
+
+    @_grad_p.setter
+    def _grad_p(self, a):
+        self._gp_raw = a
+
+    def _tm_flat(self, name):
+        a = getattr(self, name)
+        if not a.is_contiguous() or a.numel() != self._dim * self._C:
+            a = torch.empty((self._dim, self._C), dtype=a.dtype, device=a.device)
+            setattr(self, name, a)
+        return a.view(-1)
+
+    def _draw_tile_major(self, th, rho, kin0, logu, g, m, eps, half, L):
+        ops, D, C, T = self._ops, self._dim, self._C, self._chain_tile
+        thp_f, gp_f = self._tm_flat("_thp_raw"), self._tm_flat("_gp_raw")
+        if self._rho_tile is None or self._rho_tile.numel() != D * T:
+            self._rho_tile = torch.empty(D * T, dtype=torch.float64, device=ops.device)
+        lp0 = self._lp.clone() if self._stat is not None else None
+        self._out = torch.empty_like(th) if self._rebind else None
+        for c0, c1, off in self.tile_major_blocks(C, D, T):
+            n, sl = c1 - c0, slice(c0, c1)
+            thp_k, gp_k = thp_f[off:off + D * n].view(D, n), gp_f[off:off + D * n].view(D, n)
+            rho_k = self._rho_tile[:D * n].view(D, n)
+            gl = None
+            for s in range(L):
+                if s == 0:
+                    ops.kick_drift_ld(th[:, sl], thp_k, rho[:, sl], rho_k, g[:, sl], m, eps, True, -half, True, eps)
+                else:
+                    ops.kick_drift(thp_k, thp_k, rho_k, rho_k, gl, m, eps, False, 0.0, True, eps)
+                gl = self._eval_grad(thp_k, gp_k, self._lp_p[sl] if s == L - 1 else None)
+            gl = self._materialize(gl, gp_k)
+            if self._pd is not None:
+                ops.leapfrog_finish_precond(rho_k, None, gl, self._pd, half, False, self._kin1[sl])
+            else:
+                ops.leapfrog_finish(rho_k, None, gl, m, half, False, self._kin1[sl])
+            ops.mh_accept(_lib.ACCEPT_HMC, self._lp[sl], kin0[sl], self._lp_p[sl], self._kin1[sl], logu[sl],
+                          self._mask[sl], self._ret[sl], self._accepted)
+            if self._rebind:
+                ops.blend_columns_ld(self._mask[sl], th[:, sl], thp_k, self._out[:, sl])
+            else:
+                ops.select_columns_ld(self._mask[sl], th[:, sl], thp_k)
+            ops.select_columns_ld(self._mask[sl], self._grad[:, sl], gp_k)
+        if lp0 is not None:
+            ops.accept_stat(lp0, kin0, self._lp_p, self._kin1, self._stat, self._stat_work)
+        if self._rebind:
+            self._theta_dc = self._out
+        self._tm_last = True
 
     LLC_BYTES = 192 << 20
     MIN_TILE = 8192
@@ -317,8 +390,8 @@
     def _materialize_dense(self, g):
         if g.dim() == 2 and g.stride(1) == 1:
             return g
-        self._ops.relayout(g, self._grad_p)
-        return self._grad_p
+        self._ops.relayout(g, self._gp_raw)
+        return self._gp_raw
 
     def _current_randomness(self):
         self._zt_slot = 0 if not self._prefetch else self._pf_slot
@@ -418,8 +491,9 @@
         ops = self._ops
         eps, L, m = float(self._stepsize), int(self._steps), self._metric_dev
         half = 0.5 * eps
-        th, thp = self._theta_dc, self._theta_p
+        th, thp, gp_raw = self._theta_dc, self._thp_raw, self._gp_raw
         mirror = not self._batched
+        self._tm_last = False
 
         rho, kin0, logu = self._current_randomness()
         self._start_next_randomness()
@@ -447,9 +521,9 @@
             if not self._have_cache:
                 self._materialize(self._eval_grad(th, self._grad, self._lp), self._grad)
                 self._have_cache = True
-            if self._model.bk_hmc_proposal(th, rho, self._grad, thp, self._grad_p, self._lp_p, self._kin1, m, eps, L):
+            if self._model.bk_hmc_proposal(th, rho, self._grad, thp, gp_raw, self._lp_p, self._kin1, m, eps, L):
                 self._accept(kin0, logu)
-                self._take(th, thp, self._grad, self._grad_p)
+                self._take(th, thp, self._grad, gp_raw)
                 return
 
         if mirror:
@@ -469,10 +543,14 @@
             if not mirror:
                 self._lp_p.copy_(self._lp)
         elif (self._traj_hook and not mirror and self._chain_tile >= self._C
-              and self._model.bk_leapfrog_trajectory(th, rho, g, None, thp, rho, self._grad_p, self._lp_p, m, eps, L,
+              and self._model.bk_leapfrog_trajectory(th, rho, g, None, thp, rho, gp_raw, self._lp_p, m, eps, L,
                                                      hmc_first=True)):
             self._grad_calls += L
-            g_last = self._grad_p
+            g_last = gp_raw
+        elif (self._chain_tile < self._C and not mirror and self._M is None and not self._step_hook
+              and hasattr(ops, "kick_drift_ld")):
+            self._draw_tile_major(th, rho, kin0, logu, g, m, eps, half, L)
+            return
         else:
             g_last = None
             T = self._chain_tile
@@ -480,7 +558,7 @@
                 c1 = min(self._C, c0 + T)
                 tile = (c0, c1) != (0, self._C)
                 v = (lambda a: a[:, c0:c1]) if tile else (lambda a: a)
-                th_t, thp_t, rho_t, gp_t, g_t = v(th), v(thp), v(rho), v(self._grad_p), v(g)
+                th_t, thp_t, rho_t, gp_t, g_t = v(th), v(thp), v(rho), v(gp_raw), v(g)
                 lp_t = self._lp_p[c0:c1] if tile else self._lp_p
                 gl = None
                 for n in range(L):
@@ -498,7 +576,7 @@
                     gl = self._eval_grad(thp_t, gp_t, want_lp)
                 if tile:
                     self._materialize(gl, gp_t)
-                    g_last = self._grad_p
+                    g_last = gp_raw
                 else:
                     g_last = gl
         if self._pd is not None:
@@ -514,7 +592,7 @@
         if mirror:
             self._select(self._mask, th, thp)
         else:
-            gp = self._materialize(g_last, self._grad_p) if L > 0 else None
+            gp = self._materialize(g_last, gp_raw) if L > 0 else None
             self._take(th, thp, self._grad if gp is not None else None, gp)
 
     def _accept(self, kin0, logu):
diff --git a/bayes-kit_amd/build.py b/bayes-kit_amd/build.py
--- a/bayes-kit_amd/build.py
+++ b/bayes-kit_amd/build.py
@@ -10,7 +10,7 @@
 OBJ_DIR = os.path.join(HERE, "build")
 LIB = os.path.join(OUT_DIR, "libbkhip.so")
 SOURCES = ["bk_rng.hip", "bk_integrator.hip", "bk_targets.hip", "bk_targets_gauss_lanes.hip", "bk_diag.hip", "bk_dr.hip", "bk_dense.hip", "bk_smc.hip", "bk_mala.hip", "bk_sort.hip", "bk_fft.hip", "bk_ess_multi.hip"]
-HEADERS = ["bk_common.hpp", "bk_ess_tile.hpp", "bk_rng.hpp", "bk_lanes.hpp", "bk_elementwise.hpp", "bk_mala_step.hpp", "ziggurat_tables.inc", os.path.join("..", "..", "include", "bkhip.h"),
+HEADERS = ["bk_common.hpp", "bk_ess_tile.hpp", "bk_rng.hpp", "bk_lanes.hpp", "bk_elementwise.hpp", "bk_mala_step.hpp", "bk_tile_kernels.hpp", "ziggurat_tables.inc", os.path.join("..", "..", "include", "bkhip.h"),
            os.path.join("..", "..", "include", "bkhip_math.h")]
 FLAGS = ["--offload-arch=gfx950", "-O3", "-std=c++17", "-fPIC", "-ffp-contract=off", "-fno-fast-math",
          "-Wall", "-Wno-unused-function"]
diff --git a/bayes-kit_amd/csrc/bk_integrator.hip b/bayes-kit_amd/csrc/bk_integrator.hip
--- a/bayes-kit_amd/csrc/bk_integrator.hip
+++ b/bayes-kit_amd/csrc/bk_integrator.hip
@@ -1,4 +1,5 @@
 #include "bk_common.hpp"
+#include "bk_tile_kernels.hpp"
 
 namespace {
 
@@ -638,6 +639,8 @@
   precond[2 * D + d] = 1.0 / x;
 }
 
+constexpr int BK_RED_T_CP = 8, BK_RED_T_U = 8;
+
 template <bool KV>
 static int finish_level(const double* rho_in, double* rho_out, int64_t ld, const double* grad, int64_t ldg_d,
                         int64_t ldg_c, const double* metric, double half, int negate, double* kin_out,
@@ -657,7 +660,10 @@
   const bool vec = plain && C % 2 == 0 && ld % 2 == 0 && C * D >= ((i64)1 << 22) && bk_aligned16(rho_in) &&
                    (!rho_out || bk_aligned16(rho_out)) && (!kin_out || bk_aligned16(kin_out)) &&
                    (!grad || (ldg_c == 1 && ldg_d % 2 == 0 && bk_aligned16(grad)));
-  if (vec)
+  if (vec && !bk_streams_past_llc(bk_distinct_arrays({rho_in, rho_out, grad}) * C * D))
+    bkt::k_finish_t<BK_RED_T_CP, BK_RED_T_U, 0, KV><<<dim3((unsigned)bk_cdiv(C / 2, BK_RED_T_CP)), dim3(RED_BLOCK), 0, s>>>(
+        rho_in, rho_out, ld, grad, ldg_d, metric, half, negate, kin_out, C / 2, D);
+  else if (vec)
     k_finish_v2<KV><<<dim3((unsigned)bk_cdiv(C / 2, BK_WAVE)), dim3(RED_BLOCK), 0, s>>>(
         rho_in, rho_out, ld, grad, ldg_d, metric, half, negate, kin_out, C / 2, D);
   else
@@ -745,6 +751,82 @@
   BK_RETURN_LAUNCH_STATUS();
 }
 
+static unsigned ld_rows(i64 n) { return (unsigned)(n < 1 ? 1 : (n > 65535 ? 65535 : n)); }
+
+int bk_leapfrog_kick_drift_ld(const double* theta_in, int64_t ld_ti, double* theta_out, int64_t ld_to,
+                              const double* rho_in, int64_t ld_ri, double* rho_out, int64_t ld_ro, const double* grad,
+                              int64_t ldg_d, int64_t ldg_c, const double* metric, double eps, int use_pre, double pre,
+                              int use_kick, double kick, int64_t C, int64_t D, void* stream) {
+  if (!theta_in || !theta_out || !rho_in || !rho_out || !grad || C < 0 || D < 0) return BK_E_ARG;
+  if (ld_ti < C || ld_to < C || ld_ri < C || ld_ro < C) return BK_E_ALIGN;
+  if ((theta_in == theta_out && ld_ti != ld_to) || (rho_in == rho_out && ld_ri != ld_ro)) return BK_E_ARG;
+  if (C == 0 || D == 0) return BK_OK;
+  hipStream_t s = bk_stream(stream);
+  const bool vec = ldg_c == 1 && C % 2 == 0 && ld_ti % 2 == 0 && ld_to % 2 == 0 && ld_ri % 2 == 0 && ld_ro % 2 == 0 &&
+                   ldg_d % 2 == 0 && bk_aligned16(theta_in) && bk_aligned16(theta_out) && bk_aligned16(rho_in) &&
+                   bk_aligned16(rho_out) && bk_aligned16(grad);
+  if (!vec) {
+    dim3 grid((unsigned)bk_cdiv(C, bkt::KDL_BLOCK), ld_rows(D));
+    bkt::k_kick_drift_ld_s<<<grid, dim3(bkt::KDL_BLOCK), 0, s>>>(theta_in, ld_ti, theta_out, ld_to, rho_in, ld_ri, rho_out,
+                                                                 ld_ro, grad, ldg_d, ldg_c, metric, eps, use_pre, pre,
+                                                                 use_kick, kick, C, D);
+    BK_RETURN_LAUNCH_STATUS();
+  }
+  const bool past = bk_streams_past_llc(bk_distinct_arrays({theta_in, theta_out, rho_in, rho_out, grad}) * C * D);
+  const bool out_past = bk_streams_past_llc(bk_distinct_arrays({theta_out, rho_out}) * C * D);
+  dim3 grid((unsigned)bk_cdiv(C / 2, bkt::KDL_BLOCK), ld_rows(D));
+#define BK_KDL_LAUNCH(H)                                                                                              \
+  bkt::k_kick_drift_ld<H><<<grid, dim3(bkt::KDL_BLOCK), 0, s>>>(theta_in, ld_ti, theta_out, ld_to, rho_in, ld_ri, rho_out, \
+                                                                ld_ro, grad, ldg_d, metric, eps, use_pre, pre, use_kick, \
+                                                                kick, C / 2, D)
+  if (!past) BK_KDL_LAUNCH(0);
+  else if (!out_past) BK_KDL_LAUNCH(bkt::NT_IN);
+  else BK_KDL_LAUNCH(bkt::NT_IN | bkt::NT_OUT);
+#undef BK_KDL_LAUNCH
+  BK_RETURN_LAUNCH_STATUS();
+}
+
+int bk_blend_columns_ld(const uint8_t* mask, const double* a, int64_t ld_a, const double* b, int64_t ld_b, double* out,
+                        int64_t ld_o, int64_t C, int64_t D, void* stream) {
+  if (!mask || !a || !b || !out || C < 0 || D < 0) return BK_E_ARG;
+  if (ld_a < C || ld_b < C || ld_o < C) return BK_E_ALIGN;
+  if (C == 0 || D == 0) return BK_OK;
+  hipStream_t s = bk_stream(stream);
+  if (C % 2 == 0 && ld_a % 2 == 0 && ld_b % 2 == 0 && ld_o % 2 == 0 && bk_aligned16(a) && bk_aligned16(b) &&
+      bk_aligned16(out)) {
+    dim3 grid((unsigned)bk_cdiv(C / 2, 256), ld_rows(bk_cdiv(D, bkt::SELL_ROWS)));
+    if (ld_b < ld_a)
+      bkt::k_blend_ld<bkt::NT_IN | bkt::NT_OUT><<<grid, dim3(256), 0, s>>>(mask, a, ld_a, b, ld_b, out, ld_o, C / 2, D);
+    else
+      bkt::k_blend_ld<bkt::NT_IN | bkt::NT_OUT | bkt::NT_TILE><<<grid, dim3(256), 0, s>>>(mask, a, ld_a, b, ld_b, out, ld_o,
+                                                                                        C / 2, D);
+  } else {
+    dim3 grid((unsigned)bk_cdiv(C, 256), ld_rows(D));
+    bkt::k_blend_ld_s<<<grid, dim3(256), 0, s>>>(mask, a, ld_a, b, ld_b, out, ld_o, C, D);
+  }
+  BK_RETURN_LAUNCH_STATUS();
+}
+
+int bk_select_columns_ld(const uint8_t* mask, double* dst, int64_t ld_d, const double* src, int64_t ld_s, int64_t C,
+                         int64_t D, void* stream) {
+  if (!mask || !dst || !src || C < 0 || D < 0) return BK_E_ARG;
+  if (ld_d < C || ld_s < C) return BK_E_ALIGN;
+  if (C == 0 || D == 0) return BK_OK;
+  hipStream_t s = bk_stream(stream);
+  if (C % 2 == 0 && ld_d % 2 == 0 && ld_s % 2 == 0 && bk_aligned16(dst) && bk_aligned16(src)) {
+    dim3 grid((unsigned)bk_cdiv(C / 2, 256), ld_rows(bk_cdiv(D, bkt::SELL_ROWS)));
+    if (ld_s < ld_d)
+      bkt::k_select_ld<bkt::NT_IN | bkt::NT_OUT><<<grid, dim3(256), 0, s>>>(mask, dst, ld_d, src, ld_s, C / 2, D);
+    else
+      bkt::k_select_ld<bkt::NT_IN | bkt::NT_OUT | bkt::NT_TILE><<<grid, dim3(256), 0, s>>>(mask, dst, ld_d, src, ld_s,
+                                                                                         C / 2, D);
+  } else {
+    dim3 grid((unsigned)bk_cdiv(C, 256), ld_rows(D));
+    bkt::k_select_ld_s<<<grid, dim3(256), 0, s>>>(mask, dst, ld_d, src, ld_s, C, D);
+  }
+  BK_RETURN_LAUNCH_STATUS();
+}
+
 int bk_mala_logq(const double* theta, const double* grad, const double* theta_prop,
                  const double* grad_prop, int64_t ld, double eps, double* lp_forward,
                  double* lp_reverse, int64_t C, int64_t D, void* stream) {
diff --git a/bayes-kit_amd/csrc/bk_targets.hip b/bayes-kit_amd/csrc/bk_targets.hip
--- a/bayes-kit_amd/csrc/bk_targets.hip
+++ b/bayes-kit_amd/csrc/bk_targets.hip
@@ -1,5 +1,6 @@
 #include "bk_common.hpp"
 #include "bk_elementwise.hpp"
+#include "bk_tile_kernels.hpp"
 #include "bk_mala_step.hpp"
 #include "bk_lanes.hpp"
 
@@ -160,6 +161,8 @@
   }
 };
 
+constexpr int BK_RED_T_CP = 8, BK_RED_T_U = 8;
+
 int gauss(const double* theta, double* grad, double* logp, i64 ld, const double* lam, i64 C, i64 D,
           const uint32_t* n_dev, void* stream) {
   if (!theta || (!grad && !logp) || C < 0 || D < 0) return BK_E_ARG;
@@ -175,8 +178,12 @@
     BK_RETURN_LAUNCH_STATUS();
   }
   if (logp) {
-    if (C % 2 == 0 && ld % 2 == 0 && C * D >= ((i64)1 << 22) && bk_aligned16(theta) && bk_aligned16(logp) &&
-        (!grad || bk_aligned16(grad)))
+    const bool vec = C % 2 == 0 && ld % 2 == 0 && C * D >= ((i64)1 << 22) && bk_aligned16(theta) && bk_aligned16(logp) &&
+                     (!grad || bk_aligned16(grad));
+    if (vec && !bk_streams_past_llc(bk_distinct_arrays({theta, grad}) * C * D))
+      bkt::k_gauss_logp_t<BK_RED_T_CP, BK_RED_T_U, 0><<<dim3((unsigned)bk_cdiv(C / 2, BK_RED_T_CP)), dim3(RED_BLOCK), 0, s>>>(
+          theta, grad, logp, ld, lam, C / 2, D);
+    else if (vec)
       k_gauss_logp_v2<<<dim3((unsigned)bk_cdiv(C / 2, BK_WAVE)), dim3(RED_BLOCK), 0, s>>>(theta, grad, logp, ld, lam,
                                                                                           C / 2, D);
     else
diff --git a/bayes-kit_amd/csrc/bk_tile_kernels.hpp b/bayes-kit_amd/csrc/bk_tile_kernels.hpp
--- /dev/null
+++ b/bayes-kit_amd/csrc/bk_tile_kernels.hpp
@@ -0,0 +1,311 @@
+#pragma once
+#include "bk_common.hpp"
+
+namespace bkt {
+
+typedef double dvec2 __attribute__((ext_vector_type(2)));
+
+constexpr int NT_IN = 1;
+constexpr int NT_OUT = 2;
+constexpr int NT_TILE = 4;
+
+template <bool NT, class T>
+__device__ __forceinline__ T gload(const T* p) {
+  return NT ? __builtin_nontemporal_load(p) : *p;
+}
+template <bool NT, class T>
+__device__ __forceinline__ void gstore(T v, T* p) {
+  if (NT) __builtin_nontemporal_store(v, p);
+  else *p = v;
+}
+
+__device__ __forceinline__ double kd_elem(double th, double rho, double g, double m, bool has_m, double eps, int use_pre,
+                                          double pre, int use_kick, double kick, double& rho_new) {
+  double t = has_m ? m * g : g;
+  double r = rho;
+  if (use_pre) r = r + pre * t;
+  if (use_kick) r = r + kick * t;
+  rho_new = r;
+  return th + eps * r;
+}
+
+constexpr int KDL_BLOCK = 256;
+template <int HINTS>
+__global__ __launch_bounds__(KDL_BLOCK) void k_kick_drift_ld(const double* th_in, i64 ld_ti, double* th_out, i64 ld_to,
+                                                             const double* rho_in, i64 ld_ri, double* rho_out, i64 ld_ro,
+                                                             const double* grad, i64 ldg, const double* metric, double eps,
+                                                             int use_pre, double pre, int use_kick, double kick, i64 C2,
+                                                             i64 D) {
+  constexpr bool NI = (HINTS & NT_IN) != 0, NO = (HINTS & NT_OUT) != 0;
+  const i64 c2 = (i64)blockIdx.x * KDL_BLOCK + threadIdx.x;
+  if (c2 >= C2) return;
+  for (i64 d = blockIdx.y; d < D; d += gridDim.y) {
+    const dvec2 t = gload<NI>(reinterpret_cast<const dvec2*>(th_in + d * ld_ti + 2 * c2));
+    const dvec2 r = gload<NI>(reinterpret_cast<const dvec2*>(rho_in + d * ld_ri + 2 * c2));
+    const dvec2 g = gload<NI>(reinterpret_cast<const dvec2*>(grad + d * ldg + 2 * c2));
+    const double m = metric ? metric[d] : 1.0;
+    dvec2 rn, tn;
+    double rx, ry;
+    tn.x = kd_elem(t.x, r.x, g.x, m, metric != nullptr, eps, use_pre, pre, use_kick, kick, rx);
+    tn.y = kd_elem(t.y, r.y, g.y, m, metric != nullptr, eps, use_pre, pre, use_kick, kick, ry);
+    rn.x = rx;
+    rn.y = ry;
+    gstore<NO>(rn, reinterpret_cast<dvec2*>(rho_out + d * ld_ro + 2 * c2));
+    gstore<NO>(tn, reinterpret_cast<dvec2*>(th_out + d * ld_to + 2 * c2));
+  }
+}
+
+static __global__ __launch_bounds__(KDL_BLOCK) void k_kick_drift_ld_s(const double* th_in, i64 ld_ti, double* th_out, i64 ld_to,
+                                                               const double* rho_in, i64 ld_ri, double* rho_out, i64 ld_ro,
+                                                               const double* grad, i64 ldg_d, i64 ldg_c,
+                                                               const double* metric, double eps, int use_pre, double pre,
+                                                               int use_kick, double kick, i64 C, i64 D) {
+  const i64 c = (i64)blockIdx.x * KDL_BLOCK + threadIdx.x;
+  if (c >= C) return;
+  for (i64 d = blockIdx.y; d < D; d += gridDim.y) {
+    double rn;
+    const double m = metric ? metric[d] : 1.0;
+    const double tn = kd_elem(th_in[d * ld_ti + c], rho_in[d * ld_ri + c], grad[d * ldg_d + c * ldg_c], m,
+                              metric != nullptr, eps, use_pre, pre, use_kick, kick, rn);
+    rho_out[d * ld_ro + c] = rn;
+    th_out[d * ld_to + c] = tn;
+  }
+}
+
+constexpr int SELL_ROWS = 2;
+template <int HINTS>
+__global__ __launch_bounds__(256) void k_blend_ld(const uint8_t* mask, const double* a, i64 ld_a, const double* b, i64 ld_b,
+                                                  double* out, i64 ld_o, i64 C2, i64 D) {
+  constexpr bool NI = (HINTS & NT_IN) != 0, NO = (HINTS & NT_OUT) != 0, NB = (HINTS & NT_TILE) != 0;
+  const i64 c2 = (i64)blockIdx.x * 256 + threadIdx.x;
+  if (c2 >= C2) return;
+  const bool m0 = mask[2 * c2] != 0, m1 = mask[2 * c2 + 1] != 0;
+  for (i64 d0 = (i64)blockIdx.y * SELL_ROWS; d0 < D; d0 += (i64)gridDim.y * SELL_ROWS) {
+    dvec2 v[SELL_ROWS];
+#pragma unroll
+    for (int i = 0; i < SELL_ROWS; ++i)
+      if (d0 + i < D) {
+        if (m0 || m1) v[i] = gload<NB>(reinterpret_cast<const dvec2*>(b + (d0 + i) * ld_b + 2 * c2));
+        if (!(m0 && m1)) {
+          const dvec2 old = gload<NI>(reinterpret_cast<const dvec2*>(a + (d0 + i) * ld_a + 2 * c2));
+          if (!m0) v[i].x = old.x;
+          if (!m1) v[i].y = old.y;
+        }
+      }
+#pragma unroll
+    for (int i = 0; i < SELL_ROWS; ++i)
+      if (d0 + i < D) gstore<NO>(v[i], reinterpret_cast<dvec2*>(out + (d0 + i) * ld_o + 2 * c2));
+  }
+}
+
+static __global__ __launch_bounds__(256) void k_blend_ld_s(const uint8_t* mask, const double* a, i64 ld_a, const double* b, i64 ld_b,
+                                                    double* out, i64 ld_o, i64 C, i64 D) {
+  const i64 c = (i64)blockIdx.x * 256 + threadIdx.x;
+  if (c >= C) return;
+  const bool m = mask[c] != 0;
+  for (i64 d = blockIdx.y; d < D; d += gridDim.y) out[d * ld_o + c] = m ? b[d * ld_b + c] : a[d * ld_a + c];
+}
+
+template <int HINTS>
+__global__ __launch_bounds__(256) void k_select_ld(const uint8_t* mask, double* dst, i64 ld_d, const double* src, i64 ld_s,
+                                                   i64 C2, i64 D) {
+  constexpr bool NI = (HINTS & NT_IN) != 0, NO = (HINTS & NT_OUT) != 0, NB = (HINTS & NT_TILE) != 0;
+  const i64 c2 = (i64)blockIdx.x * 256 + threadIdx.x;
+  if (c2 >= C2) return;
+  const bool m0 = mask[2 * c2] != 0, m1 = mask[2 * c2 + 1] != 0;
+  for (i64 d0 = (i64)blockIdx.y * SELL_ROWS; d0 < D; d0 += (i64)gridDim.y * SELL_ROWS) {
+    dvec2 v[SELL_ROWS];
+#pragma unroll
+    for (int i = 0; i < SELL_ROWS; ++i)
+      if (d0 + i < D) {
+        if (m0 || m1) v[i] = gload<NB>(reinterpret_cast<const dvec2*>(src + (d0 + i) * ld_s + 2 * c2));
+        if (!(m0 && m1)) {
+          const dvec2 old = gload<NI>(reinterpret_cast<const dvec2*>(dst + (d0 + i) * ld_d + 2 * c2));
+          if (!m0) v[i].x = old.x;
+          if (!m1) v[i].y = old.y;
+        }
+      }
+#pragma unroll
+    for (int i = 0; i < SELL_ROWS; ++i)
+      if (d0 + i < D) gstore<NO>(v[i], reinterpret_cast<dvec2*>(dst + (d0 + i) * ld_d + 2 * c2));
+  }
+}
+
+static __global__ __launch_bounds__(256) void k_select_ld_s(const uint8_t* mask, double* dst, i64 ld_d, const double* src, i64 ld_s,
+                                                     i64 C, i64 D) {
+  const i64 c = (i64)blockIdx.x * 256 + threadIdx.x;
+  if (c >= C || !mask[c]) return;
+  for (i64 d = blockIdx.y; d < D; d += gridDim.y) dst[d * ld_d + c] = src[d * ld_s + c];
+}
+
+constexpr int RED_WAVES = 4;
+constexpr int RED_BLOCK = RED_WAVES * BK_WAVE;
+
+template <int CP, int U, int HINTS>
+__global__ __launch_bounds__(RED_BLOCK) void k_gauss_logp_t(const double* th, double* g, double* logp, i64 ld,
+                                                            const double* lam, i64 C2, i64 D) {
+  constexpr bool NI = (HINTS & NT_IN) != 0, NO = (HINTS & NT_OUT) != 0;
+  constexpr int PH = BK_WAVE / CP, R = U * PH;
+  __shared__ dvec2 term[RED_WAVES][R][CP];
+  __shared__ dvec2 part[RED_WAVES][CP];
+  const int lane = threadIdx.x & (BK_WAVE - 1), w = bk_wave_id(), j = lane % CP, ph = lane / CP;
+  const i64 c2 = (i64)blockIdx.x * CP + j;
+  const bool on = c2 < C2;
+  const i64 Dq = (D + RED_WAVES - 1) / RED_WAVES;
+  const i64 dlo = w * Dq, dhi = (dlo + Dq < D) ? dlo + Dq : D;
+  const double* p = th + 2 * c2;
+  double* q = g ? g + 2 * c2 : nullptr;
+  dvec2 t[U];
+  double l[U];
+  auto load = [&](i64 d0) {
+#pragma unroll
+    for (int u = 0; u < U; ++u) {
+      const i64 d = d0 + u * PH + ph;
+      if (on && d < dhi) {
+        t[u] = gload<NI>(reinterpret_cast<const dvec2*>(p + d * ld));
+        l[u] = lam ? lam[d] : 1.0;
+      }
+    }
+  };
+  dvec2 s = {0.0, 0.0};
+  load(dlo);
+  for (i64 r0 = 0; r0 < Dq; r0 += R) {
+    const i64 d0 = dlo + r0;
+#pragma unroll
+    for (int u = 0; u < U; ++u) {
+      const i64 d = d0 + u * PH + ph;
+      if (on && d < dhi) {
+        dvec2 lt = t[u];
+        if (lam) {
+          lt.x = l[u] * t[u].x;
+          lt.y = l[u] * t[u].y;
+        }
+        dvec2 tm;
+        tm.x = t[u].x * lt.x;
+        tm.y = t[u].y * lt.y;
+        term[w][u * PH + ph][j] = tm;
+        if (q) {
+          dvec2 o = {-lt.x, -lt.y};
+          gstore<NO>(o, reinterpret_cast<dvec2*>(q + d * ld));
+        }
+      }
+    }
+    load(d0 + R);
+    __syncthreads();
+    if (ph == 0 && on) {
+      const i64 left = dhi - d0;
+      const int nr = (int)(left < R ? (left < 0 ? 0 : left) : R);
+#pragma unroll 8
+      for (int r = 0; r < nr; ++r) {
+        const dvec2 tm = term[w][r][j];
+        s.x = s.x + tm.x;
+        s.y = s.y + tm.y;
+      }
+    }
+    __syncthreads();
+  }
+  if (ph == 0) part[w][j] = s;
+  __syncthreads();
+  if (w == 0 && ph == 0 && on) {
+    dvec2 tot = part[0][j];
+#pragma unroll
+    for (int k = 1; k < RED_WAVES; ++k) {
+      tot.x = tot.x + part[k][j].x;
+      tot.y = tot.y + part[k][j].y;
+    }
+    tot.x = -0.5 * tot.x;
+    tot.y = -0.5 * tot.y;
+    *reinterpret_cast<dvec2*>(logp + 2 * c2) = tot;
+  }
+}
+
+template <int CP, int U, int HINTS, bool KV>
+__global__ __launch_bounds__(RED_BLOCK) void k_finish_t(const double* rho_in, double* rho_out, i64 ld, const double* grad,
+                                                        i64 ldg, const double* metric, double half, int negate,
+                                                        double* kin_out, i64 C2, i64 D) {
+  constexpr bool NI = (HINTS & NT_IN) != 0, NO = (HINTS & NT_OUT) != 0;
+  constexpr int PH = BK_WAVE / CP, R = U * PH;
+  __shared__ dvec2 term[RED_WAVES][R][CP];
+  __shared__ dvec2 part[RED_WAVES][CP];
+  const int lane = threadIdx.x & (BK_WAVE - 1), w = bk_wave_id(), j = lane % CP, ph = lane / CP;
+  const i64 c2 = (i64)blockIdx.x * CP + j;
+  const bool on = c2 < C2;
+  const i64 Dq = (D + RED_WAVES - 1) / RED_WAVES;
+  const i64 dlo = w * Dq, dhi = (dlo + Dq < D) ? dlo + Dq : D;
+  const double* pr = rho_in + 2 * c2;
+  const double* pg = grad ? grad + 2 * c2 : nullptr;
+  double* qr = rho_out ? rho_out + 2 * c2 : nullptr;
+  dvec2 r[U], g[U];
+  double m[U], km[U];
+  auto load = [&](i64 d0) {
+#pragma unroll
+    for (int u = 0; u < U; ++u) {
+      const i64 d = d0 + u * PH + ph;
+      if (on && d < dhi) {
+        r[u] = gload<NI>(reinterpret_cast<const dvec2*>(pr + d * ld));
+        if (pg) g[u] = gload<NI>(reinterpret_cast<const dvec2*>(pg + d * ldg));
+        m[u] = metric ? metric[d] : 1.0;
+        km[u] = KV ? metric[2 * D + d] : m[u];
+      }
+    }
+  };
+  dvec2 kin = {0.0, 0.0};
+  load(dlo);
+  for (i64 r0 = 0; r0 < Dq; r0 += R) {
+    const i64 d0 = dlo + r0;
+#pragma unroll
+    for (int u = 0; u < U; ++u) {
+      const i64 d = d0 + u * PH + ph;
+      if (on && d < dhi) {
+        dvec2 v = r[u];
+        if (pg) {
+          const double tx = metric ? m[u] * g[u].x : g[u].x, ty = metric ? m[u] * g[u].y : g[u].y;
+          v.x = r[u].x + half * tx;
+          v.y = r[u].y + half * ty;
+        }
+        if (negate) {
+          v.x = -v.x;
+          v.y = -v.y;
+        }
+        if (qr) gstore<NO>(v, reinterpret_cast<dvec2*>(qr + d * ld));
+        if (kin_out) {
+          const double mx = metric ? km[u] * v.x : v.x, my = metric ? km[u] * v.y : v.y;
+          dvec2 tm;
+          tm.x = v.x * mx;
+          tm.y = v.y * my;
+          term[w][u * PH + ph][j] = tm;
+        }
+      }
+    }
+    load(d0 + R);
+    if (!kin_out) continue;
+    __syncthreads();
+    if (ph == 0 && on) {
+      const i64 left = dhi - d0;
+      const int nr = (int)(left < R ? (left < 0 ? 0 : left) : R);
+#pragma unroll 8
+      for (int i = 0; i < nr; ++i) {
+        const dvec2 tm = term[w][i][j];
+        kin.x = kin.x + tm.x;
+        kin.y = kin.y + tm.y;
+      }
+    }
+    __syncthreads();
+  }
+  if (!kin_out) return;
+  if (ph == 0) part[w][j] = kin;
+  __syncthreads();
+  if (w == 0 && ph == 0 && on) {
+    dvec2 s = part[0][j];
+#pragma unroll
+    for (int k = 1; k < RED_WAVES; ++k) {
+      s.x = s.x + part[k][j].x;
+      s.y = s.y + part[k][j].y;
+    }
+    s.x = 0.5 * s.x;
+    s.y = 0.5 * s.y;
+    *reinterpret_cast<dvec2*>(kin_out + 2 * c2) = s;
+  }
+}
+
+}
diff --git a/include/bkhip.h b/include/bkhip.h
--- a/include/bkhip.h
+++ b/include/bkhip.h
@@ -105,6 +105,15 @@
 int bk_blend_columns(const uint8_t* mask, const double* a, const double* b, double* out,
                      int64_t ld, int64_t C, int64_t D, void* stream);
 
+int bk_leapfrog_kick_drift_ld(const double* theta_in, int64_t ld_theta_in, double* theta_out, int64_t ld_theta_out,
+                              const double* rho_in, int64_t ld_rho_in, double* rho_out, int64_t ld_rho_out,
+                              const double* grad, int64_t ldg_d, int64_t ldg_c, const double* metric, double eps,
+                              int use_pre, double pre, int use_kick, double kick, int64_t C, int64_t D, void* stream);
+int bk_blend_columns_ld(const uint8_t* mask, const double* a, int64_t ld_a, const double* b, int64_t ld_b, double* out,
+                        int64_t ld_out, int64_t C, int64_t D, void* stream);
+int bk_select_columns_ld(const uint8_t* mask, double* dst, int64_t ld_dst, const double* src, int64_t ld_src,
+                         int64_t C, int64_t D, void* stream);
+
 
 int bk_compact_indices(const uint8_t* mask, int64_t n, int32_t* idx_out, uint32_t* count_out,
                        const uint32_t* n_dev, void* stream);
```

Result: faster. 116.4 million leapfrog steps/sec, median of 6 (+4.2%).
